# DavidPeicho/loupiote

Measured on AMD Instinct MI355X. Metric: Mrays/s (+ ms/frame) at 1920×1080, 4 spp, Sponza; 1/2/4/8 GPU, higher is better.
Workload: dtype f32

## Files before the change

bindings/rust/loupiote_hip/src/ffi.rs:

```rust
#![allow(non_camel_case_types, non_upper_case_globals, dead_code)]
use std::os::raw::{c_char, c_int, c_uint, c_void};

pub const LPT_ABI_VERSION: u32 = 6;
pub const LPT_INVALID_INDEX: u32 = 0xFFFFFFFF;
pub const LPT_ACCEL_BUILD_HOST_SAH: u32 = 0;
pub const LPT_ACCEL_BUILD_GPU_LBVH: u32 = 1;
pub const LPT_UPLOAD_NO_TEXTURE_PAIRS: u32 = 0x100;
pub const LPT_COMM_ID_BYTES: u32 = 128;
pub const LPT_OK: c_int = 0;
pub const LPT_ERR_FILE_NOT_FOUND: c_int = 1;
pub const LPT_ERR_READBACK: c_int = 2;
pub const LPT_ERR_ACCEL_BUILD: c_int = 3;
pub const LPT_ERR_HIP: c_int = 4;
pub const LPT_ERR_RCCL: c_int = 5;
pub const LPT_ERR_INVALID_ARG: c_int = 6;
pub const LPT_BLIT_PATHTRACE: c_int = 0;
pub const LPT_BLIT_DENOISED: c_int = 1;
pub const LPT_BLIT_TEMPORAL: c_int = 2;
pub const LPT_BLIT_GBUFFER: c_int = 3;
pub const LPT_BLIT_MOTION: c_int = 4;
pub const LPT_HOST_FRAME_HOST_ONLY: c_int = 1;
pub const LPT_EXCHANGE_GATHER_TILES: c_int = 0;
pub const LPT_EXCHANGE_REDUCE: c_int = 1;
pub const LPT_OPT_PACKET_PRIMARY: c_int = 1;
pub const LPT_OPT_WAVEFRONT_RAYS: c_int = 2;
pub const LPT_OPT_PATH_RAYS: c_int = 3;
pub const LPT_OPT_COOP_RAYS: c_int = 4;
pub const LPT_OPT_TAIL_LANES: c_int = 5;
pub const LPT_OPT_EXPERIMENT_BASE: c_int = 256;
pub const LPT_EXP_PIPE_RAYS: c_int = 0;
pub const LPT_EXP_REFILL: c_int = 1;
pub const LPT_EXP_TRACE_WAVES_PER_CU: c_int = 2;
pub const LPT_EXP_SHADE_BLOCKS_PER_CU: c_int = 3;
pub const LPT_EXP_PATH_WAVES_PER_CU: c_int = 4;
pub const LPT_EXP_PATH_REFILL: c_int = 5;
pub const LPT_EXP_OCC_CELL_MILLI: c_int = 6;
pub const LPT_EXP_STEP_BUDGET: c_int = 7;
pub const LPT_EXP_BUDGET_RAYS: c_int = 8;
pub const LPT_EXP_PACKET_QUADS: c_int = 9;
pub const LPT_EXP_SPLIT_RAYS: c_int = 10;
pub const LPT_EXP_BUDGET_SPLIT: c_int = 11;

#[repr(C)] pub struct lpt_device { _private: [u8; 0] }
#[repr(C)] pub struct lpt_scene { _private: [u8; 0] }
#[repr(C)] pub struct lpt_scene_gpu { _private: [u8; 0] }
#[repr(C)] pub struct lpt_probe { _private: [u8; 0] }
#[repr(C)] pub struct lpt_renderer { _private: [u8; 0] }
#[repr(C)] pub struct lpt_comm { _private: [u8; 0] }
#[repr(C)] pub struct lpt_host_frame { _private: [u8; 0] }

#[repr(C)] #[derive(Copy, Clone, Debug)]
pub struct lpt_material {
    pub color: [f32; 4],
    pub roughness: f32,
    pub reflectivity: f32,
    pub albedo_texture: u32,
    pub mra_texture: u32,
}
#[repr(C)] #[derive(Copy, Clone, Debug)]
pub struct lpt_vertex {
    pub position: [f32; 4],
    pub normal: [f32; 4],
}
#[repr(C)] #[derive(Copy, Clone, Debug)]
pub struct lpt_light {
    pub normal: [f32; 4],
    pub tangent: [f32; 4],
    pub bitangent: [f32; 4],
    pub origin: [f32; 4],
}
#[repr(C)] #[derive(Copy, Clone, Debug)]
pub struct lpt_instance {
    pub model_to_world: [f32; 16],
    pub blas_index: u32,
    pub material_index: u32,
    pub pad: [u32; 2],
}
#[repr(C)] #[derive(Copy, Clone, Debug)]
pub struct lpt_blas_entry {
    pub vertex_offset: u32,
    pub vertex_count: u32,
    pub index_offset: u32,
    pub index_count: u32,
}
#[repr(C)] #[derive(Copy, Clone, Debug)]
pub struct lpt_scene_counts {
    pub materials: u32,
    pub entries: u32,
    pub vertices: u32,
    pub indices: u32,
    pub instances: u32,
    pub lights: u32,
    pub images: u32,
}
#[repr(C)] #[derive(Copy, Clone, Debug)]
pub struct lpt_accel_stats {
    pub triangles: u32,
    pub nodes: u32,
    pub node_bytes: u32,
    pub tri_bytes: u32,
    pub max_depth: u32,
    pub build_ms: f32,
    pub host_baked_triangles: u32,
    pub upload_ms: f32,
    pub texture_pairs: u32,
    pub texture_bytes_resident: u64,
}
#[repr(C)] #[derive(Copy, Clone, Debug)]
pub struct lpt_hit {
    pub t: f32,
    pub u: f32,
    pub v: f32,
    pub prim: u32,
}
#[repr(C)] #[derive(Copy, Clone, Debug)]
pub struct lpt_ray_counts {
    pub closest: u64,
    pub shadow: u64,
    pub shaded: u64,
    pub nodes: u64,
    pub tris: u64,
    pub shadow_nodes: u64,
    pub shadow_tris: u64,
    pub wave_steps: u64,
    pub live_lanes: u64,
    pub node_lanes: u64,
    pub tri_lanes: u64,
    pub primary: u64,
    pub packet_nodes: u64,
    pub packet_tris: u64,
    pub shadow_occluded: u64,
    pub occluder_cache_found: u64,
    pub occluder_cache_hits: u64,
    pub wave_rays: u64,
}
#[repr(C)] #[derive(Copy, Clone, Debug)]
pub struct lpt_timing {
    pub label: [c_char; 32],
    pub ms: f32,
    pub launches: u32,
}

#[link(name = "loupiote_hip")]
extern "C" {
    pub fn lpt_last_error() -> *const c_char;
    pub fn lpt_status_string(status: c_int) -> *const c_char;
    pub fn lpt_abi_version() -> u32;
    pub fn lpt_device_create(hip_ordinal: c_int, out: *mut *mut lpt_device) -> c_int;
    pub fn lpt_device_destroy(dev: *mut lpt_device) -> c_int;
    pub fn lpt_device_synchronize(dev: *mut lpt_device) -> c_int;
    pub fn lpt_device_info(dev: *mut lpt_device, name: *mut c_char, name_cap: usize, compute_units: *mut c_int) -> c_int;
    pub fn lpt_device_stream(dev: *mut lpt_device, hip_stream: *mut *mut c_void) -> c_int;
    pub fn lpt_scene_create(out: *mut *mut lpt_scene) -> c_int;
    pub fn lpt_scene_destroy(scene: *mut lpt_scene) -> c_int;
    pub fn lpt_scene_counts_get(scene: *const lpt_scene, out: *mut lpt_scene_counts) -> c_int;
    pub fn lpt_scene_add_mesh(scene: *mut lpt_scene, positions: *const c_void, position_stride: usize, normals: *const c_void, normal_stride: usize, uvs: *const c_void, uv_stride: usize, vertex_count: u32, indices: *const u32, index_count: u32, out_blas_index: *mut u32) -> c_int;
    pub fn lpt_scene_add_instance(scene: *mut lpt_scene, blas_index: u32, model_to_world: *const f32, material_index: u32, out_instance_index: *mut u32) -> c_int;
    pub fn lpt_scene_set_instance_transform(scene: *mut lpt_scene, instance_index: u32, model_to_world: *const f32) -> c_int;
    pub fn lpt_scene_add_material(scene: *mut lpt_scene, m: *const lpt_material, out_index: *mut u32) -> c_int;
    pub fn lpt_scene_add_image(scene: *mut lpt_scene, rgba8: *const u8, width: u32, height: u32, out_index: *mut u32) -> c_int;
    pub fn lpt_scene_add_light(scene: *mut lpt_scene, l: *const lpt_light, out_index: *mut u32) -> c_int;
    pub fn lpt_scene_set_light(scene: *mut lpt_scene, index: u32, l: *const lpt_light) -> c_int;
    pub fn lpt_light_default(out: *mut lpt_light) -> c_int;
    pub fn lpt_scene_get_materials(s: *const lpt_scene, first: u32, count: u32, dst: *mut lpt_material) -> c_int;
    pub fn lpt_scene_get_entries(s: *const lpt_scene, first: u32, count: u32, dst: *mut lpt_blas_entry) -> c_int;
    pub fn lpt_scene_get_vertices(s: *const lpt_scene, first: u32, count: u32, dst: *mut lpt_vertex) -> c_int;
    pub fn lpt_scene_get_indices(s: *const lpt_scene, first: u32, count: u32, dst: *mut u32) -> c_int;
    pub fn lpt_scene_get_instances(s: *const lpt_scene, first: u32, count: u32, dst: *mut lpt_instance) -> c_int;
    pub fn lpt_scene_get_lights(s: *const lpt_scene, first: u32, count: u32, dst: *mut lpt_light) -> c_int;
    pub fn lpt_scene_get_image(s: *const lpt_scene, index: u32, width: *mut u32, height: *mut u32, dst_rgba8: *mut u8) -> c_int;
    pub fn lpt_load_gltf(scene: *mut lpt_scene, data: *const u8, size: usize) -> c_int;
    pub fn lpt_load_gltf_path(scene: *mut lpt_scene, path: *const c_char) -> c_int;
    pub fn lpt_write_png(path: *const c_char, rgba8: *const u8, width: u32, height: u32, row_bytes: usize) -> c_int;
    pub fn lpt_decode_hdr(data: *const u8, size: usize, rgbe8: *mut u8, capacity: usize, width: *mut u32, height: *mut u32) -> c_int;
    pub fn lpt_decode_image(data: *const u8, size: usize, rgba8: *mut u8, capacity: usize, width: *mut u32, height: *mut u32) -> c_int;
    pub fn lpt_write_hdr(path: *const c_char, rgba: *const f32, width: u32, height: u32, row_floats: usize) -> c_int;
    pub fn lpt_scene_upload(dev: *mut lpt_device, scene: *const lpt_scene, out: *mut *mut lpt_scene_gpu) -> c_int;
    pub fn lpt_scene_upload_ex(dev: *mut lpt_device, scene: *const lpt_scene, flags: u32, out: *mut *mut lpt_scene_gpu) -> c_int;
    pub fn lpt_scene_gpu_destroy(sg: *mut lpt_scene_gpu) -> c_int;
    pub fn lpt_scene_gpu_update_instances(scene_gpu: *mut lpt_scene_gpu, scene: *const lpt_scene, out_rebaked: *mut u32) -> c_int;
    pub fn lpt_scene_gpu_rebuild(scene_gpu: *mut lpt_scene_gpu, scene: *const lpt_scene) -> c_int;
    pub fn lpt_scene_gpu_stats(sg: *const lpt_scene_gpu, out: *mut lpt_accel_stats) -> c_int;
    pub fn lpt_probe_upload(dev: *mut lpt_device, rgbe8: *const u8, width: u32, height: u32, out: *mut *mut lpt_probe) -> c_int;
    pub fn lpt_probe_destroy(probe: *mut lpt_probe) -> c_int;
    pub fn lpt_trace_closest(dev: *mut lpt_device, sg: *const lpt_scene_gpu, origins: *const f32, dirs: *const f32, n: u32, out_hits: *mut lpt_hit) -> c_int;
    pub fn lpt_trace_occluded(dev: *mut lpt_device, sg: *const lpt_scene_gpu, origins: *const f32, dirs: *const f32, tmax: *const f32, n: u32, out_occluded: *mut u8) -> c_int;
    pub fn lpt_renderer_create(dev: *mut lpt_device, width: u32, height: u32, out: *mut *mut lpt_renderer) -> c_int;
    pub fn lpt_renderer_destroy(r: *mut lpt_renderer) -> c_int;
    pub fn lpt_renderer_set_downsample(r: *mut lpt_renderer, factor: f32) -> c_int;
    pub fn lpt_renderer_resize(r: *mut lpt_renderer, sg: *const lpt_scene_gpu, probe_or_null: *const lpt_probe, width: u32, height: u32) -> c_int;
    pub fn lpt_renderer_get_size(r: *const lpt_renderer, width: *mut u32, height: *mut u32) -> c_int;
    pub fn lpt_max_per_pixel_bytes() -> u32;
    pub fn lpt_renderer_set_resources(r: *mut lpt_renderer, sg: *const lpt_scene_gpu, probe_or_null: *const lpt_probe) -> c_int;
    pub fn lpt_renderer_raytrace(r: *mut lpt_renderer, view_transform: *const f32) -> c_int;
    pub fn lpt_renderer_submit(r: *mut lpt_renderer) -> c_int;
    pub fn lpt_renderer_set_max_fused(r: *mut lpt_renderer, n: u32) -> c_int;
    pub fn lpt_renderer_get_submission_stats(r: *const lpt_renderer, recorded_calls: *mut u64, wavefronts: *mut u64, pending_calls: *mut u32) -> c_int;
    pub fn lpt_renderer_raytrace_n(r: *mut lpt_renderer, view_transform: *const f32, n_samples: u32) -> c_int;
    pub fn lpt_renderer_reset_accumulation(r: *mut lpt_renderer) -> c_int;
    pub fn lpt_renderer_set_accumulate(r: *mut lpt_renderer, accumulate: c_int) -> c_int;
    pub fn lpt_renderer_get_accumulate(r: *const lpt_renderer, accumulate: *mut c_int) -> c_int;
    pub fn lpt_renderer_get_frame_state(r: *const lpt_renderer, frame_count: *mut u32, seed: *mut u32) -> c_int;
    pub fn lpt_renderer_upload_noise(r: *mut lpt_renderer, rgba8: *const u8, width: u32, height: u32, bytes_per_row: u32) -> c_int;
    pub fn lpt_renderer_use_noise(r: *mut lpt_renderer, flag: c_int) -> c_int;
    pub fn lpt_renderer_set_blit_mode(r: *mut lpt_renderer, mode: c_int) -> c_int;
    pub fn lpt_renderer_read_denoiser(r: *mut lpt_renderer, gbuffer: *mut u32, motion: *mut f32, radiance: *mut f32, history: *mut u32) -> c_int;
    pub fn lpt_renderer_blit_rgba8(r: *mut lpt_renderer, dst: *mut u8, row_bytes: usize) -> c_int;
    pub fn lpt_renderer_read_pixels(r: *mut lpt_renderer, dst: *mut u8) -> c_int;
    pub fn lpt_renderer_read_radiance(r: *mut lpt_renderer, dst: *mut f32) -> c_int;
    pub fn lpt_host_alloc(bytes: usize, out: *mut *mut c_void) -> c_int;
    pub fn lpt_host_free(ptr: *mut c_void) -> c_int;
    pub fn lpt_host_register(ptr: *mut c_void, bytes: usize) -> c_int;
    pub fn lpt_host_unregister(ptr: *mut c_void) -> c_int;
    pub fn lpt_renderer_read_radiance_owned(r: *mut lpt_renderer, frame_dst: *mut f32) -> c_int;
    pub fn lpt_host_frame_create(name: *const c_char, width: u32, height: u32, world: u32, flags: u32, out: *mut *mut lpt_host_frame) -> c_int;
    pub fn lpt_host_frame_attach(name: *const c_char, width: u32, height: u32, world: u32, flags: u32, out: *mut *mut lpt_host_frame) -> c_int;
    pub fn lpt_host_frame_ptr(f: *mut lpt_host_frame, frame: *mut *mut f32) -> c_int;
    pub fn lpt_host_frame_barrier(f: *mut lpt_host_frame, rank: u32, frame_no: u32, timeout_ms: u32) -> c_int;
    pub fn lpt_host_frame_destroy(f: *mut lpt_host_frame) -> c_int;
    pub fn lpt_renderer_get_timings(r: *mut lpt_renderer, out: *mut lpt_timing, inout_count: *mut c_int) -> c_int;
    pub fn lpt_renderer_enable_timings(r: *mut lpt_renderer, flag: c_int) -> c_int;
    pub fn lpt_renderer_set_max_bounces(r: *mut lpt_renderer, bounces: u32) -> c_int;
    pub fn lpt_renderer_set_seed(r: *mut lpt_renderer, user_seed: u32) -> c_int;
    pub fn lpt_renderer_set_vfov(r: *mut lpt_renderer, radians: f32) -> c_int;
    pub fn lpt_renderer_set_shard(r: *mut lpt_renderer, rank: u32, world_size: u32, tile_w: u32, tile_h: u32) -> c_int;
    pub fn lpt_renderer_set_shard_weighted(r: *mut lpt_renderer, rank: u32, world_size: u32, tile_w: u32, tile_h: u32, weights_or_null: *const u32) -> c_int;
    pub fn lpt_renderer_denoiser_inputs(r: *mut lpt_renderer, noisy: *mut *mut c_void, gbuffer: *mut *mut c_void, motion: *mut *mut c_void, n_pixels: *mut usize) -> c_int;
    pub fn lpt_renderer_denoise_filter(r: *mut lpt_renderer) -> c_int;
    pub fn lpt_renderer_radiance_device_ptr(r: *mut lpt_renderer, device_ptr: *mut *mut c_void, bytes: *mut usize) -> c_int;
    pub fn lpt_comm_unique_id(out_id: *mut c_void) -> c_int;
    pub fn lpt_comm_create(dev: *mut lpt_device, id: *const c_void, rank: c_int, world_size: c_int, out: *mut *mut lpt_comm) -> c_int;
    pub fn lpt_comm_destroy(comm: *mut lpt_comm) -> c_int;
    pub fn lpt_comm_info(comm: *const lpt_comm, rank: *mut c_int, world_size: *mut c_int) -> c_int;
    pub fn lpt_comm_group_begin() -> c_int;
    pub fn lpt_comm_group_end() -> c_int;
    pub fn lpt_renderer_set_comm(r: *mut lpt_renderer, comm_or_null: *mut lpt_comm) -> c_int;
    pub fn lpt_renderer_set_comm_weighted(r: *mut lpt_renderer, comm_or_null: *mut lpt_comm, weights_or_null: *const u32) -> c_int;
    pub fn lpt_renderer_exchange(r: *mut lpt_renderer, mode: c_int) -> c_int;
    pub fn lpt_renderer_exchange_local(root: *mut lpt_renderer, peers: *const *mut lpt_renderer, n_peers: c_int) -> c_int;
    pub fn lpt_renderer_set_lanes(r: *mut lpt_renderer, lanes: c_int) -> c_int;
    pub fn lpt_renderer_set_sort_queues(r: *mut lpt_renderer, flag: c_int) -> c_int;
    pub fn lpt_renderer_set_option(r: *mut lpt_renderer, option: c_int, value: u64) -> c_int;
    pub fn lpt_renderer_get_option(r: *const lpt_renderer, option: c_int, value: *mut u64) -> c_int;
    pub fn lpt_shard_layout(width: u32, height: u32, tile_w: u32, tile_h: u32, world_size: u32, rank: u32, out_slots: *mut u32, out_slot_offset: *mut u32) -> c_int;
    pub fn lpt_shard_layout_weighted(width: u32, height: u32, tile_w: u32, tile_h: u32, world_size: u32, rank: u32, weights_or_null: *const u32, out_slots: *mut u32, out_slot_offset: *mut u32) -> c_int;
    pub fn lpt_shard_owner(world_size: u32, weights_or_null: *const u32, tile: u32, out_rank: *mut u32) -> c_int;
    pub fn lpt_renderer_get_ray_counts(r: *mut lpt_renderer, out: *mut lpt_ray_counts) -> c_int;
    pub fn lpt_renderer_get_queue_counts(r: *mut lpt_renderer, closest: *mut u32, shadow: *mut u32, cap: u32) -> c_int;
    pub fn lpt_renderer_reset_ray_counts(r: *mut lpt_renderer) -> c_int;
    pub fn lpt_renderer_get_step_histogram(r: *mut lpt_renderer, max_steps: *mut u32, hist12: *mut u32) -> c_int;
    pub fn lpt_renderer_enable_stats(r: *mut lpt_renderer, flag: c_int) -> c_int;
    pub fn lpt_renderer_synchronize(r: *mut lpt_renderer) -> c_int;
    pub fn lpt_renderer_stream(r: *mut lpt_renderer, hip_stream: *mut *mut c_void) -> c_int;
}
```

include/lpt.h:

```cpp
#ifndef LPT_H
#define LPT_H

#include <stddef.h>
#include <stdint.h>

#ifdef __cplusplus
extern "C" {
#endif

#define LPT_ABI_VERSION 6u

#define LPT_INVALID_INDEX 0xFFFFFFFFu

enum {
    LPT_OK = 0,
    LPT_ERR_FILE_NOT_FOUND = 1,
    LPT_ERR_READBACK = 2,
    LPT_ERR_ACCEL_BUILD = 3,
    LPT_ERR_HIP = 4,
    LPT_ERR_RCCL = 5,
    LPT_ERR_INVALID_ARG = 6
};

const char *lpt_last_error(void);
const char *lpt_status_string(int status);
uint32_t lpt_abi_version(void);


typedef struct lpt_material {
    float color[4];
    float roughness;
    float reflectivity;
    uint32_t albedo_texture;
    uint32_t mra_texture;
} lpt_material;

typedef struct lpt_vertex {
    float position[4];
    float normal[4];
} lpt_vertex;

typedef struct lpt_light {
    float normal[4];
    float tangent[4];
    float bitangent[4];
    float origin[4];
} lpt_light;

typedef struct lpt_instance {
    float model_to_world[16];
    uint32_t blas_index;
    uint32_t material_index;
    uint32_t pad[2];
} lpt_instance;

typedef struct lpt_blas_entry {
    uint32_t vertex_offset;
    uint32_t vertex_count;
    uint32_t index_offset;
    uint32_t index_count;
} lpt_blas_entry;

typedef struct lpt_scene_counts {
    uint32_t materials, entries, vertices, indices, instances, lights, images;
} lpt_scene_counts;

typedef struct lpt_accel_stats {
    uint32_t triangles;
    uint32_t nodes;
    uint32_t node_bytes;
    uint32_t tri_bytes;
    uint32_t max_depth;
    float build_ms;
    uint32_t host_baked_triangles;
    float upload_ms;
    uint32_t texture_pairs;
    uint64_t texture_bytes_resident;
} lpt_accel_stats;

typedef struct lpt_hit {
    float t, u, v;
    uint32_t prim;
} lpt_hit;

typedef struct lpt_ray_counts {
    uint64_t closest;
    uint64_t shadow;
    uint64_t shaded;
    uint64_t nodes;
    uint64_t tris;
    uint64_t shadow_nodes;
    uint64_t shadow_tris;
    uint64_t wave_steps;
    uint64_t live_lanes;
    uint64_t node_lanes;
    uint64_t tri_lanes;
    uint64_t primary;
    uint64_t packet_nodes;
    uint64_t packet_tris;
    uint64_t shadow_occluded;
    uint64_t occluder_cache_found;
    uint64_t occluder_cache_hits;
    uint64_t wave_rays;
} lpt_ray_counts;

typedef struct lpt_timing {
    char label[32];
    float ms;
    uint32_t launches;
} lpt_timing;

enum {
    LPT_BLIT_PATHTRACE = 0,
    LPT_BLIT_DENOISED = 1,
    LPT_BLIT_TEMPORAL = 2,
    LPT_BLIT_GBUFFER = 3,
    LPT_BLIT_MOTION = 4
};

typedef struct lpt_device lpt_device;
typedef struct lpt_scene lpt_scene;
typedef struct lpt_scene_gpu lpt_scene_gpu;
typedef struct lpt_probe lpt_probe;
typedef struct lpt_renderer lpt_renderer;
typedef struct lpt_comm lpt_comm;

int lpt_device_create(int hip_ordinal, lpt_device **out);
int lpt_device_destroy(lpt_device *dev);
int lpt_device_synchronize(lpt_device *dev);
int lpt_device_info(lpt_device *dev, char *name, size_t name_cap, int *compute_units);
int lpt_device_stream(lpt_device *dev, void **hip_stream);

int lpt_scene_create(lpt_scene **out);
int lpt_scene_destroy(lpt_scene *scene);
int lpt_scene_counts_get(const lpt_scene *scene, lpt_scene_counts *out);

int lpt_scene_add_mesh(lpt_scene *scene, const void *positions, size_t position_stride,
                       const void *normals, size_t normal_stride, const void *uvs,
                       size_t uv_stride, uint32_t vertex_count, const uint32_t *indices,
                       uint32_t index_count, uint32_t *out_blas_index);
int lpt_scene_add_instance(lpt_scene *scene, uint32_t blas_index, const float model_to_world[16],
                           uint32_t material_index, uint32_t *out_instance_index);
int lpt_scene_set_instance_transform(lpt_scene *scene, uint32_t instance_index,
                                     const float model_to_world[16]);
int lpt_scene_add_material(lpt_scene *scene, const lpt_material *m, uint32_t *out_index);
int lpt_scene_add_image(lpt_scene *scene, const uint8_t *rgba8, uint32_t width, uint32_t height,
                        uint32_t *out_index);
int lpt_scene_add_light(lpt_scene *scene, const lpt_light *l, uint32_t *out_index);
int lpt_scene_set_light(lpt_scene *scene, uint32_t index, const lpt_light *l);
int lpt_light_default(lpt_light *out);

int lpt_scene_get_materials(const lpt_scene *s, uint32_t first, uint32_t count, lpt_material *dst);
int lpt_scene_get_entries(const lpt_scene *s, uint32_t first, uint32_t count, lpt_blas_entry *dst);
int lpt_scene_get_vertices(const lpt_scene *s, uint32_t first, uint32_t count, lpt_vertex *dst);
int lpt_scene_get_indices(const lpt_scene *s, uint32_t first, uint32_t count, uint32_t *dst);
int lpt_scene_get_instances(const lpt_scene *s, uint32_t first, uint32_t count, lpt_instance *dst);
int lpt_scene_get_lights(const lpt_scene *s, uint32_t first, uint32_t count, lpt_light *dst);
int lpt_scene_get_image(const lpt_scene *s, uint32_t index, uint32_t *width, uint32_t *height,
                        uint8_t *dst_rgba8 );

int lpt_load_gltf(lpt_scene *scene, const uint8_t *data, size_t size);
int lpt_load_gltf_path(lpt_scene *scene, const char *path);

int lpt_write_png(const char *path, const uint8_t *rgba8, uint32_t width, uint32_t height, size_t row_bytes);

int lpt_decode_hdr(const uint8_t *data, size_t size, uint8_t *rgbe8, size_t capacity, uint32_t *width, uint32_t *height);

int lpt_decode_image(const uint8_t *data, size_t size, uint8_t *rgba8, size_t capacity, uint32_t *width, uint32_t *height);

int lpt_write_hdr(const char *path, const float *rgba, uint32_t width, uint32_t height, size_t row_floats);

int lpt_scene_upload(lpt_device *dev, const lpt_scene *scene, lpt_scene_gpu **out);
#define LPT_ACCEL_BUILD_HOST_SAH 0u
#define LPT_ACCEL_BUILD_GPU_LBVH 1u
#define LPT_UPLOAD_NO_TEXTURE_PAIRS 0x100u
int lpt_scene_upload_ex(lpt_device *dev, const lpt_scene *scene, uint32_t flags, lpt_scene_gpu **out);
int lpt_scene_gpu_destroy(lpt_scene_gpu *sg);
int lpt_scene_gpu_update_instances(lpt_scene_gpu *scene_gpu, const lpt_scene *scene, uint32_t *out_rebaked);
int lpt_scene_gpu_rebuild(lpt_scene_gpu *scene_gpu, const lpt_scene *scene);
int lpt_scene_gpu_stats(const lpt_scene_gpu *sg, lpt_accel_stats *out);

int lpt_probe_upload(lpt_device *dev, const uint8_t *rgbe8, uint32_t width, uint32_t height,
                     lpt_probe **out);
int lpt_probe_destroy(lpt_probe *probe);

int lpt_trace_closest(lpt_device *dev, const lpt_scene_gpu *sg, const float *origins,
                      const float *dirs, uint32_t n, lpt_hit *out_hits);
int lpt_trace_occluded(lpt_device *dev, const lpt_scene_gpu *sg, const float *origins,
                       const float *dirs, const float *tmax, uint32_t n, uint8_t *out_occluded);

int lpt_renderer_create(lpt_device *dev, uint32_t width, uint32_t height, lpt_renderer **out);
int lpt_renderer_destroy(lpt_renderer *r);
int lpt_renderer_set_downsample(lpt_renderer *r, float factor);
int lpt_renderer_resize(lpt_renderer *r, const lpt_scene_gpu *sg, const lpt_probe *probe_or_null,
                        uint32_t width, uint32_t height);
int lpt_renderer_get_size(const lpt_renderer *r, uint32_t *width, uint32_t *height);
uint32_t lpt_max_per_pixel_bytes(void);
int lpt_renderer_set_resources(lpt_renderer *r, const lpt_scene_gpu *sg,
                               const lpt_probe *probe_or_null);
int lpt_renderer_raytrace(lpt_renderer *r, const float view_transform[16]);
int lpt_renderer_submit(lpt_renderer *r);
int lpt_renderer_set_max_fused(lpt_renderer *r, uint32_t n);
int lpt_renderer_get_submission_stats(const lpt_renderer *r, uint64_t *recorded_calls, uint64_t *wavefronts, uint32_t *pending_calls);
int lpt_renderer_raytrace_n(lpt_renderer *r, const float view_transform[16], uint32_t n_samples);
int lpt_renderer_reset_accumulation(lpt_renderer *r);
int lpt_renderer_set_accumulate(lpt_renderer *r, int accumulate);
int lpt_renderer_get_accumulate(const lpt_renderer *r, int *accumulate);
int lpt_renderer_get_frame_state(const lpt_renderer *r, uint32_t *frame_count, uint32_t *seed);
int lpt_renderer_upload_noise(lpt_renderer *r, const uint8_t *rgba8, uint32_t width,
                              uint32_t height, uint32_t bytes_per_row);
int lpt_renderer_use_noise(lpt_renderer *r, int flag);
int lpt_renderer_set_blit_mode(lpt_renderer *r, int mode);
int lpt_renderer_read_denoiser(lpt_renderer *r, uint32_t *gbuffer, float *motion, float *radiance, uint32_t *history);
int lpt_renderer_blit_rgba8(lpt_renderer *r, uint8_t *dst, size_t row_bytes);
int lpt_renderer_read_pixels(lpt_renderer *r, uint8_t *dst);
int lpt_renderer_read_radiance(lpt_renderer *r, float *dst);
int lpt_host_alloc(size_t bytes, void **out);
int lpt_host_free(void *ptr);
int lpt_host_register(void *ptr, size_t bytes);
int lpt_host_unregister(void *ptr);
int lpt_renderer_read_radiance_owned(lpt_renderer *r, float *frame_dst);
typedef struct lpt_host_frame lpt_host_frame;
enum { LPT_HOST_FRAME_HOST_ONLY = 1 };
int lpt_host_frame_create(const char *name, uint32_t width, uint32_t height, uint32_t world, uint32_t flags, lpt_host_frame **out);
int lpt_host_frame_attach(const char *name, uint32_t width, uint32_t height, uint32_t world, uint32_t flags, lpt_host_frame **out);
int lpt_host_frame_ptr(lpt_host_frame *f, float **frame);
int lpt_host_frame_barrier(lpt_host_frame *f, uint32_t rank, uint32_t frame_no, uint32_t timeout_ms);
int lpt_host_frame_destroy(lpt_host_frame *f);
int lpt_renderer_get_timings(lpt_renderer *r, lpt_timing *out, int *inout_count);
int lpt_renderer_enable_timings(lpt_renderer *r, int flag);

int lpt_renderer_set_max_bounces(lpt_renderer *r, uint32_t bounces);
int lpt_renderer_set_seed(lpt_renderer *r, uint32_t user_seed);
int lpt_renderer_set_vfov(lpt_renderer *r, float radians);
int lpt_renderer_set_shard(lpt_renderer *r, uint32_t rank, uint32_t world_size, uint32_t tile_w,
                           uint32_t tile_h);
int lpt_renderer_set_shard_weighted(lpt_renderer *r, uint32_t rank, uint32_t world_size, uint32_t tile_w, uint32_t tile_h,
                                    const uint32_t *weights_or_null);
int lpt_renderer_denoiser_inputs(lpt_renderer *r, void **noisy, void **gbuffer, void **motion, size_t *n_pixels);
int lpt_renderer_denoise_filter(lpt_renderer *r);
int lpt_renderer_radiance_device_ptr(lpt_renderer *r, void **device_ptr, size_t *bytes);
#define LPT_COMM_ID_BYTES 128
int lpt_comm_unique_id(void *out_id );
int lpt_comm_create(lpt_device *dev, const void *id , int rank, int world_size, lpt_comm **out);
int lpt_comm_destroy(lpt_comm *comm);
int lpt_comm_info(const lpt_comm *comm, int *rank, int *world_size);
int lpt_comm_group_begin(void);
int lpt_comm_group_end(void);

enum {
    LPT_EXCHANGE_GATHER_TILES = 0,
    LPT_EXCHANGE_REDUCE = 1
};
int lpt_renderer_set_comm(lpt_renderer *r, lpt_comm *comm_or_null);
int lpt_renderer_set_comm_weighted(lpt_renderer *r, lpt_comm *comm_or_null, const uint32_t *weights_or_null);
int lpt_renderer_exchange(lpt_renderer *r, int mode);
int lpt_renderer_exchange_local(lpt_renderer *root, lpt_renderer *const *peers, int n_peers);

int lpt_renderer_set_lanes(lpt_renderer *r, int lanes);
int lpt_renderer_set_sort_queues(lpt_renderer *r, int flag);
typedef enum lpt_option {
    LPT_OPT_PACKET_PRIMARY = 1,
    LPT_OPT_WAVEFRONT_RAYS = 2,
    LPT_OPT_PATH_RAYS = 3,
    LPT_OPT_COOP_RAYS = 4,
    LPT_OPT_TAIL_LANES = 5,
    LPT_OPT_EXPERIMENT_BASE = 256
} lpt_option;
#define LPT_OPT_EXPERIMENT(name) (LPT_OPT_EXPERIMENT_BASE + (name))
typedef enum lpt_experiment {
    LPT_EXP_PIPE_RAYS = 0,
    LPT_EXP_REFILL = 1,
    LPT_EXP_TRACE_WAVES_PER_CU = 2,
    LPT_EXP_SHADE_BLOCKS_PER_CU = 3,
    LPT_EXP_PATH_WAVES_PER_CU = 4,
    LPT_EXP_PATH_REFILL = 5,
    LPT_EXP_OCC_CELL_MILLI = 6,
    LPT_EXP_STEP_BUDGET = 7,
    LPT_EXP_BUDGET_RAYS = 8,
    LPT_EXP_PACKET_QUADS = 9,
    LPT_EXP_SPLIT_RAYS = 10,
    LPT_EXP_BUDGET_SPLIT = 11
} lpt_experiment;
int lpt_renderer_set_option(lpt_renderer *r, int option, uint64_t value);
int lpt_renderer_get_option(const lpt_renderer *r, int option, uint64_t *value);
int lpt_shard_layout(uint32_t width, uint32_t height, uint32_t tile_w, uint32_t tile_h, uint32_t world_size, uint32_t rank,
                     uint32_t *out_slots, uint32_t *out_slot_offset);
int lpt_shard_layout_weighted(uint32_t width, uint32_t height, uint32_t tile_w, uint32_t tile_h, uint32_t world_size, uint32_t rank,
                              const uint32_t *weights_or_null, uint32_t *out_slots, uint32_t *out_slot_offset);
int lpt_shard_owner(uint32_t world_size, const uint32_t *weights_or_null, uint32_t tile, uint32_t *out_rank);
int lpt_renderer_get_ray_counts(lpt_renderer *r, lpt_ray_counts *out);
int lpt_renderer_get_queue_counts(lpt_renderer *r, uint32_t *closest, uint32_t *shadow, uint32_t cap);
int lpt_renderer_reset_ray_counts(lpt_renderer *r);
int lpt_renderer_get_step_histogram(lpt_renderer *r, uint32_t *max_steps, uint32_t *hist12);
int lpt_renderer_enable_stats(lpt_renderer *r, int flag);
int lpt_renderer_synchronize(lpt_renderer *r);
int lpt_renderer_stream(lpt_renderer *r, void **hip_stream);

#ifdef __cplusplus
}
#endif
#endif
```

loupiote_amd/_abi.py:

```python
import ctypes as C
import os

import numpy as np

_HERE = os.path.dirname(os.path.abspath(__file__))
LIB_PATH = os.environ.get("LPT_LIB_PATH") or os.path.join(_HERE, "libloupiote_hip.so")

LPT_OK = 0
LPT_ERR_FILE_NOT_FOUND = 1
LPT_ERR_READBACK = 2
LPT_ERR_ACCEL_BUILD = 3
LPT_ERR_HIP = 4
LPT_ERR_RCCL = 5
LPT_ERR_INVALID_ARG = 6
COMM_ID_BYTES = 128
OPT_EXPERIMENT_BASE = 256
OPTIONS = {"packet_primary": 1, "wavefront_rays": 2, "path_rays": 3, "coop_rays": 4, "tail_lanes": 5}
EXPERIMENTS = {"pipe_rays": 0, "refill": 1, "trace_waves_per_cu": 2, "shade_blocks_per_cu": 3, "path_waves_per_cu": 4, "path_refill": 5, "occ_cell_milli": 6,
               "step_budget": 7, "budget_rays": 8, "packet_quads": 9, "split_rays": 10, "budget_split": 11}
OPTIONS.update({k: OPT_EXPERIMENT_BASE + v for k, v in EXPERIMENTS.items()})
EXCHANGE_GATHER_TILES = 0
HOST_FRAME_HOST_ONLY = 1
EXCHANGE_REDUCE = 1
INVALID_INDEX = 0xFFFFFFFF
LIGHT_BIT = 0x80000000

MATERIAL_DT = np.dtype([("color", "<f4", 4), ("roughness", "<f4"), ("reflectivity", "<f4"),
                        ("albedo_texture", "<u4"), ("mra_texture", "<u4")])
VERTEX_DT = np.dtype([("position", "<f4", 4), ("normal", "<f4", 4)])
LIGHT_DT = np.dtype([("normal", "<f4", 4), ("tangent", "<f4", 4), ("bitangent", "<f4", 4), ("origin", "<f4", 4)])
INSTANCE_DT = np.dtype([("model_to_world", "<f4", 16), ("blas_index", "<u4"), ("material_index", "<u4"),
                        ("pad", "<u4", 2)])
ENTRY_DT = np.dtype([("vertex_offset", "<u4"), ("vertex_count", "<u4"), ("index_offset", "<u4"),
                     ("index_count", "<u4")])
HIT_DT = np.dtype([("t", "<f4"), ("u", "<f4"), ("v", "<f4"), ("prim", "<u4")])


class SceneCounts(C.Structure):
    _fields_ = [(n, C.c_uint32) for n in ("materials", "entries", "vertices", "indices", "instances", "lights", "images")]


class AccelStats(C.Structure):
    _fields_ = [("triangles", C.c_uint32), ("nodes", C.c_uint32), ("node_bytes", C.c_uint32),
                ("tri_bytes", C.c_uint32), ("max_depth", C.c_uint32), ("build_ms", C.c_float),
                ("host_baked_triangles", C.c_uint32), ("upload_ms", C.c_float),
                ("texture_pairs", C.c_uint32), ("texture_bytes_resident", C.c_uint64)]


class RayCounts(C.Structure):
    _fields_ = [(n, C.c_uint64) for n in ("closest", "shadow", "shaded", "nodes", "tris", "shadow_nodes", "shadow_tris",
                                             "wave_steps", "live_lanes", "node_lanes", "tri_lanes", "primary", "packet_nodes", "packet_tris",
                                             "shadow_occluded", "occluder_cache_found", "occluder_cache_hits", "wave_rays")]


class Timing(C.Structure):
    _fields_ = [("label", C.c_char * 32), ("ms", C.c_float), ("launches", C.c_uint32)]


_vp, _u32, _i, _f, _sz = C.c_void_p, C.c_uint32, C.c_int, C.c_float, C.c_size_t
_pvp = C.POINTER(C.c_void_p)
_pu32 = C.POINTER(C.c_uint32)

SIGNATURES = {
    "lpt_last_error": (C.c_char_p, []),
    "lpt_status_string": (C.c_char_p, [_i]),
    "lpt_abi_version": (_u32, []),
    "lpt_device_create": (_i, [_i, _pvp]),
    "lpt_device_destroy": (_i, [_vp]),
    "lpt_device_synchronize": (_i, [_vp]),
    "lpt_device_info": (_i, [_vp, C.c_char_p, _sz, C.POINTER(_i)]),
    "lpt_device_stream": (_i, [_vp, _pvp]),
    "lpt_scene_create": (_i, [_pvp]),
    "lpt_scene_destroy": (_i, [_vp]),
    "lpt_scene_counts_get": (_i, [_vp, C.POINTER(SceneCounts)]),
    "lpt_scene_add_mesh": (_i, [_vp, _vp, _sz, _vp, _sz, _vp, _sz, _u32, _vp, _u32, _pu32]),
    "lpt_scene_add_instance": (_i, [_vp, _u32, _vp, _u32, _pu32]),
    "lpt_scene_set_instance_transform": (_i, [_vp, _u32, _vp]),
    "lpt_scene_add_material": (_i, [_vp, _vp, _pu32]),
    "lpt_scene_add_image": (_i, [_vp, _vp, _u32, _u32, _pu32]),
    "lpt_scene_add_light": (_i, [_vp, _vp, _pu32]),
    "lpt_scene_set_light": (_i, [_vp, _u32, _vp]),
    "lpt_light_default": (_i, [_vp]),
    "lpt_scene_get_materials": (_i, [_vp, _u32, _u32, _vp]),
    "lpt_scene_get_entries": (_i, [_vp, _u32, _u32, _vp]),
    "lpt_scene_get_vertices": (_i, [_vp, _u32, _u32, _vp]),
    "lpt_scene_get_indices": (_i, [_vp, _u32, _u32, _vp]),
    "lpt_scene_get_instances": (_i, [_vp, _u32, _u32, _vp]),
    "lpt_scene_get_lights": (_i, [_vp, _u32, _u32, _vp]),
    "lpt_scene_get_image": (_i, [_vp, _u32, _pu32, _pu32, _vp]),
    "lpt_load_gltf": (_i, [_vp, _vp, _sz]),
    "lpt_load_gltf_path": (_i, [_vp, C.c_char_p]),
    "lpt_decode_hdr": (_i, [_vp, C.c_size_t, _vp, C.c_size_t, C.POINTER(C.c_uint32), C.POINTER(C.c_uint32)]),
    "lpt_decode_image": (_i, [_vp, C.c_size_t, _vp, C.c_size_t, C.POINTER(C.c_uint32), C.POINTER(C.c_uint32)]),
    "lpt_write_hdr": (_i, [C.c_char_p, _vp, _u32, _u32, _sz]),
    "lpt_write_png": (_i, [C.c_char_p, _vp, _u32, _u32, _sz]),
    "lpt_scene_upload": (_i, [_vp, _vp, _pvp]),
    "lpt_scene_upload_ex": (_i, [_vp, _vp, _u32, _pvp]),
    "lpt_scene_gpu_destroy": (_i, [_vp]),
    "lpt_scene_gpu_stats": (_i, [_vp, C.POINTER(AccelStats)]),
    "lpt_scene_gpu_rebuild": (_i, [_vp, _vp]),
    "lpt_scene_gpu_update_instances": (_i, [_vp, _vp, C.POINTER(C.c_uint32)]),
    "lpt_probe_upload": (_i, [_vp, _vp, _u32, _u32, _pvp]),
    "lpt_probe_destroy": (_i, [_vp]),
    "lpt_trace_closest": (_i, [_vp, _vp, _vp, _vp, _u32, _vp]),
    "lpt_trace_occluded": (_i, [_vp, _vp, _vp, _vp, _vp, _u32, _vp]),
    "lpt_renderer_create": (_i, [_vp, _u32, _u32, _pvp]),
    "lpt_renderer_destroy": (_i, [_vp]),
    "lpt_renderer_set_downsample": (_i, [_vp, _f]),
    "lpt_renderer_resize": (_i, [_vp, _vp, _vp, _u32, _u32]),
    "lpt_renderer_get_size": (_i, [_vp, _pu32, _pu32]),
    "lpt_max_per_pixel_bytes": (_u32, []),
    "lpt_renderer_set_resources": (_i, [_vp, _vp, _vp]),
    "lpt_renderer_raytrace": (_i, [_vp, _vp]),
    "lpt_renderer_raytrace_n": (_i, [_vp, _vp, _u32]),
    "lpt_renderer_submit": (_i, [_vp]),
    "lpt_renderer_set_max_fused": (_i, [_vp, _u32]),
    "lpt_renderer_get_submission_stats": (_i, [_vp, C.POINTER(C.c_uint64), C.POINTER(C.c_uint64), _pu32]),
    "lpt_host_alloc": (_i, [_sz, _pvp]),
    "lpt_host_free": (_i, [_vp]),
    "lpt_host_register": (_i, [_vp, _sz]),
    "lpt_host_unregister": (_i, [_vp]),
    "lpt_renderer_read_radiance_owned": (_i, [_vp, _vp]),
    "lpt_host_frame_create": (_i, [C.c_char_p, _u32, _u32, _u32, _u32, _pvp]),
    "lpt_host_frame_attach": (_i, [C.c_char_p, _u32, _u32, _u32, _u32, _pvp]),
    "lpt_host_frame_ptr": (_i, [_vp, _pvp]),
    "lpt_host_frame_barrier": (_i, [_vp, _u32, _u32, _u32]),
    "lpt_host_frame_destroy": (_i, [_vp]),
    "lpt_renderer_reset_accumulation": (_i, [_vp]),
    "lpt_renderer_set_accumulate": (_i, [_vp, _i]),
    "lpt_renderer_get_accumulate": (_i, [_vp, C.POINTER(_i)]),
    "lpt_renderer_get_frame_state": (_i, [_vp, _pu32, _pu32]),
    "lpt_renderer_upload_noise": (_i, [_vp, _vp, _u32, _u32, _u32]),
    "lpt_renderer_use_noise": (_i, [_vp, _i]),
    "lpt_renderer_set_blit_mode": (_i, [_vp, _i]),
    "lpt_renderer_blit_rgba8": (_i, [_vp, _vp, _sz]),
    "lpt_renderer_read_pixels": (_i, [_vp, _vp]),
    "lpt_renderer_read_radiance": (_i, [_vp, _vp]),
    "lpt_renderer_read_denoiser": (_i, [_vp, _vp, _vp, _vp, _vp]),
    "lpt_renderer_get_timings": (_i, [_vp, _vp, C.POINTER(_i)]),
    "lpt_renderer_enable_timings": (_i, [_vp, _i]),
    "lpt_renderer_set_max_bounces": (_i, [_vp, _u32]),
    "lpt_renderer_set_seed": (_i, [_vp, _u32]),
    "lpt_renderer_set_vfov": (_i, [_vp, _f]),
    "lpt_renderer_set_shard": (_i, [_vp, _u32, _u32, _u32, _u32]),
    "lpt_renderer_radiance_device_ptr": (_i, [_vp, _pvp, C.POINTER(_sz)]),
    "lpt_renderer_denoiser_inputs": (_i, [_vp, C.POINTER(C.c_void_p), C.POINTER(C.c_void_p), C.POINTER(C.c_void_p), C.POINTER(C.c_size_t)]),
    "lpt_renderer_denoise_filter": (_i, [_vp]),
    "lpt_comm_unique_id": (_i, [_vp]),
    "lpt_comm_create": (_i, [_vp, _vp, _i, _i, _pvp]),
    "lpt_comm_destroy": (_i, [_vp]),
    "lpt_comm_info": (_i, [_vp, C.POINTER(_i), C.POINTER(_i)]),
    "lpt_comm_group_begin": (_i, []),
    "lpt_comm_group_end": (_i, []),
    "lpt_renderer_set_comm": (_i, [_vp, _vp]),
    "lpt_renderer_exchange": (_i, [_vp, _i]),
    "lpt_renderer_exchange_local": (_i, [_vp, _pvp, _i]),
    "lpt_shard_layout": (_i, [_u32, _u32, _u32, _u32, _u32, _u32, _pu32, _pu32]),
    "lpt_shard_layout_weighted": (_i, [_u32, _u32, _u32, _u32, _u32, _u32, _vp, _pu32, _pu32]),
    "lpt_shard_owner": (_i, [_u32, _vp, _u32, _pu32]),
    "lpt_renderer_set_shard_weighted": (_i, [_vp, _u32, _u32, _u32, _u32, _vp]),
    "lpt_renderer_set_comm_weighted": (_i, [_vp, _vp, _vp]),
    "lpt_renderer_set_lanes": (_i, [_vp, _i]),
    "lpt_renderer_set_sort_queues": (_i, [_vp, _i]),
    "lpt_renderer_set_option": (_i, [_vp, _i, C.c_uint64]),
    "lpt_renderer_get_option": (_i, [_vp, _i, C.POINTER(C.c_uint64)]),
    "lpt_renderer_get_queue_counts": (_i, [_vp, _vp, _vp, _u32]),
    "lpt_renderer_get_ray_counts": (_i, [_vp, C.POINTER(RayCounts)]),
    "lpt_renderer_reset_ray_counts": (_i, [_vp]),
    "lpt_renderer_get_step_histogram": (_i, [_vp, _pu32, _vp]),
    "lpt_renderer_enable_stats": (_i, [_vp, _i]),
    "lpt_renderer_synchronize": (_i, [_vp]),
    "lpt_renderer_stream": (_i, [_vp, _pvp]),
}

_LIB = None


def lib():
    global _LIB
    if _LIB is None:
        if not os.path.exists(LIB_PATH):
            raise ImportError(
                "loupiote_amd: %s is missing — build it with `python -c 'import __graft_entry__ as g; g.build()'` "
                "(hipcc --offload-arch=gfx950).  There is no fallback path." % LIB_PATH)
        L = C.CDLL(LIB_PATH)
        for name, (res, args) in SIGNATURES.items():
            if os.environ.get("LPT_ABI_LENIENT") and not hasattr(L, name):
                continue
            fn = getattr(L, name)
            fn.restype = res
            fn.argtypes = args
        _LIB = L
    return _LIB


def ptr(a):
    return None if a is None else a.ctypes.data_as(C.c_void_p)
```

loupiote_amd/csrc/device.hip:

```cpp
#include <hip/hip_runtime.h>

#include <dlfcn.h>

#include <algorithm>
#include <cmath>
#include <map>
#include <memory>
#include <cstdlib>
#include <mutex>
#include <new>
#include <numeric>

#include "common.h"
#include "kernels.h"
#include "build_kernels.h"
#include <hipcub/hipcub.hpp>
#include <rccl/rccl.h>

using namespace lpt;
using namespace lptd;

#define TRY(expr) do { const int st__ = (expr); if (st__ != LPT_OK) return st__; } while (0)
#define HIP_TRY(expr)                                                                              \
    do {                                                                                           \
        hipError_t e__ = (expr);                                                                   \
        if (e__ != hipSuccess) return fail(LPT_ERR_HIP, "%s failed: %s", #expr, hipGetErrorString(e__)); \
    } while (0)

struct lpt_device {
    int ordinal = 0;
    hipStream_t stream = nullptr;
    int compute_units = 0;
    char name[128] = {0};
    std::vector<lpt_renderer *> renderers;
};

struct lpt_comm {
    lpt_device *dev = nullptr;
    ncclComm_t comm = nullptr;
    int rank = 0, world = 1;
};

struct Rccl {
    void *handle = nullptr;
    ncclResult_t (*GetUniqueId)(ncclUniqueId *) = nullptr;
    ncclResult_t (*CommInitRank)(ncclComm_t *, int, ncclUniqueId, int) = nullptr;
    ncclResult_t (*CommDestroy)(ncclComm_t) = nullptr;
    ncclResult_t (*CommCount)(const ncclComm_t, int *) = nullptr;
    ncclResult_t (*CommUserRank)(const ncclComm_t, int *) = nullptr;
    ncclResult_t (*GroupStart)() = nullptr;
    ncclResult_t (*GroupEnd)() = nullptr;
    ncclResult_t (*Send)(const void *, size_t, ncclDataType_t, int, ncclComm_t, hipStream_t) = nullptr;
    ncclResult_t (*Recv)(void *, size_t, ncclDataType_t, int, ncclComm_t, hipStream_t) = nullptr;
    ncclResult_t (*Reduce)(const void *, void *, size_t, ncclDataType_t, ncclRedOp_t, int, ncclComm_t, hipStream_t) = nullptr;
    const char *(*GetErrorString)(ncclResult_t) = nullptr;
};
static const Rccl *rccl() {
    static Rccl table;
    static int state = 0;
    static std::string why = "missing symbol";
    static std::mutex mu;
    std::lock_guard<std::mutex> lock(mu);
    if (state == 1) return &table;
    if (state == 0) {
        const char *names[] = {"librccl.so.1", "librccl.so", "/opt/rocm/lib/librccl.so.1", "/opt/rocm/lib/librccl.so"};
        std::string rocm_path;
        if (const char *rp = getenv("ROCM_PATH")) rocm_path = std::string(rp) + "/lib/librccl.so";
        void *h = nullptr;
        state = -1;
        if (const char *lp = getenv("LPT_RCCL_LIBRARY")) { h = dlopen(lp, RTLD_NOW | RTLD_LOCAL); rocm_path.clear(); if (!h) { if (const char *e = dlerror()) why = e; goto rccl_done; } }
        if (!rocm_path.empty()) h = dlopen(rocm_path.c_str(), RTLD_NOW | RTLD_LOCAL);
        for (size_t i = 0; !h && i < sizeof names / sizeof names[0]; ++i) h = dlopen(names[i], RTLD_NOW | RTLD_LOCAL);
        if (!h) { if (const char *e = dlerror()) why = e; }
        if (h) {
            table.handle = h;
            bool ok = true;
#define RCCL_SYM(field, sym) do { *(void **)(&table.field) = dlsym(h, sym); if (!table.field) ok = false; } while (0)
            RCCL_SYM(GetUniqueId, "ncclGetUniqueId"); RCCL_SYM(CommInitRank, "ncclCommInitRank"); RCCL_SYM(CommDestroy, "ncclCommDestroy");
            RCCL_SYM(CommCount, "ncclCommCount"); RCCL_SYM(CommUserRank, "ncclCommUserRank");
            RCCL_SYM(GroupStart, "ncclGroupStart"); RCCL_SYM(GroupEnd, "ncclGroupEnd"); RCCL_SYM(Send, "ncclSend"); RCCL_SYM(Recv, "ncclRecv");
            RCCL_SYM(Reduce, "ncclReduce"); RCCL_SYM(GetErrorString, "ncclGetErrorString");
#undef RCCL_SYM
            if (ok) state = 1;
        }
    rccl_done:;
    }
    if (state == 1) return &table;
    fail(LPT_ERR_RCCL, "librccl could not be loaded (%s): the multi-GPU frame exchange needs RCCL", why.c_str());
    return nullptr;
}

#define RCCL_TRY(expr)                                                                                \
    do {                                                                                              \
        ncclResult_t r__ = (expr);                                                                    \
        if (r__ != ncclSuccess) return fail(LPT_ERR_RCCL, "%s failed: %s", #expr, rccl() ? rccl()->GetErrorString(r__) : "?"); \
    } while (0)

struct HipFree { void operator()(void *p) const { hipFree(p); } };
using DevMem = std::unique_ptr<void, HipFree>;
template <typename T> static inline T *as(const DevMem &m) { return (T *)m.get(); }

struct DevTree {
    DevMem nodes, woop, leaf_prim;
    DevMem node_lo, node_hi;
    std::vector<uint32_t> level_start;
    uint32_t n_nodes = 0, max_depth = 0;
    float build_ms = 0.f;
};

struct TexturePairs {
    std::map<std::pair<uint32_t, uint32_t>, uint32_t> map;
    std::vector<DImage> descs;
    std::vector<uint8_t> image_resident;
};

struct lpt_scene_gpu {
    lpt_device *dev = nullptr;
    DScene d{};
    float max_abs = 0.f;
    DevTree tree;
    DevMem tri_verts, materials, lights, texels, images, srgb_lut, pair_texels, pair_images;
    TexturePairs pairs;
    lpt_accel_stats stats{};
    DevMem obj_verts, obj_indices, bad_flag;
    DevMem arena;
    size_t arena_bytes = 0;
    std::vector<uint32_t> inst_first, inst_count;
    std::vector<lpt_instance> instances;
    size_t n_entries = 0, n_vertices = 0, n_indices = 0;
};

struct lpt_probe {
    lpt_device *dev = nullptr;
    DProbe d{};
    void *rgbe = nullptr;
};

enum { ST_RAYGEN = 0, ST_INTERSECT, ST_SHADE, ST_SHADOW, ST_ACCUM, ST_ASVGF, ST_EXCHANGE, ST_PRIMARY, ST_PATH, ST_COUNT };
static const char *kStageLabel[ST_COUNT] = {"ray generation", "intersection", "shading", "shadow", "accumulation", "asvgf", "exchange", "primary intersection", "path"};

struct Wavefront {
    hipStream_t stream = nullptr;
    Queue q[2]{};
    ShadowQueue sq{};
    float4 *hits = nullptr, *Lsum = nullptr;
    uint32_t *strag = nullptr;
    FrameCounters *ctr = nullptr;
    size_t ray_cap = 0;
    hipEvent_t done = nullptr;
    hipEvent_t consumed = nullptr;
    bool consumed_recorded = false;
};
constexpr int kMaxLanes = 4;
constexpr uint32_t kStepBudget = 48u, kBudgetRays = 3000000u;
constexpr float kPacketMaxPixelRad = 1.8e-3f;
constexpr uint32_t kOccEntries = 1u << 18;
constexpr uint32_t kPathRays = 120000u;
constexpr uint64_t kSplitRays = 3000000ull;
constexpr uint32_t kCoopRays = 32000u;
constexpr uint32_t kPacketBlocksPerCu = 128u;
constexpr uint32_t kCoopWavesPerCu = 32u;
constexpr uint64_t kWavefrontRays = 1ull << 22;

struct lpt_renderer {
    lpt_device *dev = nullptr;
    hipStream_t stream = nullptr;
    Wavefront wf[kMaxLanes];
    int n_lanes = 2;
    uint32_t lane_rr = 0;
    int last_lane = 0;
    uint32_t req_w = 0, req_h = 0, w = 0, h = 0;
    float downsample = 0.5f;
    const lpt_scene_gpu *sg = nullptr;
    const lpt_probe *probe = nullptr;
    bool resources_set = false;
    uint32_t frame_count = 1, seed = 0;
    bool accumulate = false, frame_back = true;
    struct Pending { float view[16]; uint32_t n = 0, frame_count0 = 1, seed0 = 0; bool acc0 = false; } pend;
    uint32_t max_fused = 0;
    uint32_t packet_primary = 2u;
    uint32_t pipe_rays = 0x7FFFFFFFu;
    uint64_t wavefront_rays = kWavefrontRays;
    uint32_t path_rays = kPathRays;
    uint32_t path_waves_per_cu = 16;
    int path_refill = 32;
    uint64_t n_recorded = 0, n_wavefronts = 0;
    int mode = LPT_BLIT_PATHTRACE;
    uint32_t max_bounces = 3, user_seed = 0;
    float vfov = 0.78539816339744830962f;
    uint32_t rank = 0, world = 1, tile_w = 32, tile_h = 8;
    std::vector<uint32_t> weights;
    ShardMap map{1u, 1u, {0u}};
    ShardTable h_table{};
    std::vector<uint32_t> h_offset;
    ShardTable *d_table = nullptr;
    bool use_noise = false, stats = false, timings = false;
    int refill = 44;
    int sort_queues = 0;
    uint32_t shade_blocks_per_cu = 0;
    uint32_t trace_waves_per_cu = 0;
    uint32_t n_slots = 0;
    float4 *accum = nullptr, *scratch = nullptr;
    lpt_comm *comm = nullptr;
    float4 *frame = nullptr, *xstage = nullptr;
    size_t xstage_elems = 0;
    bool presented = false;
    hipEvent_t xevent = nullptr;
    bool xevent_recorded = false;
    Totals *totals = nullptr;
    uint32_t step_budget = kStepBudget, budget_rays = kBudgetRays;
    bool budget_split = false;
    uint32_t coop_rays = kCoopRays;
    uint32_t tail_lanes = 4u;
    uint64_t split_rays = kSplitRays;
    uint32_t *err_host = nullptr, *err_dev = nullptr;
    bool packet_quads = true;
    uint32_t *occ_table = nullptr;
    float occ_cell = 0.25f;
    void *default_probe = nullptr;
    float *srgb_thr = nullptr;
    void *noise = nullptr;
    uint32_t noise_w = 0, noise_h = 0;
    uint4 *den_gbuf[2]{};
    float4 *den_rad[2]{};
    float2 *den_mom[2]{};
    uint32_t *den_hist[2]{};
    float2 *den_motion = nullptr;
    float4 *den_temp = nullptr;
    float4 *den_noisy = nullptr;
    float4 *den_nd = nullptr;
    bool den_inputs_ready = false;
    int den_cur = 1;
    CamBasis prev_cam{};
    static constexpr int kRing = 8;
    static constexpr int kMaxEvents = 3 * kMaxBounces + 4;
    hipEvent_t *ev_start = nullptr, *ev_stop = nullptr;
    int ev_stage[kRing][kMaxEvents]{};
    int ev_count[kRing]{};
    uint64_t ring_pos = 0;
    double stage_ms[ST_COUNT]{};
    uint32_t stage_launches[ST_COUNT]{};
};

static inline uint32_t div_up(uint32_t a, uint32_t b) { return (a + b - 1u) / b; }
struct ReadPlan {
    float *radiance = nullptr;
    uint8_t *rgba8 = nullptr;
    size_t row_bytes = 0;
};
static int flush_pending(lpt_renderer *r, const ReadPlan *read = nullptr);
static void forget_deferred_exchange(lpt_renderer *r);
static FrameParams shard_params(const lpt_renderer *r);
static inline uint32_t stream_grid(const lpt_renderer *r, size_t n);
#define FLUSH_OR_RETURN(r) do { int fst__ = flush_pending(r); if (fst__ != LPT_OK) return fst__; } while (0)
static int flush_device(lpt_device *dev) {
    int st = LPT_OK;
    if (!dev) return st;
    for (lpt_renderer *r : dev->renderers) {
        const int f = flush_pending(r);
        if (st == LPT_OK) st = f;
    }
    return st;
}
static inline const float4 *presented_target(const lpt_renderer *r) { return (r->presented && r->frame) ? r->frame : r->accum; }
static int check_device_error(lpt_renderer *r) {
    if (!r->err_host) return LPT_OK;
    const uint32_t code = *(volatile uint32_t *)r->err_host;
    if (!code) return LPT_OK;
    *(volatile uint32_t *)r->err_host = 0u;
    return fail(LPT_ERR_HIP, "a device-side bounded wait ran out (code 0x%x): the frame is void", code);
}
static inline size_t stack_bytes(const DScene &sc) { return (size_t)sc.stack_entries * kTraceBlock * sizeof(uint2); }

static int dev_alloc(DevMem &m, size_t bytes) {
    void *p = nullptr;
    HIP_TRY(hipMalloc(&p, bytes));
    m.reset(p);
    return LPT_OK;
}

template <typename T>
static int upload(DevMem &dst, const std::vector<T> &src, hipStream_t s) {
    TRY(dev_alloc(dst, sizeof(T) * std::max<size_t>(src.size(), 1u)));
    if (!src.empty()) HIP_TRY(hipMemcpyAsync(dst.get(), src.data(), sizeof(T) * src.size(), hipMemcpyHostToDevice, s));
    return LPT_OK;
}

static int scene_bounds_and_grid(lpt_scene_gpu *sg, uint32_t n, hipStream_t s, float blo[3], float bhi[3], bool keep_pad) {
    int hb[6];
    const int init[6] = {0x7FFFFFFF, 0x7FFFFFFF, 0x7FFFFFFF, (int)0x80000000, (int)0x80000000, (int)0x80000000};
    DevMem db;
    TRY(dev_alloc(db, sizeof init));
    HIP_TRY(hipMemcpyAsync(db.get(), init, sizeof init, hipMemcpyHostToDevice, s));
    hipLaunchKernelGGL(k_lbvh_bounds, dim3(std::min<uint32_t>(div_up(n, 256u), 1024u)), dim3(256), 0, s, sg->d, n, as<int>(db));
    HIP_TRY(hipMemcpyAsync(hb, db.get(), sizeof hb, hipMemcpyDeviceToHost, s));
    HIP_TRY(hipStreamSynchronize(s));
    for (int a = 0; a < 6; ++a) { const int o = hb[a] >= 0 ? hb[a] : hb[a] ^ 0x7FFFFFFF; float f; memcpy(&f, &o, 4); (a < 3 ? blo[a] : bhi[a - 3]) = f; }
    float now_abs = 0.0f;
    for (int a = 0; a < 3; ++a) now_abs = std::max(now_abs, std::max(fabsf(blo[a]), fabsf(bhi[a])));
    sg->max_abs = keep_pad ? std::max(sg->max_abs, now_abs) : now_abs;
    sg->d.pad_abs = kScenePad * sg->max_abs;
    float glo[3], ghi[3];
    for (int a = 0; a < 3; ++a) {
        const float e = 4.0f * sg->d.pad_abs + 2e-6f * (bhi[a] - blo[a]) + 1e-30f;
        glo[a] = blo[a] - e;
        ghi[a] = bhi[a] + e;
    }
    scene_grid(glo, ghi, sg->d.grid_lo, sg->d.grid_step);
    return LPT_OK;
}

static void refit_levels(const DScene &d, const DevTree &t, hipStream_t s) {
    for (size_t l = t.level_start.size() - 1; l-- > 0;) {
        const uint32_t a = t.level_start[l], b = t.level_start[l + 1];
        if (b > a) hipLaunchKernelGGL(k_refit_level, dim3(div_up(b - a, 64u)), dim3(64), 0, s, d, as<uint4>(t.nodes), as<float4>(t.node_lo), as<float4>(t.node_hi), a, b);
    }
}

static void scatter_woop(const DevTree &t, const void *woop_prim, uint32_t first, uint32_t count, hipStream_t s) {
    const uint32_t n_places = kNodeTris * t.n_nodes;
    hipLaunchKernelGGL(k_lbvh_scatter_woop, dim3(div_up(n_places, 256u)), dim3(256), 0, s, (const float4 *)woop_prim, as<float4>(t.woop), as<const uint32_t>(t.leaf_prim),
                       n_places, first, count);
}

static int build_lbvh(lpt_scene_gpu *sg, uint32_t n, const void *woop_prim, hipStream_t s, DevTree &out) {
    const auto t0 = std::chrono::steady_clock::now();
    float blo[3], bhi[3];
    TRY(scene_bounds_and_grid(sg, n, s, blo, bhi, false));
    float binv[3];
    for (int a = 0; a < 3; ++a) binv[a] = bhi[a] > blo[a] ? 1.0f / (bhi[a] - blo[a]) : 0.0f;

    size_t sort_bytes = 0, scan_bytes = 0;
    hipcub::DeviceRadixSort::SortPairs(nullptr, sort_bytes, (uint32_t *)nullptr, (uint32_t *)nullptr, (uint32_t *)nullptr, (uint32_t *)nullptr, (int)n, 0, 30, s);
    hipcub::DeviceScan::ExclusiveSum(nullptr, scan_bytes, (uint32_t *)nullptr, (uint32_t *)nullptr, (int)n, s);
    const size_t cub_cap = std::max(sort_bytes, scan_bytes);
    const size_t need = (size_t)n * 400u + cub_cap + 64u * 256u;
    if (sg->arena_bytes < need) {
        sg->arena.reset();
        sg->arena_bytes = 0;
        if (dev_alloc(sg->arena, need) != LPT_OK) return fail(LPT_ERR_HIP, "GPU BVH build: out of device memory (%zu bytes of scratch)", need);
        sg->arena_bytes = need;
    }
    size_t arena_used = 0;
    auto carve = [&](auto *&p, size_t count) {
        const size_t at = (arena_used + 255u) & ~(size_t)255u;
        p = (std::remove_reference_t<decltype(p)>)((char *)sg->arena.get() + at);
        arena_used = at + sizeof(*p) * count;
    };
    uint32_t *keys, *vals, *keys_s, *vals_s, *leaf_big, *inner_count, *tri_count, *inner_off, *tri_off;
    uint8_t *cub_tmp;
    uint4 *nodes_big;
    int *items_a, *items_b, *kid_ref;
    LbvhTree T{};
    carve(keys, n); carve(vals, n); carve(keys_s, n); carve(vals_s, n);
    carve(T.left, n); carve(T.right, n); carve(T.parent, n); carve(T.leaf_parent, n);
    carve(T.first, n); carve(T.last, n); carve(T.lo, n); carve(T.hi, n); carve(T.tri_lo, n); carve(T.tri_hi, n); carve(T.flag, n);
    carve(cub_tmp, cub_cap);
    carve(nodes_big, 4u * (size_t)n);
    carve(leaf_big, (size_t)kNodeTris * n);
    carve(items_a, n); carve(items_b, n); carve(kid_ref, 8u * (size_t)n);
    carve(inner_count, n); carve(tri_count, n); carve(inner_off, n); carve(tri_off, n);
    if (arena_used > sg->arena_bytes) return fail(LPT_ERR_HIP, "GPU BVH build: out of device memory");
    T.sorted_tri = vals_s; T.keys = keys_s; T.n = n;

    const uint32_t b256 = div_up(n, 256u);
    hipLaunchKernelGGL(k_lbvh_morton, dim3(b256), dim3(256), 0, s, sg->d, n, make_float3(blo[0], blo[1], blo[2]), make_float3(binv[0], binv[1], binv[2]), keys, vals);
    size_t cub_bytes = cub_cap;
    if (hipcub::DeviceRadixSort::SortPairs(cub_tmp, cub_bytes, keys, keys_s, vals, vals_s, (int)n, 0, 30, s) != hipSuccess) return fail(LPT_ERR_HIP, "GPU BVH build: sort failed");
    hipLaunchKernelGGL(k_lbvh_leaf_boxes, dim3(b256), dim3(256), 0, s, sg->d, T);
    HIP_TRY(hipMemsetAsync(T.flag, 0, sizeof(uint32_t) * n, s));
    hipLaunchKernelGGL(k_lbvh_tree, dim3(b256), dim3(256), 0, s, T);
    hipLaunchKernelGGL(k_lbvh_fit, dim3(b256), dim3(256), 0, s, T);

    HIP_TRY(hipMemsetAsync(leaf_big, 0xFF, sizeof(uint32_t) * (size_t)kNodeTris * n, s));
    HIP_TRY(hipMemsetAsync(items_a, 0, sizeof(int), s));
    int *items_cur = items_a, *items_next = items_b;
    uint32_t n_items = 1, level_first = 0, tri_running = 0;
    DevTree t;
    while (n_items) {
        if (t.level_start.size() > 64) return fail(LPT_ERR_ACCEL_BUILD, "GPU BVH build: tree deeper than 64 levels");
        LbvhLevel L{items_cur, n_items, kid_ref, inner_count, tri_count};
        hipLaunchKernelGGL(k_lbvh_collapse, dim3(div_up(n_items, 64u)), dim3(64), 0, s, T, L);
        cub_bytes = cub_cap;
        hipcub::DeviceScan::ExclusiveSum(cub_tmp, cub_bytes, inner_count, inner_off, (int)n_items, s);
        cub_bytes = cub_cap;
        hipcub::DeviceScan::ExclusiveSum(cub_tmp, cub_bytes, tri_count, tri_off, (int)n_items, s);
        uint32_t tail[4];
        HIP_TRY(hipMemcpyAsync(&tail[0], inner_off + (n_items - 1), 4, hipMemcpyDeviceToHost, s));
        HIP_TRY(hipMemcpyAsync(&tail[1], inner_count + (n_items - 1), 4, hipMemcpyDeviceToHost, s));
        HIP_TRY(hipMemcpyAsync(&tail[2], tri_off + (n_items - 1), 4, hipMemcpyDeviceToHost, s));
        HIP_TRY(hipMemcpyAsync(&tail[3], tri_count + (n_items - 1), 4, hipMemcpyDeviceToHost, s));
        HIP_TRY(hipStreamSynchronize(s));
        const uint32_t inner_total = tail[0] + tail[1], tri_total = tail[2] + tail[3];
        if ((size_t)level_first + n_items + inner_total > n) return fail(LPT_ERR_ACCEL_BUILD, "GPU BVH build: node budget exceeded");
        hipLaunchKernelGGL(k_lbvh_emit, dim3(div_up(n_items, 64u)), dim3(64), 0, s, T, L, inner_off, tri_off, level_first, level_first + n_items, tri_running,
                           nodes_big, leaf_big, items_next);
        t.level_start.push_back(level_first);
        level_first += n_items;
        tri_running += tri_total;
        n_items = inner_total;
        std::swap(items_cur, items_next);
    }
    t.level_start.push_back(level_first);
    if (tri_running != n) return fail(LPT_ERR_ACCEL_BUILD, "GPU BVH build: %u of %u triangles referenced", tri_running, n);
    t.n_nodes = level_first;
    t.max_depth = (uint32_t)t.level_start.size() - 1u;
    const size_t places = (size_t)kNodeTris * t.n_nodes;
    TRY(dev_alloc(t.nodes, sizeof(Node8) * (size_t)t.n_nodes));
    HIP_TRY(hipMemcpyAsync(t.nodes.get(), nodes_big, sizeof(Node8) * (size_t)t.n_nodes, hipMemcpyDeviceToDevice, s));
    TRY(dev_alloc(t.node_lo, sizeof(float4) * (size_t)t.n_nodes));
    TRY(dev_alloc(t.node_hi, sizeof(float4) * (size_t)t.n_nodes));
    TRY(dev_alloc(t.leaf_prim, sizeof(uint32_t) * places));
    HIP_TRY(hipMemcpyAsync(t.leaf_prim.get(), leaf_big, sizeof(uint32_t) * places, hipMemcpyDeviceToDevice, s));
    TRY(dev_alloc(t.woop, sizeof(WoopTri) * places));
    HIP_TRY(hipMemsetAsync(t.woop.get(), 0, sizeof(WoopTri) * places, s));
    scatter_woop(t, woop_prim, 0u, n, s);
    DScene d = sg->d;
    d.leaf_prim = as<const uint32_t>(t.leaf_prim);
    refit_levels(d, t, s);
    HIP_TRY(hipGetLastError());
    HIP_TRY(hipStreamSynchronize(s));
    t.build_ms = std::chrono::duration<float, std::milli>(std::chrono::steady_clock::now() - t0).count();
    out = std::move(t);
    return LPT_OK;
}

static int refit(lpt_scene_gpu *sg) {
    hipStream_t s = sg->dev->stream;
    float blo[3], bhi[3];
    TRY(scene_bounds_and_grid(sg, sg->stats.triangles, s, blo, bhi, true));
    refit_levels(sg->d, sg->tree, s);
    HIP_TRY(hipGetLastError());
    HIP_TRY(hipStreamSynchronize(s));
    return LPT_OK;
}

static void bind_view(lpt_scene_gpu *sg) {
    const DevTree &t = sg->tree;
    sg->d.nodes = as<const DNode8>(t.nodes);
    sg->d.leaf_prim = as<const uint32_t>(t.leaf_prim);
    sg->d.woop = as<const float4>(t.woop);
    sg->d.stack_entries = t.max_depth > 2u ? t.max_depth - 1u : 1u;
    sg->stats.nodes = t.n_nodes;
    sg->stats.max_depth = t.max_depth;
    sg->stats.build_ms = t.build_ms;
}

static lpt_material device_material(const TexturePairs &p, const lpt_material &m, bool *ok = nullptr) {
    lpt_material d = m;
    if (ok) *ok = true;
    const auto it = p.map.find(std::make_pair(m.albedo_texture, m.mra_texture));
    if (it != p.map.end()) {
        const DImage &di = p.descs[it->second];
        d.albedo_texture = kPairedBit | di.offset;
        d.mra_texture = di.width | (di.height << 16);
        return d;
    }
    uint32_t *ids[2] = {&d.albedo_texture, &d.mra_texture};
    for (uint32_t *id : ids) {
        if (*id >= p.image_resident.size()) *id = LPT_INVALID_INDEX;
        else if (!p.image_resident[*id] && ok) *ok = false;
    }
    return d;
}

static int bake_instances(lpt_scene_gpu *sg, const lpt_scene &scene, const std::vector<uint32_t> &which, void *woop_prim) {
    std::vector<BakeArgs> args;
    for (uint32_t i : which) {
        const lpt_instance &now = scene.instances[i];
        const uint32_t n = sg->inst_count[i];
        if (!n) continue;
        const lpt_blas_entry &e = scene.entries[now.blas_index];
        if (e.index_count / 3u != n) return fail(LPT_ERR_INVALID_ARG, "triangle count of instance %u changed since the upload", i);
        BakeArgs a;
        memcpy(a.m, now.model_to_world, sizeof a.m);
        const float *m = a.m;
        const float a00 = m[0], a10 = m[1], a20 = m[2], a01 = m[4], a11 = m[5], a21 = m[6], a02 = m[8], a12 = m[9], a22 = m[10];
        a.c[0] = a11 * a22 - a12 * a21; a.c[1] = a12 * a20 - a10 * a22; a.c[2] = a10 * a21 - a11 * a20;
        a.c[3] = a02 * a21 - a01 * a22; a.c[4] = a00 * a22 - a02 * a20; a.c[5] = a01 * a20 - a00 * a21;
        a.c[6] = a01 * a12 - a02 * a11; a.c[7] = a02 * a10 - a00 * a12; a.c[8] = a00 * a11 - a01 * a10;
        a.vertex_offset = e.vertex_offset; a.index_offset = e.index_offset; a.first_tri = sg->inst_first[i]; a.n_tris = n;
        bool resident = true;
        const lpt_material dm = device_material(sg->pairs, scene.materials[now.material_index < scene.materials.size() ? now.material_index : 0u], &resident);
        if (!resident) return fail(LPT_ERR_INVALID_ARG, "instance %u now samples a texture on its own that was uploaded only as half of an (albedo, mra) pair: upload the scene again", i);
        memcpy(a.mat, &dm, 32);
        args.push_back(a);
    }
    if (args.empty()) return LPT_OK;
    hipStream_t s = sg->dev->stream;
    for (const BakeArgs &a : args)
        hipLaunchKernelGGL(k_bake_instance, dim3(div_up(a.n_tris, 256u)), dim3(256), 0, s, a, as<const float4>(sg->obj_verts), as<const uint32_t>(sg->obj_indices),
                           as<float4>(sg->tri_verts), (float4 *)woop_prim, as<uint32_t>(sg->bad_flag));
    uint32_t bad = 0;
    HIP_TRY(hipMemcpyAsync(&bad, sg->bad_flag.get(), sizeof bad, hipMemcpyDeviceToHost, s));
    HIP_TRY(hipStreamSynchronize(s));
    if (!bad) return LPT_OK;
    HIP_TRY(hipMemsetAsync(sg->bad_flag.get(), 0, sizeof bad, s));
    return fail(LPT_ERR_ACCEL_BUILD, "non-finite vertex in a baked instance");
}

static std::vector<uint32_t> every_instance(const lpt_scene &scene) {
    std::vector<uint32_t> all(scene.instances.size());
    std::iota(all.begin(), all.end(), 0u);
    return all;
}

static int check_same_layout(const lpt_scene_gpu *sg, const lpt_scene &scene, const char *fn) {
    if (scene.instances.size() != sg->instances.size() || scene.entries.size() != sg->n_entries ||
        scene.vertices.size() != sg->n_vertices || scene.indices.size() != sg->n_indices)
        return fail(LPT_ERR_INVALID_ARG, "%s: the scene's meshes / instance list changed since the upload; upload again", fn);
    for (size_t i = 0; i < scene.instances.size(); ++i)
        if (scene.instances[i].blas_index != sg->instances[i].blas_index) return fail(LPT_ERR_INVALID_ARG, "%s: instance %zu refers to another mesh; upload again", fn, i);
    return LPT_OK;
}

static int instance_layout(const lpt_scene &scene, Accel &acc, uint32_t &n_tris) {
    size_t total = 0;
    for (const lpt_instance &in : scene.instances) {
        const uint32_t cnt = in.blas_index < scene.entries.size() ? scene.entries[in.blas_index].index_count / 3u : 0u;
        acc.inst_first.push_back((uint32_t)total);
        acc.inst_count.push_back(cnt);
        total += cnt;
    }
    if (total >= (1u << 29)) return fail(LPT_ERR_ACCEL_BUILD, "too many triangles (%zu)", total);
    n_tris = (uint32_t)total;
    return LPT_OK;
}

static std::vector<uint64_t> pair_textures(const lpt_scene &scene, bool enable, TexturePairs &p) {
    std::vector<uint64_t> texels;
    const size_t budget = (size_t)1 << 30;
    for (const lpt_material &m : scene.materials) {
        if (!enable) break;
        const uint32_t a = m.albedo_texture, r = m.mra_texture;
        if (a >= scene.images.size() || r >= scene.images.size()) continue;
        const Image &ia = scene.images[a], &ir = scene.images[r];
        if (ia.width != ir.width || ia.height != ir.height || !ia.width || !ia.height || ia.width > 65535u || ia.height > 65535u) continue;
        if (p.map.count(std::make_pair(a, r))) continue;
        const uint32_t tx = (ia.width + 2u) / 3u, ty = (ia.height + 2u) / 3u;
        if ((texels.size() + (size_t)tx * ty * 16u) * 8u > budget || texels.size() + (size_t)tx * ty * 16u > 0x3FFFFFFFull) continue;
        DImage di;
        di.offset = (uint32_t)texels.size();
        di.width = ia.width; di.height = ia.height; di.pad = tx;
        const size_t base = texels.size();
        texels.resize(base + (size_t)tx * ty * 16u, 0);
        for (uint32_t tyi = 0; tyi < ty; ++tyi)
            for (uint32_t txi = 0; txi < tx; ++txi)
                for (uint32_t j = 0; j < 4u; ++j)
                    for (uint32_t i = 0; i < 4u; ++i) {
                        const uint32_t x = (3u * txi + i) % ia.width, y = (3u * tyi + j) % ia.height;
                        uint32_t wa, wr;
                        memcpy(&wa, &ia.rgba8[4u * ((size_t)y * ia.width + x)], 4);
                        memcpy(&wr, &ir.rgba8[4u * ((size_t)y * ir.width + x)], 4);
                        texels[base + ((size_t)tyi * tx + txi) * 16u + j * 4u + i] = (uint64_t)wa | ((uint64_t)wr << 32);
                    }
        p.map[std::make_pair(a, r)] = (uint32_t)p.descs.size();
        p.descs.push_back(di);
    }
    std::vector<uint8_t> referenced(scene.images.size(), 0), alone(scene.images.size(), 0);
    for (const lpt_material &m : scene.materials) {
        const bool paired = p.map.count(std::make_pair(m.albedo_texture, m.mra_texture)) != 0;
        for (uint32_t id : {m.albedo_texture, m.mra_texture})
            if (id < scene.images.size()) { referenced[id] = 1; if (!paired) alone[id] = 1; }
    }
    p.image_resident.assign(scene.images.size(), 1);
    for (size_t i = 0; i < scene.images.size(); ++i) p.image_resident[i] = (!referenced[i] || alone[i]) ? 1 : 0;
    return texels;
}

static std::vector<uint8_t> tiled_atlas(const lpt_scene &scene, const std::vector<uint8_t> &image_resident, std::vector<DImage> &descs) {
    std::vector<uint8_t> texels;
    for (size_t ii = 0; ii < scene.images.size(); ++ii) {
        const Image &im = scene.images[ii];
        DImage di;
        di.offset = (uint32_t)(texels.size() / 4);
        if (!image_resident[ii]) {
            di.width = di.height = di.pad = 0u;
            descs.push_back(di);
            continue;
        }
        di.width = im.width; di.height = im.height;
        const uint32_t tx = (im.width + 7u) / 8u, ty = (im.height + 3u) / 4u;
        di.pad = tx;
        descs.push_back(di);
        const size_t base = texels.size();
        texels.resize(base + (size_t)tx * ty * 128u, 0);
        for (uint32_t y = 0; y < im.height; ++y)
            for (uint32_t x = 0; x < im.width; ++x)
                memcpy(&texels[base + 4u * (((size_t)(y >> 2) * tx + (x >> 3)) * 32u + (y & 3u) * 8u + (x & 7u))], &im.rgba8[4u * ((size_t)y * im.width + x)], 4);
    }
    return texels;
}

struct TriRec { float4 v[kTriRec]; };
static_assert(sizeof(TriRec) == 128 && sizeof(lpt_vertex) * 3 == 96 && sizeof(lpt_material) == 32, "shading record layout");
static std::vector<TriRec> shading_records(const lpt_scene &scene, const Accel &acc, const TexturePairs &p) {
    std::vector<TriRec> recs(acc.tri_material.size());
    for (size_t t = 0; t < recs.size(); ++t) {
        memcpy(recs[t].v, &acc.tri_verts[3 * t], 96);
        const lpt_material dm = device_material(p, scene.materials[acc.tri_material[t] < scene.materials.size() ? acc.tri_material[t] : 0]);
        memcpy(&recs[t].v[6], &dm, 32);
    }
    return recs;
}

extern "C" {

int lpt_device_create(int hip_ordinal, lpt_device **out) {
    if (!out) return fail(LPT_ERR_INVALID_ARG, "lpt_device_create: null out");
    int n = 0;
    hipError_t e = hipGetDeviceCount(&n);
    if (e != hipSuccess || n <= 0)
        return fail(LPT_ERR_HIP, "no HIP device visible (%s); this library has no CPU fallback", e == hipSuccess ? "count = 0" : hipGetErrorString(e));
    if (hip_ordinal < 0 || hip_ordinal >= n) return fail(LPT_ERR_INVALID_ARG, "HIP ordinal %d out of range (%d devices)", hip_ordinal, n);
    HIP_TRY(hipSetDevice(hip_ordinal));
    hipDeviceProp_t prop;
    HIP_TRY(hipGetDeviceProperties(&prop, hip_ordinal));
    lpt_device *d = new (std::nothrow) lpt_device();
    if (!d) return fail(LPT_ERR_INVALID_ARG, "out of host memory");
    d->ordinal = hip_ordinal;
    d->compute_units = prop.multiProcessorCount;
    snprintf(d->name, sizeof d->name, "%s (%s)", prop.name, prop.gcnArchName);
    hipError_t se = hipStreamCreateWithFlags(&d->stream, hipStreamNonBlocking);
    if (se != hipSuccess) { delete d; return fail(LPT_ERR_HIP, "hipStreamCreate failed: %s", hipGetErrorString(se)); }
    *out = d;
    return LPT_OK;
}

int lpt_device_destroy(lpt_device *dev) {
    if (!dev) return LPT_OK;
    hipSetDevice(dev->ordinal);
    hipStreamSynchronize(dev->stream);
    hipStreamDestroy(dev->stream);
    delete dev;
    return LPT_OK;
}

int lpt_device_synchronize(lpt_device *dev) {
    if (!dev) return fail(LPT_ERR_INVALID_ARG, "lpt_device_synchronize: null");
    HIP_TRY(hipStreamSynchronize(dev->stream));
    return LPT_OK;
}

int lpt_device_info(lpt_device *dev, char *name, size_t cap, int *cus) {
    if (!dev) return fail(LPT_ERR_INVALID_ARG, "lpt_device_info: null");
    if (name && cap) snprintf(name, cap, "%s", dev->name);
    if (cus) *cus = dev->compute_units;
    return LPT_OK;
}

int lpt_device_stream(lpt_device *dev, void **stream) {
    if (!dev || !stream) return fail(LPT_ERR_INVALID_ARG, "lpt_device_stream: null");
    *stream = (void *)dev->stream;
    return LPT_OK;
}

int lpt_scene_gpu_destroy(lpt_scene_gpu *sg) {
    if (!sg) return LPT_OK;
    hipSetDevice(sg->dev->ordinal);
    flush_device(sg->dev);
    hipDeviceSynchronize();
    for (lpt_renderer *r : sg->dev->renderers)
        if (r->sg == sg) { r->sg = nullptr; r->resources_set = false; }
    delete sg;
    return LPT_OK;
}

int lpt_scene_upload(lpt_device *dev, const lpt_scene *scene, lpt_scene_gpu **out) { return lpt_scene_upload_ex(dev, scene, LPT_ACCEL_BUILD_HOST_SAH, out); }

int lpt_scene_upload_ex(lpt_device *dev, const lpt_scene *scene, uint32_t flags, lpt_scene_gpu **out) {
    if (!dev || !scene || !out) return fail(LPT_ERR_INVALID_ARG, "lpt_scene_upload: null");
    if ((flags & ~LPT_UPLOAD_NO_TEXTURE_PAIRS) > LPT_ACCEL_BUILD_GPU_LBVH) return fail(LPT_ERR_INVALID_ARG, "lpt_scene_upload_ex: unknown flags %u", flags);
    const bool enable_pairs = !(flags & LPT_UPLOAD_NO_TEXTURE_PAIRS);
    flags &= ~LPT_UPLOAD_NO_TEXTURE_PAIRS;
    HIP_TRY(hipSetDevice(dev->ordinal));
    const auto t_upload = std::chrono::steady_clock::now();
    Accel acc;
    uint32_t n_tris = 0;
    bool gpu_build = flags == LPT_ACCEL_BUILD_GPU_LBVH;
    if (gpu_build) {
        TRY(instance_layout(*scene, acc, n_tris));
        gpu_build = n_tris >= 16u;
    }
    if (!gpu_build) {
        TRY(bake_and_build(*scene, acc));
        n_tris = (uint32_t)acc.tri_material.size();
    }
    TexturePairs pairs;
    const std::vector<uint64_t> pair_texels = pair_textures(*scene, enable_pairs, pairs);
    std::vector<DImage> descs;
    const std::vector<uint8_t> texels = tiled_atlas(*scene, pairs.image_resident, descs);
    const std::vector<TriRec> recs = gpu_build ? std::vector<TriRec>() : shading_records(*scene, acc, pairs);
    std::vector<float> lut(256);
    for (int i = 0; i < 256; ++i) {
        const double c = (double)i / 255.0;
        lut[i] = (float)(c <= 0.04045 ? c / 12.92 : pow((c + 0.055) / 1.055, 2.4));
    }
    const std::vector<uint32_t> zero(1, 0u);

    std::unique_ptr<lpt_scene_gpu, int (*)(lpt_scene_gpu *)> sg(new lpt_scene_gpu(), lpt_scene_gpu_destroy);
    sg->dev = dev;
    sg->pairs = std::move(pairs);
    hipStream_t s = dev->stream;
    if (gpu_build) {
        TRY(dev_alloc(sg->tri_verts, sizeof(TriRec) * (size_t)n_tris));
    } else {
        DevTree &t = sg->tree;
        t.n_nodes = (uint32_t)acc.nodes.size();
        t.max_depth = acc.max_depth;
        t.level_start = acc.level_start;
        t.build_ms = acc.build_ms;
        TRY(upload(t.nodes, acc.nodes, s));
        TRY(upload(t.woop, acc.woop, s));
        TRY(upload(t.leaf_prim, acc.leaf_prim, s));
        const size_t box_bytes = sizeof(float4) * std::max<size_t>(t.n_nodes, 1u);
        TRY(dev_alloc(t.node_lo, box_bytes));
        TRY(dev_alloc(t.node_hi, box_bytes));
        HIP_TRY(hipMemsetAsync(t.node_lo.get(), 0, box_bytes, s));
        HIP_TRY(hipMemsetAsync(t.node_hi.get(), 0, box_bytes, s));
        TRY(upload(sg->tri_verts, recs, s));
    }
    TRY(upload(sg->materials, scene->materials, s));
    TRY(upload(sg->lights, scene->lights, s));
    TRY(upload(sg->images, descs, s));
    TRY(upload(sg->texels, texels, s));
    TRY(upload(sg->pair_images, sg->pairs.descs, s));
    TRY(upload(sg->pair_texels, pair_texels, s));
    TRY(upload(sg->srgb_lut, lut, s));
    TRY(upload(sg->obj_verts, scene->vertices, s));
    TRY(upload(sg->obj_indices, scene->indices, s));
    TRY(upload(sg->bad_flag, zero, s));
    HIP_TRY(hipStreamSynchronize(s));
    sg->inst_first = acc.inst_first; sg->inst_count = acc.inst_count;
    sg->instances = scene->instances;
    sg->n_entries = scene->entries.size(); sg->n_vertices = scene->vertices.size(); sg->n_indices = scene->indices.size();

    DScene &d = sg->d;
    sg->max_abs = acc.max_abs;
    d.pad_abs = kScenePad * acc.max_abs;
    for (int a = 0; a < 3; ++a) { d.grid_lo[a] = acc.grid_lo[a]; d.grid_step[a] = acc.grid_step[a]; }
    d.tri_verts = as<const float4>(sg->tri_verts);
    d.materials = as<const lpt_material>(sg->materials);
    d.lights = as<const lpt_light>(sg->lights);
    d.texels = as<const uint8_t>(sg->texels);
    d.images = as<const DImage>(sg->images);
    d.srgb_lut = as<const float>(sg->srgb_lut);
    d.pair_texels = as<const uint2>(sg->pair_texels);
    d.pair_images = as<const DImage>(sg->pair_images);
    d.n_pairs = (uint32_t)sg->pairs.descs.size();
    d.n_tris = n_tris;
    d.n_materials = (uint32_t)scene->materials.size();
    d.n_lights = (uint32_t)scene->lights.size();
    d.n_images = (uint32_t)scene->images.size();
    sg->stats.triangles = d.n_tris;
    sg->stats.node_bytes = (uint32_t)sizeof(Node8);
    sg->stats.tri_bytes = (uint32_t)sizeof(WoopTri);
    sg->stats.host_baked_triangles = gpu_build ? 0u : n_tris;
    sg->stats.texture_bytes_resident = (uint64_t)texels.size() + 8u * (uint64_t)pair_texels.size();
    sg->stats.texture_pairs = d.n_pairs;

    if (gpu_build) {
        DevMem woop_prim;
        TRY(dev_alloc(woop_prim, sizeof(WoopTri) * (size_t)n_tris));
        TRY(bake_instances(sg.get(), *scene, every_instance(*scene), woop_prim.get()));
        TRY(build_lbvh(sg.get(), n_tris, woop_prim.get(), s, sg->tree));
    }
    bind_view(sg.get());
    sg->stats.upload_ms = std::chrono::duration<float, std::milli>(std::chrono::steady_clock::now() - t_upload).count();
    *out = sg.release();
    return LPT_OK;
}

int lpt_scene_gpu_stats(const lpt_scene_gpu *sg, lpt_accel_stats *out) {
    if (!sg || !out) return fail(LPT_ERR_INVALID_ARG, "lpt_scene_gpu_stats: null");
    *out = sg->stats;
    return LPT_OK;
}

int lpt_scene_gpu_update_instances(lpt_scene_gpu *sg, const lpt_scene *scene, uint32_t *out_rebaked) {
    if (!sg || !scene) return fail(LPT_ERR_INVALID_ARG, "lpt_scene_gpu_update_instances: null");
    TRY(check_same_layout(sg, *scene, "lpt_scene_gpu_update_instances"));
    HIP_TRY(hipSetDevice(sg->dev->ordinal));
    TRY(flush_device(sg->dev));
    HIP_TRY(hipDeviceSynchronize());
    std::vector<uint32_t> changed;
    for (size_t i = 0; i < scene->instances.size(); ++i)
        if (memcmp(&scene->instances[i], &sg->instances[i], sizeof(lpt_instance)) != 0) changed.push_back((uint32_t)i);
    if (!changed.empty()) {
        DevMem woop_prim;
        TRY(dev_alloc(woop_prim, sizeof(WoopTri) * (size_t)std::max(sg->stats.triangles, 1u)));
        const int st = bake_instances(sg, *scene, changed, woop_prim.get());
        if (st == LPT_ERR_INVALID_ARG) return st;
        for (uint32_t i : changed) {
            sg->instances[i] = scene->instances[i];
            if (sg->inst_count[i]) scatter_woop(sg->tree, woop_prim.get(), sg->inst_first[i], sg->inst_count[i], sg->dev->stream);
        }
        if (st != LPT_OK) return st;
        if (sg->stats.triangles) TRY(refit(sg));
    }
    if (out_rebaked) *out_rebaked = (uint32_t)changed.size();
    return LPT_OK;
}

int lpt_scene_gpu_rebuild(lpt_scene_gpu *sg, const lpt_scene *scene) {
    if (!sg || !scene) return fail(LPT_ERR_INVALID_ARG, "lpt_scene_gpu_rebuild: null");
    TRY(check_same_layout(sg, *scene, "lpt_scene_gpu_rebuild"));
    const uint32_t n = sg->stats.triangles;
    if (n < 16u) return lpt_scene_gpu_update_instances(sg, scene, nullptr);
    HIP_TRY(hipSetDevice(sg->dev->ordinal));
    TRY(flush_device(sg->dev));
    HIP_TRY(hipDeviceSynchronize());
    DevMem woop_prim;
    TRY(dev_alloc(woop_prim, sizeof(WoopTri) * (size_t)n));
    TRY(bake_instances(sg, *scene, every_instance(*scene), woop_prim.get()));
    DevTree t;
    const int st = build_lbvh(sg, n, woop_prim.get(), sg->dev->stream, t);
    if (st == LPT_OK) {
        sg->tree = std::move(t);
        bind_view(sg);
    } else {
        scatter_woop(sg->tree, woop_prim.get(), 0u, n, sg->dev->stream);
        refit(sg);
    }
    sg->instances = scene->instances;
    return st;
}

int lpt_probe_upload(lpt_device *dev, const uint8_t *rgbe8, uint32_t w, uint32_t h, lpt_probe **out) {
    if (!dev || !rgbe8 || !w || !h || !out) return fail(LPT_ERR_INVALID_ARG, "lpt_probe_upload: null or empty");
    HIP_TRY(hipSetDevice(dev->ordinal));
    lpt_probe *p = new lpt_probe();
    p->dev = dev;
    hipError_t e = hipMalloc(&p->rgbe, (size_t)w * h * 4);
    if (e == hipSuccess) e = hipMemcpy(p->rgbe, rgbe8, (size_t)w * h * 4, hipMemcpyHostToDevice);
    if (e != hipSuccess) { if (p->rgbe) hipFree(p->rgbe); delete p; return fail(LPT_ERR_HIP, "probe upload failed: %s", hipGetErrorString(e)); }
    p->d.rgbe = (const uint8_t *)p->rgbe;
    p->d.w = w; p->d.h = h;
    *out = p;
    return LPT_OK;
}

int lpt_probe_destroy(lpt_probe *p) {
    if (!p) return LPT_OK;
    hipSetDevice(p->dev->ordinal);
    flush_device(p->dev);
    hipDeviceSynchronize();
    for (lpt_renderer *r : p->dev->renderers)
        if (r->probe == p) r->probe = nullptr;
    if (p->rgbe) hipFree(p->rgbe);
    delete p;
    return LPT_OK;
}

int lpt_trace_closest(lpt_device *dev, const lpt_scene_gpu *sg, const float *origins, const float *dirs, uint32_t n, lpt_hit *out) {
    if (!dev || !sg || (n && (!origins || !dirs || !out))) return fail(LPT_ERR_INVALID_ARG, "lpt_trace_closest: null");
    if (!n) return LPT_OK;
    HIP_TRY(hipSetDevice(dev->ordinal));
    std::vector<float4> o(n), d(n);
    for (uint32_t i = 0; i < n; ++i) {
        o[i] = make_float4(origins[3 * i], origins[3 * i + 1], origins[3 * i + 2], 0.f);
        d[i] = make_float4(dirs[3 * i], dirs[3 * i + 1], dirs[3 * i + 2], -1.f);
    }
    float4 *dO = nullptr, *dD = nullptr, *dH = nullptr;
    int st = LPT_OK;
    hipError_t e = hipMalloc(&dO, sizeof(float4) * n);
    if (e == hipSuccess) e = hipMalloc(&dD, sizeof(float4) * n);
    if (e == hipSuccess) e = hipMalloc(&dH, sizeof(float4) * n);
    if (e == hipSuccess) e = hipMemcpyAsync(dO, o.data(), sizeof(float4) * n, hipMemcpyHostToDevice, dev->stream);
    if (e == hipSuccess) e = hipMemcpyAsync(dD, d.data(), sizeof(float4) * n, hipMemcpyHostToDevice, dev->stream);
    if (e == hipSuccess) {
        hipLaunchKernelGGL(k_query_closest, dim3(div_up(n, kTraceBlock)), dim3(kTraceBlock), stack_bytes(sg->d), dev->stream, sg->d, dO, dD, dH, n);
        e = hipGetLastError();
    }
    if (e == hipSuccess) e = hipMemcpyAsync(out, dH, sizeof(float4) * n, hipMemcpyDeviceToHost, dev->stream);
    if (e == hipSuccess) e = hipStreamSynchronize(dev->stream);
    if (e != hipSuccess) st = fail(LPT_ERR_HIP, "lpt_trace_closest: %s", hipGetErrorString(e));
    hipFree(dO); hipFree(dD); hipFree(dH);
    return st;
}

int lpt_trace_occluded(lpt_device *dev, const lpt_scene_gpu *sg, const float *origins, const float *dirs, const float *tmax, uint32_t n, uint8_t *out) {
    if (!dev || !sg || (n && (!origins || !dirs || !tmax || !out))) return fail(LPT_ERR_INVALID_ARG, "lpt_trace_occluded: null");
    if (!n) return LPT_OK;
    HIP_TRY(hipSetDevice(dev->ordinal));
    std::vector<float4> o(n), d(n);
    for (uint32_t i = 0; i < n; ++i) {
        o[i] = make_float4(origins[3 * i], origins[3 * i + 1], origins[3 * i + 2], tmax[i]);
        d[i] = make_float4(dirs[3 * i], dirs[3 * i + 1], dirs[3 * i + 2], 0.f);
    }
    float4 *dO = nullptr, *dD = nullptr;
    uint8_t *dR = nullptr;
    int st = LPT_OK;
    hipError_t e = hipMalloc(&dO, sizeof(float4) * n);
    if (e == hipSuccess) e = hipMalloc(&dD, sizeof(float4) * n);
    if (e == hipSuccess) e = hipMalloc(&dR, n);
    if (e == hipSuccess) e = hipMemcpyAsync(dO, o.data(), sizeof(float4) * n, hipMemcpyHostToDevice, dev->stream);
    if (e == hipSuccess) e = hipMemcpyAsync(dD, d.data(), sizeof(float4) * n, hipMemcpyHostToDevice, dev->stream);
    if (e == hipSuccess) {
        hipLaunchKernelGGL(k_query_occluded, dim3(div_up(n, kTraceBlock)), dim3(kTraceBlock), stack_bytes(sg->d), dev->stream, sg->d, dO, dD, dR, n);
        e = hipGetLastError();
    }
    if (e == hipSuccess) e = hipMemcpyAsync(out, dR, n, hipMemcpyDeviceToHost, dev->stream);
    if (e == hipSuccess) e = hipStreamSynchronize(dev->stream);
    if (e != hipSuccess) st = fail(LPT_ERR_HIP, "lpt_trace_occluded: %s", hipGetErrorString(e));
    hipFree(dO); hipFree(dD); hipFree(dR);
    return st;
}

static void free_denoiser(lpt_renderer *r) {
    for (int k = 0; k < 2; ++k) {
        if (r->den_gbuf[k]) hipFree(r->den_gbuf[k]);
        if (r->den_rad[k]) hipFree(r->den_rad[k]);
        if (r->den_mom[k]) hipFree(r->den_mom[k]);
        if (r->den_hist[k]) hipFree(r->den_hist[k]);
        r->den_gbuf[k] = nullptr; r->den_rad[k] = nullptr; r->den_mom[k] = nullptr; r->den_hist[k] = nullptr;
    }
    if (r->den_motion) hipFree(r->den_motion);
    if (r->den_temp) hipFree(r->den_temp);
    if (r->den_noisy) hipFree(r->den_noisy);
    if (r->den_nd) hipFree(r->den_nd);
    r->den_motion = nullptr; r->den_temp = nullptr; r->den_noisy = nullptr; r->den_nd = nullptr;
    r->den_inputs_ready = false;
    r->den_cur = 1;
}

static int alloc_denoiser(lpt_renderer *r);
static int ensure_denoiser(lpt_renderer *r) {
    if (r->den_temp) return LPT_OK;
    const int st = alloc_denoiser(r);
    if (st != LPT_OK) free_denoiser(r);
    return st;
}
static int alloc_denoiser(lpt_renderer *r) {
    const size_t n = (size_t)r->w * r->h;
    hipStream_t s = r->stream;
    for (int k = 0; k < 2; ++k) {
        HIP_TRY(hipMalloc(&r->den_gbuf[k], sizeof(uint4) * n));
        HIP_TRY(hipMalloc(&r->den_rad[k], sizeof(float4) * n));
        HIP_TRY(hipMalloc(&r->den_mom[k], sizeof(float2) * n));
        HIP_TRY(hipMalloc(&r->den_hist[k], sizeof(uint32_t) * n));
        HIP_TRY(hipMemsetAsync(r->den_gbuf[k], 0, sizeof(uint4) * n, s));
        HIP_TRY(hipMemsetAsync(r->den_rad[k], 0, sizeof(float4) * n, s));
        HIP_TRY(hipMemsetAsync(r->den_mom[k], 0, sizeof(float2) * n, s));
        HIP_TRY(hipMemsetAsync(r->den_hist[k], 0, sizeof(uint32_t) * n, s));
    }
    HIP_TRY(hipMalloc(&r->den_motion, sizeof(float2) * n));
    HIP_TRY(hipMalloc(&r->den_noisy, sizeof(float4) * n));
    HIP_TRY(hipMalloc(&r->den_nd, sizeof(float4) * n));
    HIP_TRY(hipMalloc(&r->den_temp, sizeof(float4) * n));
    HIP_TRY(hipMemsetAsync(r->den_noisy, 0, sizeof(float4) * n, s));
    HIP_TRY(hipMemsetAsync(r->den_motion, 0, sizeof(float2) * n, s));
    HIP_TRY(hipStreamSynchronize(s));
    return LPT_OK;
}

static void free_ray_buffers(Wavefront &wf) {
    void *ptrs[] = {wf.q[0].o, wf.q[0].d, wf.q[0].T, wf.q[1].o, wf.q[1].d, wf.q[1].T, wf.sq.o, wf.sq.d, wf.sq.c, wf.hits, wf.Lsum, wf.strag};
    for (void *p : ptrs) if (p) hipFree(p);
    wf.q[0] = Queue{}; wf.q[1] = Queue{}; wf.sq = ShadowQueue{};
    wf.hits = wf.Lsum = nullptr;
    wf.strag = nullptr;
    wf.ray_cap = 0;
}

static void free_frame_buffers(lpt_renderer *r) {
    free_denoiser(r);
    for (int l = 0; l < kMaxLanes; ++l) free_ray_buffers(r->wf[l]);
    if (r->accum) hipFree(r->accum);
    if (r->scratch) hipFree(r->scratch);
    r->accum = r->scratch = nullptr;
    if (r->frame) hipFree(r->frame);
    if (r->xstage) hipFree(r->xstage);
    r->frame = r->xstage = nullptr;
    r->xstage_elems = 0;
    r->xevent_recorded = false;
    r->presented = false;
    r->n_slots = 0;
}

static std::vector<uint32_t> deal_virtual_ranks(const std::vector<uint32_t> &weights, uint32_t world) {
    std::vector<uint32_t> owner;
    if (weights.empty()) { owner.resize(world); for (uint32_t q = 0; q < world; ++q) owner[q] = q; return owner; }
    uint32_t V = 0;
    for (uint32_t wq : weights) V += wq;
    std::vector<uint32_t> given(world, 0u);
    for (uint32_t v = 0; v < V; ++v) {
        uint32_t best = 0;
        long long best_deficit = -(1ll << 60);
        for (uint32_t q = 0; q < world; ++q) {
            const long long deficit = (long long)weights[q] * (v + 1u) - (long long)given[q] * V;
            if (given[q] < weights[q] && deficit > best_deficit) { best = q; best_deficit = deficit; }
        }
        owner.push_back(best);
        given[best]++;
    }
    return owner;
}
static inline uint32_t tiles_of_virtual(uint32_t n_tiles, uint32_t V, uint32_t v) { return n_tiles / V + (v < n_tiles % V ? 1u : 0u); }
static ShardMap make_shard_map(const std::vector<uint32_t> &weights, uint32_t rank, uint32_t world) {
    ShardMap m{};
    const std::vector<uint32_t> owner = deal_virtual_ranks(weights, world);
    m.V = (uint32_t)owner.size();
    for (uint32_t v = 0; v < m.V; ++v)
        if (owner[v] == rank && m.w < kMaxWeight) m.vlist[m.w++] = v;
    return m;
}
static uint32_t owned_tiles(const ShardMap &m, uint32_t n_tiles) {
    uint32_t n = 0;
    for (uint32_t j = 0; j < m.w; ++j) n += tiles_of_virtual(n_tiles, m.V, m.vlist[j]);
    return n;
}
static ShardTable make_shard_table(const std::vector<uint32_t> &weights, uint32_t world, uint32_t n_tiles, uint32_t area, std::vector<uint32_t> &offsets) {
    ShardTable t{};
    offsets.assign((size_t)world + 1u, 0u);
    if (weights.empty()) {
        t.V = world;
        t.unit_world = world;
        for (uint32_t q = 0; q <= world; ++q) offsets[q] = shard_slot_offset(n_tiles, world, area, q);
        return t;
    }
    const std::vector<uint32_t> owner = deal_virtual_ranks(weights, world);
    t.V = (uint32_t)owner.size();
    std::vector<uint32_t> tiles(world, 0u);
    for (uint32_t v = 0; v < t.V && v < kMaxVirtual; ++v) {
        if (owner[v] >= kMaxWorld) continue;
        t.owner[v] = (uint8_t)owner[v];
        t.j[v] = (uint8_t)t.w[owner[v]]++;
        tiles[owner[v]] += tiles_of_virtual(n_tiles, t.V, v);
    }
    for (uint32_t q = 0; q < world; ++q) {
        offsets[q + 1] = offsets[q] + tiles[q] * area;
        if (q < kMaxWorld) t.offset[q + 1] = offsets[q + 1];
    }
    return t;
}

static void shard_geometry(const lpt_renderer *r, uint32_t &tiles_x, uint32_t &n_tiles, uint32_t &n_slots) {
    tiles_x = div_up(r->w, r->tile_w);
    const uint32_t tiles_y = div_up(r->h, r->tile_h);
    n_tiles = tiles_x * tiles_y;
    n_slots = owned_tiles(r->map, n_tiles) * r->tile_w * r->tile_h;
}

static int alloc_ray_buffers(Wavefront &wf, size_t rays) {
    free_ray_buffers(wf);
    const size_t n = std::max<size_t>(rays, 64);
    if (n > 0x7FFFFFFFull) return fail(LPT_ERR_INVALID_ARG, "a wavefront of %zu rays exceeds 2^31", n);
    for (int k = 0; k < 2; ++k) {
        HIP_TRY(hipMalloc(&wf.q[k].o, sizeof(float4) * n));
        HIP_TRY(hipMalloc(&wf.q[k].d, sizeof(float4) * n));
        HIP_TRY(hipMalloc(&wf.q[k].T, sizeof(float4) * n));
    }
    HIP_TRY(hipMalloc(&wf.sq.o, sizeof(float4) * n));
    HIP_TRY(hipMalloc(&wf.sq.d, sizeof(float4) * n));
    HIP_TRY(hipMalloc(&wf.sq.c, sizeof(float4) * n));
    HIP_TRY(hipMalloc(&wf.hits, sizeof(float4) * n));
    HIP_TRY(hipMalloc(&wf.Lsum, sizeof(float4) * n));
    HIP_TRY(hipMalloc(&wf.strag, sizeof(uint32_t) * 2 * n));
    wf.ray_cap = n;
    return LPT_OK;
}

static int ensure_lane(lpt_renderer *r, int l) {
    Wavefront &wf = r->wf[l];
    if (!wf.stream) HIP_TRY(hipStreamCreateWithFlags(&wf.stream, hipStreamNonBlocking));
    if (!wf.done) HIP_TRY(hipEventCreateWithFlags(&wf.done, hipEventDisableTiming));
    if (!wf.consumed) HIP_TRY(hipEventCreateWithFlags(&wf.consumed, hipEventDisableTiming));
    if (!wf.ctr) HIP_TRY(hipMalloc(&wf.ctr, sizeof(FrameCounters)));
    return LPT_OK;
}

static int alloc_frame_buffers(lpt_renderer *r) {
    HIP_TRY(hipSetDevice(r->dev->ordinal));
    HIP_TRY(hipStreamSynchronize(r->stream));
    free_frame_buffers(r);
    if (!r->w || !r->h) return LPT_OK;
    uint32_t tiles_x, n_tiles, n_slots;
    shard_geometry(r, tiles_x, n_tiles, n_slots);
    const size_t px = (size_t)r->w * r->h;
    r->n_slots = n_slots;
    if (r->rank == 0u) {
        r->h_table = make_shard_table(r->weights, r->world, n_tiles, r->tile_w * r->tile_h, r->h_offset);
        if (!r->d_table) HIP_TRY(hipMalloc(&r->d_table, sizeof(ShardTable)));
        HIP_TRY(hipMemcpy(r->d_table, &r->h_table, sizeof(ShardTable), hipMemcpyHostToDevice));
    }
    HIP_TRY(hipMalloc(&r->accum, sizeof(float4) * px));
    HIP_TRY(hipMalloc(&r->scratch, sizeof(float4) * px));
    HIP_TRY(hipMemsetAsync(r->accum, 0, sizeof(float4) * px, r->stream));
    return LPT_OK;
}

int lpt_renderer_create(lpt_device *dev, uint32_t width, uint32_t height, lpt_renderer **out) {
    if (!dev || !out) return fail(LPT_ERR_INVALID_ARG, "lpt_renderer_create: null");
    HIP_TRY(hipSetDevice(dev->ordinal));
    lpt_renderer *r = new lpt_renderer();
    r->dev = dev;
    {
        hipError_t se = hipStreamCreateWithFlags(&r->stream, hipStreamNonBlocking);
        if (se != hipSuccess) { delete r; return fail(LPT_ERR_HIP, "hipStreamCreate failed: %s", hipGetErrorString(se)); }
    }
    r->prev_cam.origin = mk3(0.f, 0.f, 0.f); r->prev_cam.right = mk3(1.f, 0.f, 0.f); r->prev_cam.up = mk3(0.f, 1.f, 0.f);
    r->prev_cam.fwd = mk3(0.f, 0.f, 1.f); r->prev_cam.ax = r->prev_cam.ay = 1.0f;
    r->req_w = width; r->req_h = height;
    r->w = (uint32_t)((float)width * r->downsample);
    r->h = (uint32_t)((float)height * r->downsample);
    hipError_t e = hipMalloc(&r->totals, sizeof(Totals));
    if (e == hipSuccess) e = hipMemset(r->totals, 0, sizeof(Totals));
    if (e == hipSuccess) e = hipHostMalloc((void **)&r->err_host, sizeof(uint32_t), hipHostMallocMapped);
    if (e == hipSuccess) { *r->err_host = 0u; e = hipHostGetDevicePointer((void **)&r->err_dev, r->err_host, 0); }
    if (e == hipSuccess) e = hipMalloc(&r->default_probe, 4);
    if (e == hipSuccess) e = hipMemset(r->default_probe, 0, 4);
    if (e == hipSuccess) e = hipMalloc(&r->srgb_thr, 256 * sizeof(float));
    if (e == hipSuccess) {
        float thr[256];
        thr[0] = 0.0f;
        for (int i = 1; i < 256; ++i) {
            const double v = ((double)i - 0.5) / 255.0;
            thr[i] = (float)(v <= 0.04045 ? v / 12.92 : pow((v + 0.055) / 1.055, 2.4));
        }
        e = hipMemcpy(r->srgb_thr, thr, sizeof thr, hipMemcpyHostToDevice);
    }
    if (e != hipSuccess) {
        const int st = fail(LPT_ERR_HIP, "renderer allocation failed: %s", hipGetErrorString(e));
        lpt_renderer_destroy(r);
        return st;
    }
    int st = alloc_frame_buffers(r);
    if (st != LPT_OK) { lpt_renderer_destroy(r); return st; }
    dev->renderers.push_back(r);
    *out = r;
    return LPT_OK;
}

int lpt_renderer_destroy(lpt_renderer *r) {
    if (!r) return LPT_OK;
    hipSetDevice(r->dev->ordinal);
    r->pend.n = 0;
    forget_deferred_exchange(r);
    {
        auto &v = r->dev->renderers;
        v.erase(std::remove(v.begin(), v.end(), r), v.end());
    }
    hipStreamSynchronize(r->stream);
    for (int l = 0; l < kMaxLanes; ++l)
        if (r->wf[l].stream) hipStreamSynchronize(r->wf[l].stream);
    free_frame_buffers(r);
    for (int l = 0; l < kMaxLanes; ++l) {
        Wavefront &wf = r->wf[l];
        if (wf.stream) hipStreamDestroy(wf.stream);
        if (wf.done) hipEventDestroy(wf.done);
        if (wf.consumed) hipEventDestroy(wf.consumed);
        if (wf.ctr) hipFree(wf.ctr);
    }
    if (r->totals) hipFree(r->totals);
    if (r->err_host) hipHostFree(r->err_host);
    if (r->occ_table) hipFree(r->occ_table);
    if (r->d_table) hipFree(r->d_table);
    if (r->default_probe) hipFree(r->default_probe);
    if (r->srgb_thr) hipFree(r->srgb_thr);
    if (r->xevent) hipEventDestroy(r->xevent);
    if (r->stream) hipStreamDestroy(r->stream);
    if (r->noise) hipFree(r->noise);
    if (r->ev_start) {
        for (int i = 0; i < lpt_renderer::kRing * lpt_renderer::kMaxEvents; ++i) {
            if (r->ev_start[i]) hipEventDestroy(r->ev_start[i]);
            if (r->ev_stop[i]) hipEventDestroy(r->ev_stop[i]);
        }
        delete[] r->ev_start;
        delete[] r->ev_stop;
    }
    delete r;
    return LPT_OK;
}

int lpt_renderer_set_downsample(lpt_renderer *r, float factor) {
    if (!r || !(factor > 0.f) || factor > 16.f) return fail(LPT_ERR_INVALID_ARG, "lpt_renderer_set_downsample: factor must be in (0,16]");
    FLUSH_OR_RETURN(r);
    r->downsample = factor;
    return LPT_OK;
}

int lpt_renderer_set_resources(lpt_renderer *r, const lpt_scene_gpu *sg, const lpt_probe *probe) {
    if (!r || !sg) return fail(LPT_ERR_INVALID_ARG, "lpt_renderer_set_resources: null");
    if (sg->dev != r->dev || (probe && probe->dev != r->dev)) return fail(LPT_ERR_INVALID_ARG, "resources belong to another device");
    FLUSH_OR_RETURN(r);
    r->sg = sg;
    r->probe = probe;
    r->resources_set = true;
    r->frame_count = 1;
    return LPT_OK;
}

int lpt_renderer_resize(lpt_renderer *r, const lpt_scene_gpu *sg, const lpt_probe *probe, uint32_t width, uint32_t height) {
    if (!r || !sg) return fail(LPT_ERR_INVALID_ARG, "lpt_renderer_resize: null");
    FLUSH_OR_RETURN(r);
    const uint32_t nw = (uint32_t)((float)width * r->downsample), nh = (uint32_t)((float)height * r->downsample);
    if (nw > 8192u || nh > 8192u) return fail(LPT_ERR_INVALID_ARG, "lpt_renderer_resize: the path-traced size is limited to 8192 x 8192 (got %u x %u)", nw, nh);
    r->req_w = width; r->req_h = height;
    r->w = nw;
    r->h = nh;
    int st = alloc_frame_buffers(r);
    if (st != LPT_OK) return st;
    return lpt_renderer_set_resources(r, sg, probe);
}

int lpt_renderer_get_size(const lpt_renderer *r, uint32_t *w, uint32_t *h) {
    if (!r) return fail(LPT_ERR_INVALID_ARG, "lpt_renderer_get_size: null");
    if (w) *w = r->w;
    if (h) *h = r->h;
    return LPT_OK;
}

uint32_t lpt_max_per_pixel_bytes(void) { return 48u; }

int lpt_renderer_set_max_bounces(lpt_renderer *r, uint32_t b) {
    if (!r || b == 0 || b > (uint32_t)kMaxBounces) return fail(LPT_ERR_INVALID_ARG, "max_bounces must be in [1,%d]", kMaxBounces);
    FLUSH_OR_RETURN(r);
    r->max_bounces = b;
    return LPT_OK;
}
int lpt_renderer_set_seed(lpt_renderer *r, uint32_t s) {
    if (!r) return fail(LPT_ERR_INVALID_ARG, "lpt_renderer_set_seed: null");
    FLUSH_OR_RETURN(r);
    r->user_seed = s;
    return LPT_OK;
}
int lpt_renderer_set_vfov(lpt_renderer *r, float radians) {
    if (!r || !(radians > 0.f) || !(radians < 3.14159f)) return fail(LPT_ERR_INVALID_ARG, "vfov must be in (0, pi)");
    FLUSH_OR_RETURN(r);
    r->vfov = radians;
    return LPT_OK;
}
int lpt_renderer_set_shard_weighted(lpt_renderer *r, uint32_t rank, uint32_t world, uint32_t tile_w, uint32_t tile_h, const uint32_t *weights) {
    if (!r || world == 0 || rank >= world || tile_w == 0 || tile_h == 0 || (tile_w * tile_h) % 64u != 0u)
        return fail(LPT_ERR_INVALID_ARG, "bad shard (rank %u of %u, tile %ux%u; tile area must be a multiple of 64)", rank, world, tile_w, tile_h);
    std::vector<uint32_t> wv;
    if (weights) {
        if (world > kMaxWorld) return fail(LPT_ERR_INVALID_ARG, "weighted shards: at most %u ranks", kMaxWorld);
        uint32_t sum = 0;
        bool unit = true;
        for (uint32_t q = 0; q < world; ++q) {
            if (weights[q] > kMaxWeight) return fail(LPT_ERR_INVALID_ARG, "weighted shards: weight %u of rank %u exceeds %u", weights[q], q, kMaxWeight);
            sum += weights[q];
            unit = unit && weights[q] == 1u;
        }
        if (sum == 0u || sum > kMaxVirtual) return fail(LPT_ERR_INVALID_ARG, "weighted shards: the weights must sum to 1..%u (got %u)", kMaxVirtual, sum);
        if (!unit) wv.assign(weights, weights + world);
    }
    FLUSH_OR_RETURN(r);
    r->rank = rank; r->world = world; r->tile_w = tile_w; r->tile_h = tile_h;
    r->weights = wv;
    r->map = make_shard_map(r->weights, rank, world);
    r->frame_count = 1;
    return alloc_frame_buffers(r);
}
int lpt_renderer_set_shard(lpt_renderer *r, uint32_t rank, uint32_t world, uint32_t tile_w, uint32_t tile_h) {
    return lpt_renderer_set_shard_weighted(r, rank, world, tile_w, tile_h, nullptr);
}
int lpt_renderer_reset_accumulation(lpt_renderer *r) {
    if (!r) return fail(LPT_ERR_INVALID_ARG, "lpt_renderer_reset_accumulation: null");
    r->frame_count = 1;
    r->accumulate = false;
    return LPT_OK;
}
int lpt_renderer_set_accumulate(lpt_renderer *r, int a) {
    if (!r) return fail(LPT_ERR_INVALID_ARG, "lpt_renderer_set_accumulate: null");
    r->accumulate = a != 0;
    return LPT_OK;
}
int lpt_renderer_get_accumulate(const lpt_renderer *r, int *a) {
    if (!r || !a) return fail(LPT_ERR_INVALID_ARG, "lpt_renderer_get_accumulate: null");
    *a = r->accumulate ? 1 : 0;
    return LPT_OK;
}
int lpt_renderer_get_frame_state(const lpt_renderer *r, uint32_t *fc, uint32_t *seed) {
    if (!r) return fail(LPT_ERR_INVALID_ARG, "lpt_renderer_get_frame_state: null");
    if (fc) *fc = r->frame_count;
    if (seed) *seed = r->seed;
    return LPT_OK;
}
int lpt_renderer_upload_noise(lpt_renderer *r, const uint8_t *rgba8, uint32_t w, uint32_t h, uint32_t row_bytes) {
    if (!r || !rgba8 || !w || !h || row_bytes < w * 4u) return fail(LPT_ERR_INVALID_ARG, "lpt_renderer_upload_noise: bad arguments");
    FLUSH_OR_RETURN(r);
    HIP_TRY(hipSetDevice(r->dev->ordinal));
    HIP_TRY(hipStreamSynchronize(r->stream));
    if (r->noise) { hipFree(r->noise); r->noise = nullptr; }
    HIP_TRY(hipMalloc(&r->noise, (size_t)w * h * 4));
    HIP_TRY(hipMemcpy2D(r->noise, (size_t)w * 4, rgba8, row_bytes, (size_t)w * 4, h, hipMemcpyHostToDevice));
    r->noise_w = w; r->noise_h = h;
    return LPT_OK;
}
int lpt_renderer_use_noise(lpt_renderer *r, int flag) {
    if (!r) return fail(LPT_ERR_INVALID_ARG, "lpt_renderer_use_noise: null");
    FLUSH_OR_RETURN(r);
    r->use_noise = flag != 0;
    return LPT_OK;
}
int lpt_renderer_set_blit_mode(lpt_renderer *r, int mode) {
    if (!r || mode < LPT_BLIT_PATHTRACE || mode > LPT_BLIT_MOTION) return fail(LPT_ERR_INVALID_ARG, "lpt_renderer_set_blit_mode: bad mode %d", mode);
    FLUSH_OR_RETURN(r);
    r->mode = mode;
    return LPT_OK;
}
int lpt_renderer_set_lanes(lpt_renderer *r, int lanes) {
    if (!r || lanes < 1 || lanes > kMaxLanes) return fail(LPT_ERR_INVALID_ARG, "lpt_renderer_set_lanes: 1..%d", kMaxLanes);
    FLUSH_OR_RETURN(r);
    HIP_TRY(hipSetDevice(r->dev->ordinal));
    HIP_TRY(hipStreamSynchronize(r->stream));
    for (int l = 0; l < kMaxLanes; ++l) {
        if (r->wf[l].stream) HIP_TRY(hipStreamSynchronize(r->wf[l].stream));
        r->wf[l].consumed_recorded = false;
        if (l >= lanes) free_ray_buffers(r->wf[l]);
    }
    r->n_lanes = lanes;
    r->lane_rr = 0;
    return LPT_OK;
}
int lpt_renderer_set_sort_queues(lpt_renderer *r, int flag) {
    if (!r) return fail(LPT_ERR_INVALID_ARG, "lpt_renderer_set_sort_queues: null");
    FLUSH_OR_RETURN(r);
    r->sort_queues = flag ? ((flag & 3) ? (flag & 3) : 3) : 0;
    return LPT_OK;
}
int lpt_renderer_set_option(lpt_renderer *r, int option, uint64_t value) {
    if (!r) return fail(LPT_ERR_INVALID_ARG, "lpt_renderer_set_option: null");
    FLUSH_OR_RETURN(r);
    switch (option) {
    case LPT_OPT_PACKET_PRIMARY: if (value > 2u) return fail(LPT_ERR_INVALID_ARG, "LPT_OPT_PACKET_PRIMARY: 0 (never), 1 (always), 2 (by pixel footprint)"); r->packet_primary = (uint32_t)value; break;
    case LPT_OPT_EXPERIMENT(LPT_EXP_PIPE_RAYS): r->pipe_rays = (uint32_t)std::min<uint64_t>(value, 0x7FFFFFFFu); break;
    case LPT_OPT_WAVEFRONT_RAYS: r->wavefront_rays = std::max<uint64_t>(value, 64u); break;
    case LPT_OPT_EXPERIMENT(LPT_EXP_REFILL): if (value > 63u) return fail(LPT_ERR_INVALID_ARG, "LPT_EXP_REFILL: 0..63"); r->refill = (int)value; break;
    case LPT_OPT_EXPERIMENT(LPT_EXP_TRACE_WAVES_PER_CU): if (value > 32u) return fail(LPT_ERR_INVALID_ARG, "LPT_EXP_TRACE_WAVES_PER_CU: 0 (auto) or 1..32"); r->trace_waves_per_cu = (uint32_t)value; break;
    case LPT_OPT_EXPERIMENT(LPT_EXP_SHADE_BLOCKS_PER_CU): if (value > 64u) return fail(LPT_ERR_INVALID_ARG, "LPT_EXP_SHADE_BLOCKS_PER_CU: 0 (by the submission) or 1..64"); r->shade_blocks_per_cu = (uint32_t)value; break;
    case LPT_OPT_PATH_RAYS: r->path_rays = (uint32_t)std::min<uint64_t>(value, 0x7FFFFFFFu); break;
    case LPT_OPT_EXPERIMENT(LPT_EXP_PATH_WAVES_PER_CU): if (value < 1u || value > 32u) return fail(LPT_ERR_INVALID_ARG, "LPT_EXP_PATH_WAVES_PER_CU: 1..32"); r->path_waves_per_cu = (uint32_t)value; break;
    case LPT_OPT_EXPERIMENT(LPT_EXP_PATH_REFILL): if (value > 63u) return fail(LPT_ERR_INVALID_ARG, "LPT_EXP_PATH_REFILL: 0..63"); r->path_refill = (int)value; break;
    case LPT_OPT_EXPERIMENT(LPT_EXP_OCC_CELL_MILLI): r->occ_cell = (float)std::min<uint64_t>(value, 1000000u) * 1.0e-3f; break;
    case LPT_OPT_EXPERIMENT(LPT_EXP_STEP_BUDGET): r->step_budget = (uint32_t)std::min<uint64_t>(value, 1u << 20); break;
    case LPT_OPT_EXPERIMENT(LPT_EXP_BUDGET_RAYS): r->budget_rays = (uint32_t)std::min<uint64_t>(value, 0x7FFFFFFFu); break;
    case LPT_OPT_EXPERIMENT(LPT_EXP_PACKET_QUADS): r->packet_quads = value != 0; break;
    case LPT_OPT_EXPERIMENT(LPT_EXP_SPLIT_RAYS): r->split_rays = value; break;
    case LPT_OPT_EXPERIMENT(LPT_EXP_BUDGET_SPLIT): r->budget_split = value != 0; break;
    case LPT_OPT_TAIL_LANES: r->tail_lanes = (uint32_t)std::min<uint64_t>(value, kTailMax); break;
    case LPT_OPT_COOP_RAYS: r->coop_rays = (uint32_t)std::min<uint64_t>(value, 0x7FFFFFFFu); break;
    default: return fail(LPT_ERR_INVALID_ARG, "lpt_renderer_set_option: unknown option %d", option);
    }
    return LPT_OK;
}
int lpt_renderer_get_option(const lpt_renderer *r, int option, uint64_t *value) {
    if (!r || !value) return fail(LPT_ERR_INVALID_ARG, "lpt_renderer_get_option: null");
    switch (option) {
    case LPT_OPT_PACKET_PRIMARY: *value = r->packet_primary; break;
    case LPT_OPT_EXPERIMENT(LPT_EXP_PIPE_RAYS): *value = r->pipe_rays; break;
    case LPT_OPT_WAVEFRONT_RAYS: *value = r->wavefront_rays; break;
    case LPT_OPT_EXPERIMENT(LPT_EXP_REFILL): *value = (uint64_t)r->refill; break;
    case LPT_OPT_EXPERIMENT(LPT_EXP_TRACE_WAVES_PER_CU): *value = r->trace_waves_per_cu; break;
    case LPT_OPT_EXPERIMENT(LPT_EXP_SHADE_BLOCKS_PER_CU): *value = r->shade_blocks_per_cu; break;
    case LPT_OPT_PATH_RAYS: *value = r->path_rays; break;
    case LPT_OPT_EXPERIMENT(LPT_EXP_PATH_WAVES_PER_CU): *value = r->path_waves_per_cu; break;
    case LPT_OPT_EXPERIMENT(LPT_EXP_PATH_REFILL): *value = (uint64_t)r->path_refill; break;
    case LPT_OPT_EXPERIMENT(LPT_EXP_OCC_CELL_MILLI): *value = (uint64_t)(r->occ_cell * 1000.0f + 0.5f); break;
    case LPT_OPT_EXPERIMENT(LPT_EXP_STEP_BUDGET): *value = r->step_budget; break;
    case LPT_OPT_EXPERIMENT(LPT_EXP_BUDGET_RAYS): *value = r->budget_rays; break;
    case LPT_OPT_EXPERIMENT(LPT_EXP_PACKET_QUADS): *value = r->packet_quads; break;
    case LPT_OPT_EXPERIMENT(LPT_EXP_SPLIT_RAYS): *value = r->split_rays; break;
    case LPT_OPT_EXPERIMENT(LPT_EXP_BUDGET_SPLIT): *value = r->budget_split; break;
    case LPT_OPT_TAIL_LANES: *value = r->tail_lanes; break;
    case LPT_OPT_COOP_RAYS: *value = r->coop_rays; break;
    default: return fail(LPT_ERR_INVALID_ARG, "lpt_renderer_get_option: unknown option %d", option);
    }
    return LPT_OK;
}
int lpt_renderer_enable_stats(lpt_renderer *r, int flag) {
    if (!r) return fail(LPT_ERR_INVALID_ARG, "lpt_renderer_enable_stats: null");
    FLUSH_OR_RETURN(r);
    r->stats = flag != 0;
    if (flag) {
        HIP_TRY(hipSetDevice(r->dev->ordinal));
        if (!r->occ_table) HIP_TRY(hipMalloc(&r->occ_table, sizeof(uint32_t) * kOccEntries));
        HIP_TRY(hipMemsetAsync(r->occ_table, 0, sizeof(uint32_t) * kOccEntries, r->stream));
        HIP_TRY(hipStreamSynchronize(r->stream));
    }
    return LPT_OK;
}
int lpt_renderer_enable_timings(lpt_renderer *r, int flag) {
    if (!r) return fail(LPT_ERR_INVALID_ARG, "lpt_renderer_enable_timings: null");
    FLUSH_OR_RETURN(r);
    HIP_TRY(hipSetDevice(r->dev->ordinal));
    const int total = lpt_renderer::kRing * lpt_renderer::kMaxEvents;
    if (flag && !r->ev_start) {
        r->ev_start = new hipEvent_t[total]();
        r->ev_stop = new hipEvent_t[total]();
    }
    if (flag) {
        for (int i = 0; i < total; ++i) {
            if (!r->ev_start[i]) HIP_TRY(hipEventCreate(&r->ev_start[i]));
            if (!r->ev_stop[i]) HIP_TRY(hipEventCreate(&r->ev_stop[i]));
        }
    }
    if (flag) {
        HIP_TRY(hipStreamSynchronize(r->stream));
        for (int k = 0; k < lpt_renderer::kRing; ++k) r->ev_count[k] = 0;
        for (int i = 0; i < ST_COUNT; ++i) { r->stage_ms[i] = 0.0; r->stage_launches[i] = 0; }
    }
    r->timings = flag != 0;
    return LPT_OK;
}

static void harvest_slot(lpt_renderer *r, int slot) {
    const int n = r->ev_count[slot];
    for (int i = 0; i < n; ++i) {
        const int e = slot * lpt_renderer::kMaxEvents + i;
        float ms = 0.f;
        hipEventSynchronize(r->ev_stop[e]);
        if (hipEventElapsedTime(&ms, r->ev_start[e], r->ev_stop[e]) == hipSuccess) {
            r->stage_ms[r->ev_stage[slot][i]] += ms;
            r->stage_launches[r->ev_stage[slot][i]]++;
        }
    }
    r->ev_count[slot] = 0;
}
static inline int cur_slot(const lpt_renderer *r) { return (int)(r->ring_pos % lpt_renderer::kRing); }
static inline void stage_begin(lpt_renderer *r, int stage, hipStream_t stream) {
    if (!r->timings) return;
    const int slot = cur_slot(r);
    if (r->ev_count[slot] >= lpt_renderer::kMaxEvents) return;
    r->ev_stage[slot][r->ev_count[slot]] = stage;
    hipEventRecord(r->ev_start[slot * lpt_renderer::kMaxEvents + r->ev_count[slot]], stream);
}
static inline void stage_end(lpt_renderer *r, hipStream_t stream) {
    if (!r->timings) return;
    const int slot = cur_slot(r);
    if (r->ev_count[slot] >= lpt_renderer::kMaxEvents) return;
    hipEventRecord(r->ev_stop[slot * lpt_renderer::kMaxEvents + r->ev_count[slot]], stream);
    r->ev_count[slot]++;
}

}

static void launch_filter(lpt_renderer *r, hipStream_t s) {
    if (r->mode != LPT_BLIT_DENOISED && r->mode != LPT_BLIT_TEMPORAL) return;
    const int cur = r->den_cur, prv = 1 - r->den_cur;
    const uint32_t npx = r->w * r->h;
    const uint32_t px_blocks = div_up(npx, kBlock);
    const uint32_t stream_blocks = std::min<uint32_t>(px_blocks, (uint32_t)r->dev->compute_units * 8u);
    hipLaunchKernelGGL(k_temporal, dim3(stream_blocks), dim3(kBlock), 0, s, (int)r->w, (int)r->h, r->den_noisy, r->den_gbuf[cur], r->den_gbuf[prv], r->den_motion,
                       r->den_rad[prv], r->den_mom[prv], r->den_hist[prv], r->den_rad[cur], r->den_mom[cur], r->den_hist[cur]);
    const float4 *result = r->den_rad[cur];
    if (r->mode == LPT_BLIT_DENOISED) {
        hipMemcpyAsync(r->den_temp, r->den_rad[cur], sizeof(float4) * npx, hipMemcpyDeviceToDevice, s);
        hipLaunchKernelGGL(k_decode_gbuf, dim3(px_blocks), dim3(kBlock), 0, s, r->den_gbuf[cur], r->den_nd, npx);
        hipLaunchKernelGGL(k_atrous, dim3(px_blocks), dim3(kBlock), 0, s, r->den_nd, r->den_temp, r->accum, (int)r->w, (int)r->h, 1);
        hipLaunchKernelGGL(k_atrous, dim3(px_blocks), dim3(kBlock), 0, s, r->den_nd, r->accum, r->den_temp, (int)r->w, (int)r->h, 2);
        hipLaunchKernelGGL(k_atrous, dim3(px_blocks), dim3(kBlock), 0, s, r->den_nd, r->den_temp, r->accum, (int)r->w, (int)r->h, 4);
        hipLaunchKernelGGL(k_atrous, dim3(px_blocks), dim3(kBlock), 0, s, r->den_nd, r->accum, r->den_temp, (int)r->w, (int)r->h, 8);
        result = r->den_temp;
    }
    hipLaunchKernelGGL(k_composite, dim3(px_blocks), dim3(kBlock), 0, s, r->den_gbuf[cur], result, r->accum, npx);
}

extern "C" {

struct Ticket {
    FrameParams p;
    int lane = 0;
    bool split = false, denoise = false, packet = false;
    CamBasis cur{};
};

static int wavefront_trace(lpt_renderer *r, const float view[16], uint32_t n_samples, uint32_t frame_count0, uint32_t seed0, bool acc0,
                           uint32_t slot0, uint32_t piece_slots, Ticket &tk, bool solo) {
    HIP_TRY(hipSetDevice(r->dev->ordinal));
    hipStream_t sm = r->stream;
    const uint32_t nb = r->max_bounces;

    FrameParams p;
    p.right = mk3(view[0], view[1], view[2]);
    p.up = mk3(view[4], view[5], view[6]);
    p.fwd = mk3(view[8], view[9], view[10]);
    p.origin = mk3(view[12], view[13], view[14]);
    const float th = tanf(0.5f * r->vfov);
    const float aspect = (float)r->w / (float)r->h;
    p.ax = aspect * th; p.ay = th;
    p.width = r->w; p.height = r->h;
    p.user_seed = r->user_seed;
    p.seed_counter = seed0;
    p.rank = r->rank; p.world = r->world; p.tile_w = r->tile_w; p.tile_h = r->tile_h;
    p.map = r->map;
    shard_geometry(r, p.tiles_x, p.n_tiles, p.n_slots);
    p.slot0 = slot0;
    p.block8 = (r->tile_w % 8u == 0u && r->tile_h % 8u == 0u) ? 1u : 0u;
    p.n_slots = piece_slots;
    p.frame_count = frame_count0;
    p.max_bounces = nb;
    p.n_samples = n_samples;
    p.fc_inc0 = acc0 ? 1u : 0u;
    const uint32_t n_rays = p.n_slots * n_samples;
    const bool denoise = r->mode != LPT_BLIT_PATHTRACE;
    const bool split = r->n_lanes > 1;
    const int lane = (denoise || !split) ? 0 : (int)(r->lane_rr++ % (uint32_t)r->n_lanes);
    {
        int st = ensure_lane(r, lane);
        if (st != LPT_OK) return st;
    }
    Wavefront &wf = r->wf[lane];
    hipStream_t s = split ? wf.stream : sm;
    r->last_lane = lane;
    if ((size_t)n_rays > wf.ray_cap && p.n_slots) {
        HIP_TRY(hipStreamSynchronize(sm));
        HIP_TRY(hipStreamSynchronize(s));
        int st = alloc_ray_buffers(wf, n_rays);
        if (st != LPT_OK) return st;
        for (int l = 0; split && !denoise && l < r->n_lanes; ++l) {
            if (l == lane || r->wf[l].ray_cap >= (size_t)n_rays) continue;
            st = ensure_lane(r, l);
            if (st != LPT_OK) return st;
            HIP_TRY(hipStreamSynchronize(r->wf[l].stream));
            st = alloc_ray_buffers(r->wf[l], n_rays);
            if (st != LPT_OK) return st;
        }
    }
    GBufArgs gb{};
    if (denoise) {
        int st = ensure_denoiser(r);
        if (st != LPT_OK) return st;
    }
    if (split && denoise) { HIP_TRY(hipEventRecord(wf.consumed, sm)); wf.consumed_recorded = true; }
    if (split && wf.consumed_recorded) HIP_TRY(hipStreamWaitEvent(s, wf.consumed, 0));
    if (denoise) {
        r->den_cur = 1 - r->den_cur;
        if (r->world != 1u) {
            const size_t npx = (size_t)r->w * r->h;
            HIP_TRY(hipMemsetAsync(r->den_gbuf[r->den_cur], 0, sizeof(uint4) * npx, s));
            HIP_TRY(hipMemsetAsync(r->den_motion, 0, sizeof(float2) * npx, s));
            HIP_TRY(hipMemsetAsync(r->den_noisy, 0, sizeof(float4) * npx, sm));
        }
        gb.gbuf = r->den_gbuf[r->den_cur];
        gb.motion = r->den_motion;
        gb.cur.origin = p.origin; gb.cur.right = p.right; gb.cur.up = p.up; gb.cur.fwd = p.fwd; gb.cur.ax = p.ax; gb.cur.ay = p.ay;
        gb.prev = r->prev_cam;
    }

    DProbe probe = r->probe ? r->probe->d : DProbe{(const uint8_t *)r->default_probe, 1u, 1u};
    DNoise nz{(const uint8_t *)r->noise, r->noise_w, r->noise_h, (r->use_noise && r->noise) ? 1u : 0u};
    const DScene &sc = r->sg->d;
    if (r->timings) { r->ring_pos++; harvest_slot(r, cur_slot(r)); }

    if (p.n_slots) {
        HIP_TRY(hipMemsetAsync(wf.ctr, 0, sizeof(FrameCounters), s));
        const uint32_t cus = (uint32_t)r->dev->compute_units;
        const uint32_t stream_blocks = std::min<uint32_t>(div_up(n_rays, kBlock), cus * 8u);
        const uint32_t shade_blocks = std::min<uint32_t>(div_up(n_rays, kBlock), cus * (r->shade_blocks_per_cu ? r->shade_blocks_per_cu : (solo ? 4u : 3u)));
        const bool pipe = n_rays <= r->pipe_rays;
        uint32_t waves = r->trace_waves_per_cu ? cus * r->trace_waves_per_cu : std::min(std::max(n_rays / 160u, cus * 8u), cus * (pipe ? 24u : 32u));
        waves = std::max(8u, waves & ~7u);
        const uint32_t trace_blocks = std::min<uint32_t>(div_up(n_rays, kTraceBlock), waves);
        const size_t lds = stack_bytes(sc);

        stage_begin(r, ST_RAYGEN, s);
        const bool dense = (r->w % r->tile_w == 0u) && (r->h % r->tile_h == 0u);
        if (dense) {
            hipLaunchKernelGGL(k_raygen<true>, dim3(stream_blocks), dim3(kBlock), 0, s, p, nz, wf.q[0], wf.Lsum, wf.ctr);
        } else {
            hipLaunchKernelGGL(k_raygen<false>, dim3(stream_blocks), dim3(kBlock), 0, s, p, nz, wf.q[0], wf.Lsum, wf.ctr);
        }
        stage_end(r, s);

        const float pixel_rad = 2.0f * th / (float)std::max(r->h, 1u);
        const bool packet = (r->packet_primary == 1u || (r->packet_primary == 2u && pixel_rad <= kPacketMaxPixelRad));
        tk.packet = packet;
        uint32_t seed = seed0;
        OccProbe occ{nullptr, 0u, 0.0f};
        if (r->stats && r->occ_table && r->occ_cell > 0.0f) occ = OccProbe{r->occ_table, kOccEntries - 1u, 1.0f / r->occ_cell};
        const bool tail_launch = !r->stats && (solo || r->budget_split) && n_rays <= r->budget_rays;
        const uint32_t tail = tail_launch ? std::min(std::min(r->tail_lanes, kTailMax), (uint32_t)std::max(r->refill, 0)) : 0u;
        const uint32_t budget = (tail_launch && !tail && r->step_budget) ? r->step_budget : 0u;
        const size_t tail_lds = tail ? sizeof(uint32_t) * tail_lds_words(r->sg->stats.max_depth) : 0u;
        const bool coop_all = !r->stats && r->coop_rays && n_rays <= r->coop_rays;
        auto trace = [&](int cb, int sb) {
            stage_begin(r, cb >= 0 ? ST_INTERSECT : ST_SHADOW, s);
            const Queue qin = wf.q[(uint32_t)(cb < 0 ? 0 : cb) & 1u];
            const int launch_no = cb >= 0 ? cb : (int)nb;
            if (coop_all) {
                const size_t clds = sizeof(uint32_t) * coop_stack_entries(kCoopStack, r->sg->stats.max_depth);
                hipLaunchKernelGGL(k_trace_coop<false>, dim3(std::min(2u * n_rays, cus * kCoopWavesPerCu)), dim3(kTraceBlock), clds, s, sc, qin, wf.hits, wf.sq, wf.Lsum, wf.ctr, cb, sb, (const uint32_t *)nullptr, launch_no);
                stage_end(r, s);
                return;
            }
            if (tail) {
                if (pipe) hipLaunchKernelGGL((k_trace<false, true, true>), dim3(trace_blocks), dim3(kTraceBlock), lds + tail_lds, s, TraceKernargs{sc, qin, wf.hits, wf.sq, wf.Lsum, wf.ctr, cb, sb, r->refill, occ, 0u, wf.strag, launch_no, tail});
                else hipLaunchKernelGGL((k_trace<false, false, true>), dim3(trace_blocks), dim3(kTraceBlock), lds + tail_lds, s, TraceKernargs{sc, qin, wf.hits, wf.sq, wf.Lsum, wf.ctr, cb, sb, r->refill, occ, 0u, wf.strag, launch_no, tail});
            } else if (pipe) {
                if (r->stats) hipLaunchKernelGGL((k_trace<true, true>), dim3(trace_blocks), dim3(kTraceBlock), lds + 64u, s, TraceKernargs{sc, qin, wf.hits, wf.sq, wf.Lsum, wf.ctr, cb, sb, r->refill, occ, budget, wf.strag, launch_no, 0u});
                else hipLaunchKernelGGL((k_trace<false, true>), dim3(trace_blocks), dim3(kTraceBlock), lds, s, TraceKernargs{sc, qin, wf.hits, wf.sq, wf.Lsum, wf.ctr, cb, sb, r->refill, occ, budget, wf.strag, launch_no, 0u});
            } else if (r->stats) hipLaunchKernelGGL((k_trace<true, false>), dim3(trace_blocks), dim3(kTraceBlock), lds + 64u, s, TraceKernargs{sc, qin, wf.hits, wf.sq, wf.Lsum, wf.ctr, cb, sb, r->refill, occ, budget, wf.strag, launch_no, 0u});
            else hipLaunchKernelGGL((k_trace<false, false>), dim3(trace_blocks), dim3(kTraceBlock), lds, s, TraceKernargs{sc, qin, wf.hits, wf.sq, wf.Lsum, wf.ctr, cb, sb, r->refill, occ, budget, wf.strag, launch_no, 0u});
            if (budget) {
                const size_t clds = sizeof(uint32_t) * coop_stack_entries(kCoopStack, r->sg->stats.max_depth);
                if (r->stats) hipLaunchKernelGGL(k_trace_coop<true>, dim3(cus * kCoopWavesPerCu), dim3(kTraceBlock), clds, s, sc, qin, wf.hits, wf.sq, wf.Lsum, wf.ctr, cb, sb, wf.strag, launch_no);
                else hipLaunchKernelGGL(k_trace_coop<false>, dim3(cus * kCoopWavesPerCu), dim3(kTraceBlock), clds, s, sc, qin, wf.hits, wf.sq, wf.Lsum, wf.ctr, cb, sb, wf.strag, launch_no);
            }
            stage_end(r, s);
        };
        {
            if (packet) {
                stage_begin(r, ST_PRIMARY, s);
                const uint32_t packets = div_up(n_rays, 64u);
                const size_t plds = (size_t)(48u + 7u * r->sg->stats.max_depth + 8u) * sizeof(uint32_t);
                const uint32_t quad_slots = (r->packet_quads && dense && p.block8 && p.n_slots % 64u == 0u && p.slot0 % 64u == 0u && n_samples % 4u == 0u) ? p.n_slots : 0u;
                if (r->stats) hipLaunchKernelGGL(k_trace_packet<true>, dim3(std::min(packets, cus * kPacketBlocksPerCu)), dim3(kTraceBlock), plds, s, sc, wf.q[0], wf.hits, wf.ctr, 0, quad_slots);
                else hipLaunchKernelGGL(k_trace_packet<false>, dim3(std::min(packets, cus * kPacketBlocksPerCu)), dim3(kTraceBlock), plds, s, sc, wf.q[0], wf.hits, wf.ctr, 0, quad_slots);
                stage_end(r, s);
            } else if (coop_all || !(r->path_rays && n_rays <= r->path_rays)) trace(0, -1);
        }
        const bool path = r->path_rays && n_rays <= r->path_rays && !coop_all;
        if (path) {
            stage_begin(r, ST_PATH, s);
            const uint32_t pblocks = std::min<uint32_t>(div_up(n_rays, kTraceBlock), std::max(8u, (cus * r->path_waves_per_cu) & ~7u));
            const size_t plds = lds + kPathLdsExtra;
            if (denoise) {
                if (r->stats) hipLaunchKernelGGL((k_path<true, true>), dim3(pblocks), dim3(kTraceBlock), plds, s, sc, probe, nz, p, wf.q[0], packet ? wf.hits : (const float4 *)nullptr, wf.Lsum, wf.ctr, seed0, gb, r->path_refill);
                else hipLaunchKernelGGL((k_path<true, false>), dim3(pblocks), dim3(kTraceBlock), plds, s, sc, probe, nz, p, wf.q[0], packet ? wf.hits : (const float4 *)nullptr, wf.Lsum, wf.ctr, seed0, gb, r->path_refill);
            } else if (r->stats) hipLaunchKernelGGL((k_path<false, true>), dim3(pblocks), dim3(kTraceBlock), plds, s, sc, probe, nz, p, wf.q[0], packet ? wf.hits : (const float4 *)nullptr, wf.Lsum, wf.ctr, seed0, gb, r->path_refill);
            else hipLaunchKernelGGL((k_path<false, false>), dim3(pblocks), dim3(kTraceBlock), plds, s, sc, probe, nz, p, wf.q[0], packet ? wf.hits : (const float4 *)nullptr, wf.Lsum, wf.ctr, seed0, gb, r->path_refill);
            stage_end(r, s);
        }
        for (uint32_t b = 0; b < nb && !path; ++b) {
            seed += 1u;
            const Queue qin = wf.q[b & 1u], qout = wf.q[(b + 1u) & 1u];
            stage_begin(r, ST_SHADE, s);
            if (denoise && b == 0u)
                hipLaunchKernelGGL(k_shade<true>, dim3(shade_blocks), dim3(kBlock), 0, s, sc, probe, nz, p, qin, wf.hits, qout, wf.sq, wf.Lsum, wf.ctr, (int)b, seed, gb, r->sort_queues);
            else
                hipLaunchKernelGGL(k_shade<false>, dim3(shade_blocks), dim3(kBlock), 0, s, sc, probe, nz, p, qin, wf.hits, qout, wf.sq, wf.Lsum, wf.ctr, (int)b, seed, gb, r->sort_queues);
            stage_end(r, s);
            trace(b + 1u < nb ? (int)(b + 1u) : -1, (int)b);
        }
        if (split) HIP_TRY(hipEventRecord(wf.done, s));
        HIP_TRY(hipGetLastError());
    }
    tk.p = p; tk.lane = lane; tk.split = split; tk.denoise = denoise; tk.cur = gb.cur;
    return LPT_OK;
}

static int wavefront_finish(lpt_renderer *r, const Ticket &tk, const ReadPlan *read, uint32_t row0, uint32_t row1) {
    hipStream_t sm = r->stream;
    const FrameParams &p = tk.p;
    Wavefront &wf = r->wf[tk.lane];
    const bool split = tk.split;
    const uint32_t nb = p.max_bounces;
    if (p.n_slots) {
        const uint32_t stream_blocks = std::min<uint32_t>(div_up(p.n_slots * p.n_samples, kBlock), (uint32_t)r->dev->compute_units * 8u);
        if (split) HIP_TRY(hipStreamWaitEvent(sm, wf.done, 0));
        if (r->mode == LPT_BLIT_PATHTRACE) {
            stage_begin(r, ST_ACCUM, sm);
            hipLaunchKernelGGL(k_accumulate, dim3(stream_blocks), dim3(kBlock), 0, sm, p, wf.Lsum, r->accum);
            stage_end(r, sm);
            if (read && row1 > row0) {
                const size_t off = (size_t)row0 * r->w, cnt = (size_t)(row1 - row0) * r->w;
                if (read->radiance) {
                    hipLaunchKernelGGL(k_resolve, dim3(div_up((uint32_t)cnt, kBlock)), dim3(kBlock), 0, sm, r->accum + off, r->scratch + off, (uint32_t)cnt);
                    HIP_TRY(hipMemcpyAsync(read->radiance + 4u * off, r->scratch + off, sizeof(float4) * cnt, hipMemcpyDeviceToHost, sm));
                } else {
                    uchar4 *px = reinterpret_cast<uchar4 *>(r->scratch) + off;
                    hipLaunchKernelGGL(k_tonemap, dim3(div_up((uint32_t)cnt, kBlock)), dim3(kBlock), 0, sm, r->accum + off, px, (uint32_t)cnt, r->srgb_thr);
                    HIP_TRY(hipMemcpy2DAsync(read->rgba8 + (size_t)row0 * read->row_bytes, read->row_bytes, px, (size_t)r->w * 4, (size_t)r->w * 4, row1 - row0, hipMemcpyDeviceToHost, sm));
                }
            }
        } else {
            stage_begin(r, ST_ASVGF, sm);
            hipLaunchKernelGGL(k_den_scatter, dim3(stream_blocks), dim3(kBlock), 0, sm, p, wf.Lsum, r->den_noisy);
            r->den_inputs_ready = true;
            if (r->world == 1u) launch_filter(r, sm);
            stage_end(r, sm);
        }
        hipLaunchKernelGGL(k_finish_frame, dim3(1), dim3(64), 0, sm, wf.ctr, r->totals, nb, tk.packet ? 1u : 0u);
        if (split) {
            HIP_TRY(hipEventRecord(wf.consumed, sm));
            wf.consumed_recorded = true;
        }
        HIP_TRY(hipGetLastError());
    } else if (r->mode != LPT_BLIT_PATHTRACE) {
        r->den_inputs_ready = true;
    }
    if (tk.denoise) r->prev_cam = tk.cur;
    return LPT_OK;
}

static int flush_pending(lpt_renderer *r, const ReadPlan *read) {
    if (!r->pend.n) return LPT_OK;
    const lpt_renderer::Pending b = r->pend;
    r->pend.n = 0;
    uint32_t tiles_x, n_tiles, n_slots;
    shard_geometry(r, tiles_x, n_tiles, n_slots);
    const uint32_t area = r->tile_w * r->tile_h;
    const bool whole_rows = r->world == 1u;
    const uint32_t granule = whole_rows ? tiles_x * area : area;
    const uint32_t granules = granule ? n_slots / granule : 0u;
    uint32_t per_piece = granules;
    const uint64_t total = (uint64_t)n_slots * b.n;
    if (!r->max_fused && r->mode == LPT_BLIT_PATHTRACE && granules > 1u && (total > r->wavefront_rays || (r->split_rays && total > r->split_rays && r->n_lanes > 1))) {
        const uint64_t fit = r->wavefront_rays / ((uint64_t)granule * b.n);
        const uint32_t pieces = std::max(2u, div_up(granules, (uint32_t)std::max<uint64_t>(fit, 1u)));
        per_piece = div_up(granules, pieces);
    }
    Ticket tk[kMaxLanes];
    if (!granules) {
        r->n_wavefronts++;
        const int st = wavefront_trace(r, b.view, b.n, b.frame_count0, b.seed0, b.acc0, 0u, 0u, tk[0], true);
        return st != LPT_OK ? st : wavefront_finish(r, tk[0], nullptr, 0u, 0u);
    }
    const bool early = read && whole_rows && r->mode == LPT_BLIT_PATHTRACE;
    const uint32_t ahead = (r->mode != LPT_BLIT_PATHTRACE || r->n_lanes < 2) ? 1u : (uint32_t)r->n_lanes;
    const uint32_t pieces = div_up(granules, per_piece);
    auto finish = [&](uint32_t k) {
        const uint32_t g0 = k * per_piece, g1 = std::min(granules, g0 + per_piece);
        return wavefront_finish(r, tk[k % ahead], early ? read : nullptr, std::min(r->h, g0 * r->tile_h), std::min(r->h, g1 * r->tile_h));
    };
    auto bail = [&](int st) {
        for (int l = 0; l < kMaxLanes; ++l) {
            if (r->wf[l].stream) hipStreamSynchronize(r->wf[l].stream);
            r->wf[l].consumed_recorded = false;
        }
        hipStreamSynchronize(r->stream);
        return st;
    };
    for (uint32_t k = 0; k < pieces; ++k) {
        if (k >= ahead) { const int st = finish(k - ahead); if (st != LPT_OK) return bail(st); }
        const uint32_t g0 = k * per_piece, g1 = std::min(granules, g0 + per_piece);
        r->n_wavefronts++;
        const int st = wavefront_trace(r, b.view, b.n, b.frame_count0, b.seed0, b.acc0, g0 * granule, (g1 - g0) * granule, tk[k % ahead], pieces == 1u);
        if (st != LPT_OK) return bail(st);
    }
    for (uint32_t k = pieces > ahead ? pieces - ahead : 0u; k < pieces; ++k) { const int st = finish(k); if (st != LPT_OK) return bail(st); }
    return LPT_OK;
}

static uint32_t fuse_cap(const lpt_renderer *r) { return r->max_fused ? r->max_fused : 64u; }

static int record_call(lpt_renderer *r, const float view[16]) {
    r->frame_back = !r->frame_back;
    if (!r->resources_set || !r->sg) return LPT_OK;
    if (!r->w || !r->h) return LPT_OK;
    r->presented = false;
    lpt_renderer::Pending &b = r->pend;
    const bool pathtrace = r->mode == LPT_BLIT_PATHTRACE;
    if (b.n) {
        const uint32_t expect_fc = b.frame_count0 + (b.acc0 ? 1u : 0u) + (b.n - 1u);
        const bool fuses = pathtrace && r->accumulate && r->frame_count == expect_fc && b.n < fuse_cap(r) && memcmp(view, b.view, sizeof b.view) == 0;
        if (!fuses) FLUSH_OR_RETURN(r);
    }
    if (!b.n) {
        memcpy(b.view, view, sizeof b.view);
        b.frame_count0 = r->frame_count; b.seed0 = r->seed; b.acc0 = r->accumulate;
    }
    b.n++;
    r->n_recorded++;
    r->seed += r->max_bounces;
    if (pathtrace && r->accumulate) r->frame_count += 1u;
    if (!pathtrace || b.n >= fuse_cap(r)) return flush_pending(r);
    return LPT_OK;
}

int lpt_renderer_raytrace(lpt_renderer *r, const float view[16]) {
    if (!r || !view) return fail(LPT_ERR_INVALID_ARG, "lpt_renderer_raytrace: null");
    return record_call(r, view);
}

int lpt_renderer_submit(lpt_renderer *r) {
    if (!r) return fail(LPT_ERR_INVALID_ARG, "lpt_renderer_submit: null");
    return flush_pending(r);
}

int lpt_renderer_get_submission_stats(const lpt_renderer *r, uint64_t *recorded_calls, uint64_t *wavefronts, uint32_t *pending_calls) {
    if (!r) return fail(LPT_ERR_INVALID_ARG, "lpt_renderer_get_submission_stats: null");
    if (recorded_calls) *recorded_calls = r->n_recorded;
    if (wavefronts) *wavefronts = r->n_wavefronts;
    if (pending_calls) *pending_calls = r->pend.n;
    return LPT_OK;
}

int lpt_renderer_set_max_fused(lpt_renderer *r, uint32_t n) {
    if (!r || n > 64u) return fail(LPT_ERR_INVALID_ARG, "lpt_renderer_set_max_fused: 0 (auto) or 1..64");
    FLUSH_OR_RETURN(r);
    r->max_fused = n;
    return LPT_OK;
}

int lpt_renderer_raytrace_n(lpt_renderer *r, const float view[16], uint32_t n_samples) {
    if (!r || !view) return fail(LPT_ERR_INVALID_ARG, "lpt_renderer_raytrace: null");
    if (n_samples == 0u || n_samples > 64u) return fail(LPT_ERR_INVALID_ARG, "lpt_renderer_raytrace_n: n must be in [1,64]");
    const uint32_t keep = r->max_fused;
    if (r->mode == LPT_BLIT_PATHTRACE) r->max_fused = std::min(64u, std::max(fuse_cap(r), n_samples + r->pend.n));
    int st = LPT_OK;
    for (uint32_t k = 0; k < n_samples && st == LPT_OK; ++k) {
        st = record_call(r, view);
        if (n_samples > 1u) r->accumulate = true;
    }
    if (st == LPT_OK) st = flush_pending(r);
    r->max_fused = keep;
    return st;
}

int lpt_renderer_stream(lpt_renderer *r, void **stream) {
    if (!r || !stream) return fail(LPT_ERR_INVALID_ARG, "lpt_renderer_stream: null");
    FLUSH_OR_RETURN(r);
    *stream = (void *)r->stream;
    return LPT_OK;
}

int lpt_renderer_synchronize(lpt_renderer *r) {
    if (!r) return fail(LPT_ERR_INVALID_ARG, "lpt_renderer_synchronize: null");
    FLUSH_OR_RETURN(r);
    HIP_TRY(hipSetDevice(r->dev->ordinal));
    HIP_TRY(hipStreamSynchronize(r->stream));
    return check_device_error(r);
}

int lpt_renderer_radiance_device_ptr(lpt_renderer *r, void **ptr, size_t *bytes) {
    if (!r || !ptr) return fail(LPT_ERR_INVALID_ARG, "lpt_renderer_radiance_device_ptr: null");
    FLUSH_OR_RETURN(r);
    *ptr = r->accum;
    if (bytes) *bytes = sizeof(float4) * (size_t)r->w * r->h;
    return LPT_OK;
}

int lpt_renderer_read_radiance(lpt_renderer *r, float *dst) {
    if (!r || !dst) return fail(LPT_ERR_INVALID_ARG, "lpt_renderer_read_radiance: null");
    if (r->pend.n && r->accum && r->world == 1u && r->mode == LPT_BLIT_PATHTRACE) {
        ReadPlan plan;
        plan.radiance = dst;
        const int st = flush_pending(r, &plan);
        if (st != LPT_OK) return st;
        const hipError_t se = hipStreamSynchronize(r->stream);
        if (se != hipSuccess) return fail(LPT_ERR_READBACK, "failed to read pixels from GPU to CPU: %s", hipGetErrorString(se));
        return check_device_error(r);
    }
    FLUSH_OR_RETURN(r);
    if (!r->accum) return fail(LPT_ERR_READBACK, "failed to read pixels from GPU to CPU: no render target");
    hipError_t e = hipSetDevice(r->dev->ordinal);
    const uint32_t n = r->w * r->h;
    if (e == hipSuccess) { hipLaunchKernelGGL(k_resolve, dim3(div_up(n, kBlock)), dim3(kBlock), 0, r->stream, presented_target(r), r->scratch, n); e = hipGetLastError(); }
    if (e == hipSuccess) e = hipMemcpyAsync(dst, r->scratch, sizeof(float4) * (size_t)n, hipMemcpyDeviceToHost, r->stream);
    if (e == hipSuccess) e = hipStreamSynchronize(r->stream);
    if (e != hipSuccess) return fail(LPT_ERR_READBACK, "failed to read pixels from GPU to CPU: %s", hipGetErrorString(e));
    return check_device_error(r);
}

int lpt_renderer_read_radiance_owned(lpt_renderer *r, float *frame_dst) {
    if (!r || !frame_dst) return fail(LPT_ERR_INVALID_ARG, "lpt_renderer_read_radiance_owned: null");
    FLUSH_OR_RETURN(r);
    if (!r->accum) return fail(LPT_ERR_READBACK, "failed to read pixels from GPU to CPU: no render target");
    if (r->mode != LPT_BLIT_PATHTRACE) return fail(LPT_ERR_INVALID_ARG, "lpt_renderer_read_radiance_owned: BlitMode::Pathtrace only (the denoising modes filter the whole frame on rank 0)");
    HIP_TRY(hipSetDevice(r->dev->ordinal));
    void *mapped = nullptr;
    if (hipHostGetDevicePointer(&mapped, frame_dst, 0) != hipSuccess || !mapped) {
        (void)hipGetLastError();
        return fail(LPT_ERR_INVALID_ARG, "lpt_renderer_read_radiance_owned: the destination must be page-locked host memory (lpt_host_alloc / lpt_host_register)");
    }
    const FrameParams p = shard_params(r);
    if (p.n_slots) hipLaunchKernelGGL(k_resolve_owned, dim3(stream_grid(r, p.n_slots)), dim3(kBlock), 0, r->stream, p, r->accum, reinterpret_cast<float4 *>(mapped));
    hipError_t e = hipGetLastError();
    if (e == hipSuccess) e = hipStreamSynchronize(r->stream);
    if (e != hipSuccess) return fail(LPT_ERR_READBACK, "failed to read pixels from GPU to CPU: %s", hipGetErrorString(e));
    return check_device_error(r);
}

int lpt_host_register(void *ptr, size_t bytes) {
    if (!ptr || !bytes) return fail(LPT_ERR_INVALID_ARG, "lpt_host_register: null");
    HIP_TRY(hipHostRegister(ptr, bytes, hipHostRegisterMapped | hipHostRegisterPortable));
    return LPT_OK;
}
int lpt_host_unregister(void *ptr) {
    if (!ptr) return LPT_OK;
    HIP_TRY(hipHostUnregister(ptr));
    return LPT_OK;
}

int lpt_host_alloc(size_t bytes, void **out) {
    if (!out || !bytes) return fail(LPT_ERR_INVALID_ARG, "lpt_host_alloc: null / zero size");
    HIP_TRY(hipHostMalloc(out, bytes, hipHostMallocDefault));
    return LPT_OK;
}
int lpt_host_free(void *ptr) {
    if (ptr) HIP_TRY(hipHostFree(ptr));
    return LPT_OK;
}

int lpt_renderer_blit_rgba8(lpt_renderer *r, uint8_t *dst, size_t row_bytes) {
    if (!r || !dst || row_bytes < (size_t)r->w * 4) return fail(LPT_ERR_INVALID_ARG, "lpt_renderer_blit_rgba8: bad arguments");
    if (r->pend.n && r->accum && r->world == 1u && r->mode == LPT_BLIT_PATHTRACE) {
        ReadPlan plan;
        plan.rgba8 = dst; plan.row_bytes = row_bytes;
        const int st = flush_pending(r, &plan);
        if (st != LPT_OK) return st;
        const hipError_t se = hipStreamSynchronize(r->stream);
        if (se != hipSuccess) return fail(LPT_ERR_READBACK, "failed to read pixels from GPU to CPU: %s", hipGetErrorString(se));
        return check_device_error(r);
    }
    FLUSH_OR_RETURN(r);
    if (!r->accum) return fail(LPT_ERR_READBACK, "failed to read pixels from GPU to CPU: no render target");
    hipError_t e = hipSetDevice(r->dev->ordinal);
    const uint32_t n = r->w * r->h;
    if (e == hipSuccess) {
        if ((r->mode == LPT_BLIT_GBUFFER || r->mode == LPT_BLIT_MOTION) && r->den_temp)
            hipLaunchKernelGGL(k_debug_view, dim3(div_up(n, kBlock)), dim3(kBlock), 0, r->stream, r->den_gbuf[r->den_cur], r->den_motion,
                               (uchar4 *)r->scratch, (int)r->w, (int)r->h, r->mode);
        else
            hipLaunchKernelGGL(k_tonemap, dim3(div_up(n, kBlock)), dim3(kBlock), 0, r->stream, presented_target(r), (uchar4 *)r->scratch, n, r->srgb_thr);
        e = hipGetLastError();
    }
    if (e == hipSuccess) e = hipMemcpy2DAsync(dst, row_bytes, r->scratch, (size_t)r->w * 4, (size_t)r->w * 4, r->h, hipMemcpyDeviceToHost, r->stream);
    if (e == hipSuccess) e = hipStreamSynchronize(r->stream);
    if (e != hipSuccess) return fail(LPT_ERR_READBACK, "failed to read pixels from GPU to CPU: %s", hipGetErrorString(e));
    return check_device_error(r);
}

int lpt_renderer_read_pixels(lpt_renderer *r, uint8_t *dst) {
    if (!r || !dst) return fail(LPT_ERR_INVALID_ARG, "lpt_renderer_read_pixels: null");
    const int mode = r->mode;
    if (mode == LPT_BLIT_GBUFFER || mode == LPT_BLIT_MOTION) r->mode = LPT_BLIT_PATHTRACE;
    const int st = lpt_renderer_blit_rgba8(r, dst, (size_t)r->w * 4);
    r->mode = mode;
    return st;
}

int lpt_renderer_read_denoiser(lpt_renderer *r, uint32_t *gbuffer, float *motion, float *radiance, uint32_t *history) {
    if (!r) return fail(LPT_ERR_INVALID_ARG, "lpt_renderer_read_denoiser: null");
    FLUSH_OR_RETURN(r);
    if (!r->den_temp) return fail(LPT_ERR_READBACK, "failed to read pixels from GPU to CPU: no denoising frame has been traced");
    HIP_TRY(hipSetDevice(r->dev->ordinal));
    HIP_TRY(hipStreamSynchronize(r->stream));
    const size_t n = (size_t)r->w * r->h;
    const int c = r->den_cur;
    if (gbuffer) HIP_TRY(hipMemcpy(gbuffer, r->den_gbuf[c], sizeof(uint4) * n, hipMemcpyDeviceToHost));
    if (motion) HIP_TRY(hipMemcpy(motion, r->den_motion, sizeof(float2) * n, hipMemcpyDeviceToHost));
    if (radiance) HIP_TRY(hipMemcpy(radiance, r->den_rad[c], sizeof(float4) * n, hipMemcpyDeviceToHost));
    if (history) HIP_TRY(hipMemcpy(history, r->den_hist[c], sizeof(uint32_t) * n, hipMemcpyDeviceToHost));
    return LPT_OK;
}

int lpt_renderer_denoiser_inputs(lpt_renderer *r, void **noisy, void **gbuffer, void **motion, size_t *n_pixels) {
    if (!r) return fail(LPT_ERR_INVALID_ARG, "lpt_renderer_denoiser_inputs: null");
    FLUSH_OR_RETURN(r);
    if (!r->den_temp) return fail(LPT_ERR_INVALID_ARG, "lpt_renderer_denoiser_inputs: no denoising frame has been traced");
    if (noisy) *noisy = r->den_noisy;
    if (gbuffer) *gbuffer = r->den_gbuf[r->den_cur];
    if (motion) *motion = r->den_motion;
    if (n_pixels) *n_pixels = (size_t)r->w * r->h;
    return LPT_OK;
}

int lpt_renderer_denoise_filter(lpt_renderer *r) {
    if (!r) return fail(LPT_ERR_INVALID_ARG, "lpt_renderer_denoise_filter: null");
    FLUSH_OR_RETURN(r);
    if (!r->den_temp || !r->den_inputs_ready) return fail(LPT_ERR_INVALID_ARG, "lpt_renderer_denoise_filter: no denoising frame has been traced");
    if (r->world == 1u) return LPT_OK;
    HIP_TRY(hipSetDevice(r->dev->ordinal));
    launch_filter(r, r->stream);
    HIP_TRY(hipGetLastError());
    r->den_inputs_ready = false;
    return LPT_OK;
}

int lpt_renderer_get_ray_counts(lpt_renderer *r, lpt_ray_counts *out) {
    if (!r || !out) return fail(LPT_ERR_INVALID_ARG, "lpt_renderer_get_ray_counts: null");
    FLUSH_OR_RETURN(r);
    HIP_TRY(hipSetDevice(r->dev->ordinal));
    Totals t;
    HIP_TRY(hipMemcpyAsync(&t, r->totals, sizeof t, hipMemcpyDeviceToHost, r->stream));
    HIP_TRY(hipStreamSynchronize(r->stream));
    out->closest = t.closest; out->shadow = t.shadow; out->shaded = t.shaded; out->nodes = t.nodes; out->tris = t.tris;
    out->shadow_nodes = t.shadow_nodes; out->shadow_tris = t.shadow_tris;
    out->wave_steps = t.wave_steps; out->live_lanes = t.live_lanes; out->node_lanes = t.node_lanes; out->tri_lanes = t.tri_lanes;
    out->primary = t.primary; out->packet_nodes = t.packet_nodes; out->packet_tris = t.packet_tris;
    out->shadow_occluded = t.shadow_occluded; out->occluder_cache_found = t.occ_found; out->occluder_cache_hits = t.occ_hits; out->wave_rays = t.wave_rays;
    return check_device_error(r);
}

int lpt_renderer_reset_ray_counts(lpt_renderer *r) {
    if (!r) return fail(LPT_ERR_INVALID_ARG, "lpt_renderer_reset_ray_counts: null");
    FLUSH_OR_RETURN(r);
    HIP_TRY(hipSetDevice(r->dev->ordinal));
    HIP_TRY(hipMemsetAsync(r->totals, 0, sizeof(Totals), r->stream));
    return LPT_OK;
}

int lpt_renderer_get_timings(lpt_renderer *r, lpt_timing *out, int *inout_count) {
    if (!r || !inout_count) return fail(LPT_ERR_INVALID_ARG, "lpt_renderer_get_timings: null");
    FLUSH_OR_RETURN(r);
    HIP_TRY(hipSetDevice(r->dev->ordinal));
    HIP_TRY(hipStreamSynchronize(r->stream));
    lpt_timing acc[ST_COUNT];
    if (r->ev_start) for (int k = 0; k < lpt_renderer::kRing; ++k) harvest_slot(r, k);
    for (int i = 0; i < ST_COUNT; ++i) {
        memset(&acc[i], 0, sizeof acc[i]);
        snprintf(acc[i].label, sizeof acc[i].label, "%s", kStageLabel[i]);
        acc[i].ms = (float)r->stage_ms[i];
        acc[i].launches = r->stage_launches[i];
    }
    const int n = std::min(*inout_count, (int)ST_COUNT);
    if (out) for (int i = 0; i < n; ++i) out[i] = acc[i];
    *inout_count = ST_COUNT;
    return LPT_OK;
}

int lpt_renderer_get_queue_counts(lpt_renderer *r, uint32_t *closest, uint32_t *shadow, uint32_t cap) {
    if (!r) return fail(LPT_ERR_INVALID_ARG, "lpt_renderer_get_queue_counts: null");
    FLUSH_OR_RETURN(r);
    HIP_TRY(hipSetDevice(r->dev->ordinal));
    const uint32_t n = std::min<uint32_t>(cap, (uint32_t)kMaxBounces);
    HIP_TRY(hipStreamSynchronize(r->stream));
    const FrameCounters *ctr = r->wf[r->last_lane].ctr;
    if (!ctr) { if (closest) memset(closest, 0, sizeof(uint32_t) * n); if (shadow) memset(shadow, 0, sizeof(uint32_t) * n); return LPT_OK; }
    uint32_t host[2 + 2 * kMaxBounces];
    HIP_TRY(hipMemcpy(host, &ctr->q0, sizeof host, hipMemcpyDeviceToHost));
    for (uint32_t b = 0; b < n; ++b) {
        if (closest) closest[b] = b == 0u ? host[0] : host[2u + 2u * (b - 1u) + 1u];
        if (shadow) shadow[b] = host[2u + 2u * b];
    }
    return LPT_OK;
}

int lpt_renderer_get_step_histogram(lpt_renderer *r, uint32_t *max_steps, uint32_t *hist12) {
    if (!r) return fail(LPT_ERR_INVALID_ARG, "lpt_renderer_get_step_histogram: null");
    FLUSH_OR_RETURN(r);
    HIP_TRY(hipSetDevice(r->dev->ordinal));
    HIP_TRY(hipStreamSynchronize(r->stream));
    const FrameCounters *ctr = r->wf[r->last_lane].ctr;
    if (max_steps) *max_steps = 0;
    if (hist12) memset(hist12, 0, sizeof(uint32_t) * 12);
    if (!ctr) return LPT_OK;
    if (max_steps) HIP_TRY(hipMemcpy(max_steps, &ctr->max_steps, sizeof(uint32_t), hipMemcpyDeviceToHost));
    if (hist12) HIP_TRY(hipMemcpy(hist12, ctr->step_hist, sizeof(uint32_t) * 12, hipMemcpyDeviceToHost));
    return LPT_OK;
}

int lpt_comm_unique_id(void *out_id) {
    if (!out_id) return fail(LPT_ERR_INVALID_ARG, "lpt_comm_unique_id: null");
    static_assert(sizeof(ncclUniqueId) == LPT_COMM_ID_BYTES, "LPT_COMM_ID_BYTES must match ncclUniqueId");
    const Rccl *nc = rccl();
    if (!nc) return LPT_ERR_RCCL;
    ncclUniqueId id;
    RCCL_TRY(nc->GetUniqueId(&id));
    memcpy(out_id, &id, sizeof id);
    return LPT_OK;
}

int lpt_comm_create(lpt_device *dev, const void *id_bytes, int rank, int world, lpt_comm **out) {
    if (!dev || !id_bytes || !out) return fail(LPT_ERR_INVALID_ARG, "lpt_comm_create: null");
    if (world < 1 || rank < 0 || rank >= world) return fail(LPT_ERR_INVALID_ARG, "lpt_comm_create: rank %d of %d", rank, world);
    const Rccl *nc = rccl();
    if (!nc) return LPT_ERR_RCCL;
    HIP_TRY(hipSetDevice(dev->ordinal));
    ncclUniqueId id;
    memcpy(&id, id_bytes, sizeof id);
    lpt_comm *c = new (std::nothrow) lpt_comm();
    if (!c) return fail(LPT_ERR_INVALID_ARG, "out of host memory");
    c->dev = dev; c->rank = rank; c->world = world;
    ncclResult_t st = nc->CommInitRank(&c->comm, world, id, rank);
    if (st != ncclSuccess) { delete c; return fail(LPT_ERR_RCCL, "ncclCommInitRank(rank %d of %d) failed: %s", rank, world, nc->GetErrorString(st)); }
    *out = c;
    return LPT_OK;
}

int lpt_comm_destroy(lpt_comm *c) {
    if (!c) return LPT_OK;
    hipSetDevice(c->dev->ordinal);
    flush_device(c->dev);
    for (lpt_renderer *r : c->dev->renderers)
        if (r->comm == c) { forget_deferred_exchange(r); hipStreamSynchronize(r->stream); r->comm = nullptr; }
    if (c->comm && rccl()) rccl()->CommDestroy(c->comm);
    delete c;
    return LPT_OK;
}

int lpt_comm_info(const lpt_comm *c, int *rank, int *world) {
    if (!c) return fail(LPT_ERR_INVALID_ARG, "lpt_comm_info: null");
    const Rccl *nc = rccl();
    if (!nc) return LPT_ERR_RCCL;
    int rk = -1, n = -1;
    if (c->comm) {
        RCCL_TRY(nc->CommUserRank(c->comm, &rk));
        RCCL_TRY(nc->CommCount(c->comm, &n));
    }
    if (rank) *rank = rk;
    if (world) *world = n;
    return LPT_OK;
}

int lpt_shard_layout_weighted(uint32_t width, uint32_t height, uint32_t tile_w, uint32_t tile_h, uint32_t world, uint32_t rank, const uint32_t *weights,
                              uint32_t *out_slots, uint32_t *out_offset) {
    if (!world || rank >= world || !tile_w || !tile_h) return fail(LPT_ERR_INVALID_ARG, "lpt_shard_layout: bad shard (rank %u of %u, tile %ux%u)", rank, world, tile_w, tile_h);
    const uint32_t n_tiles = div_up(width, tile_w) * div_up(height, tile_h), area = tile_w * tile_h;
    if (!weights) {
        const uint32_t a = shard_slot_offset(n_tiles, world, area, rank), b = shard_slot_offset(n_tiles, world, area, rank + 1u);
        if (out_slots) *out_slots = b - a;
        if (out_offset) *out_offset = a;
        return LPT_OK;
    }
    if (world > kMaxWorld) return fail(LPT_ERR_INVALID_ARG, "weighted shards: at most %u ranks", kMaxWorld);
    uint32_t sum = 0;
    for (uint32_t q = 0; q < world; ++q) { if (weights[q] > kMaxWeight) return fail(LPT_ERR_INVALID_ARG, "weighted shards: weight %u exceeds %u", weights[q], kMaxWeight); sum += weights[q]; }
    if (sum == 0u || sum > kMaxVirtual) return fail(LPT_ERR_INVALID_ARG, "weighted shards: the weights must sum to 1..%u (got %u)", kMaxVirtual, sum);
    std::vector<uint32_t> off;
    make_shard_table(std::vector<uint32_t>(weights, weights + world), world, n_tiles, area, off);
    if (out_slots) *out_slots = off[rank + 1] - off[rank];
    if (out_offset) *out_offset = off[rank];
    return LPT_OK;
}
int lpt_shard_layout(uint32_t width, uint32_t height, uint32_t tile_w, uint32_t tile_h, uint32_t world, uint32_t rank, uint32_t *out_slots, uint32_t *out_offset) {
    return lpt_shard_layout_weighted(width, height, tile_w, tile_h, world, rank, nullptr, out_slots, out_offset);
}
int lpt_shard_owner(uint32_t world, const uint32_t *weights, uint32_t tile, uint32_t *out_rank) {
    if (!world || !out_rank || (weights && world > kMaxWorld)) return fail(LPT_ERR_INVALID_ARG, "lpt_shard_owner: bad arguments");
    std::vector<uint32_t> wv;
    if (weights) {
        uint32_t sum = 0;
        for (uint32_t q = 0; q < world; ++q) { if (weights[q] > kMaxWeight) return fail(LPT_ERR_INVALID_ARG, "weighted shards: weight %u exceeds %u", weights[q], kMaxWeight); sum += weights[q]; }
        if (sum == 0u || sum > kMaxVirtual) return fail(LPT_ERR_INVALID_ARG, "weighted shards: the weights must sum to 1..%u (got %u)", kMaxVirtual, sum);
        wv.assign(weights, weights + world);
    }
    const std::vector<uint32_t> owner = deal_virtual_ranks(wv, world);
    *out_rank = owner[tile % owner.size()];
    return LPT_OK;
}

int lpt_renderer_set_comm_weighted(lpt_renderer *r, lpt_comm *comm, const uint32_t *weights) {
    if (!r) return fail(LPT_ERR_INVALID_ARG, "lpt_renderer_set_comm: null");
    if (comm && comm->dev != r->dev) return fail(LPT_ERR_INVALID_ARG, "lpt_renderer_set_comm: the communicator belongs to another device");
    FLUSH_OR_RETURN(r);
    const int st = comm ? lpt_renderer_set_shard_weighted(r, (uint32_t)comm->rank, (uint32_t)comm->world, 32u, 8u, weights) : lpt_renderer_set_shard(r, 0u, 1u, 32u, 8u);
    if (st == LPT_OK) r->comm = comm;
    return st;
}
int lpt_renderer_set_comm(lpt_renderer *r, lpt_comm *comm) { return lpt_renderer_set_comm_weighted(r, comm, nullptr); }

}

static FrameParams shard_params(const lpt_renderer *r) {
    FrameParams p{};
    p.width = r->w; p.height = r->h;
    p.rank = r->rank; p.world = r->world; p.tile_w = r->tile_w; p.tile_h = r->tile_h;
    p.map = r->map;
    p.block8 = (r->tile_w % 8u == 0u && r->tile_h % 8u == 0u) ? 1u : 0u;
    shard_geometry(r, p.tiles_x, p.n_tiles, p.n_slots);
    return p;
}

static int ensure_exchange_buffers(lpt_renderer *r, bool root, bool want_frame, bool want_stage, size_t bytes_per_slot = 16) {
    const size_t npx = (size_t)r->w * r->h;
    if ((root || want_frame) && !r->frame) HIP_TRY(hipMalloc(&r->frame, sizeof(float4) * std::max<size_t>(npx, 1)));
    if (!r->xevent) HIP_TRY(hipEventCreateWithFlags(&r->xevent, hipEventDisableTiming));
    if (!want_stage) return LPT_OK;
    const FrameParams p = shard_params(r);
    const size_t slots = root ? (size_t)p.n_tiles * p.tile_w * p.tile_h : (size_t)p.n_slots;
    const size_t need = std::max<size_t>((slots * bytes_per_slot + 15) / 16, 1);
    if (r->xstage_elems < need) {
        HIP_TRY(hipStreamSynchronize(r->stream));
        if (r->xstage) hipFree(r->xstage);
        r->xstage = nullptr; r->xstage_elems = 0;
        HIP_TRY(hipMalloc(&r->xstage, sizeof(float4) * need));
        r->xstage_elems = need;
    }
    return LPT_OK;
}
static inline uint32_t stream_grid(const lpt_renderer *r, size_t n) {
    return (uint32_t)std::max<size_t>(1, std::min<size_t>((n + kBlock - 1) / kBlock, (size_t)r->dev->compute_units * 8u));
}

static int exchange_enqueue(lpt_renderer *r, int mode) {
    lpt_comm *c = r->comm;
    hipStream_t s = r->stream;
    const bool root = c->rank == 0;
    const size_t npx = (size_t)r->w * r->h;
    const Rccl &nc = *rccl();
    stage_begin(r, ST_EXCHANGE, s);
    if (r->mode != LPT_BLIT_PATHTRACE) {
        if (mode == LPT_EXCHANGE_REDUCE) {
            RCCL_TRY(nc.Reduce(r->den_noisy, r->den_noisy, 4 * npx, ncclFloat32, ncclSum, 0, c->comm, s));
            RCCL_TRY(nc.Reduce(r->den_gbuf[r->den_cur], r->den_gbuf[r->den_cur], 4 * npx, ncclInt32, ncclSum, 0, c->comm, s));
            RCCL_TRY(nc.Reduce(r->den_motion, r->den_motion, 2 * npx, ncclFloat32, ncclSum, 0, c->comm, s));
            return LPT_OK;
        }
        int st = ensure_exchange_buffers(r, root, false, true, 40);
        if (st != LPT_OK) return st;
        const FrameParams p = shard_params(r);
        unsigned char *stage = reinterpret_cast<unsigned char *>(r->xstage);
        if (p.n_slots) hipLaunchKernelGGL(k_pack_den, dim3(stream_grid(r, p.n_slots)), dim3(kBlock), 0, s, p, r->den_noisy, r->den_gbuf[r->den_cur], r->den_motion, stage);
        HIP_TRY(hipGetLastError());
        if (root) {
            RCCL_TRY(nc.GroupStart());
            for (uint32_t q = 1; q < p.world; ++q) {
                const uint32_t nq = r->h_offset[q + 1] - r->h_offset[q];
                if (!nq) continue;
                ncclResult_t e = nc.Recv(stage + 40u * (size_t)r->h_offset[q], 40u * (size_t)nq, ncclUint8, (int)q, c->comm, s);
                if (e != ncclSuccess) { nc.GroupEnd(); return fail(LPT_ERR_RCCL, "ncclRecv from rank %u failed: %s", q, nc.GetErrorString(e)); }
            }
            RCCL_TRY(nc.GroupEnd());
        } else if (p.n_slots) {
            RCCL_TRY(nc.Send(stage, 40u * (size_t)p.n_slots, ncclUint8, 0, c->comm, s));
        }
        return LPT_OK;
    }
    int st = ensure_exchange_buffers(r, root, mode == LPT_EXCHANGE_REDUCE, mode == LPT_EXCHANGE_GATHER_TILES);
    if (st != LPT_OK) return st;
    const FrameParams p = shard_params(r);
    if (mode == LPT_EXCHANGE_REDUCE) {
        RCCL_TRY(nc.Reduce(r->accum, r->frame, 4 * npx, ncclFloat32, ncclSum, 0, c->comm, s));
        return LPT_OK;
    }
    if (p.n_slots) hipLaunchKernelGGL(k_pack_owned, dim3(stream_grid(r, p.n_slots)), dim3(kBlock), 0, s, p, r->accum, r->xstage);
    HIP_TRY(hipGetLastError());
    if (root) {
        RCCL_TRY(nc.GroupStart());
        for (uint32_t q = 1; q < p.world; ++q) {
            const uint32_t nq = r->h_offset[q + 1] - r->h_offset[q];
            if (!nq) continue;
            ncclResult_t e = nc.Recv(r->xstage + r->h_offset[q], 4 * (size_t)nq, ncclFloat32, (int)q, c->comm, s);
            if (e != ncclSuccess) { nc.GroupEnd(); return fail(LPT_ERR_RCCL, "ncclRecv from rank %u failed: %s", q, nc.GetErrorString(e)); }
        }
        RCCL_TRY(nc.GroupEnd());
    } else if (p.n_slots) {
        RCCL_TRY(nc.Send(r->xstage, 4 * (size_t)p.n_slots, ncclFloat32, 0, c->comm, s));
    }
    return LPT_OK;
}

static int exchange_finish(lpt_renderer *r, int mode) {
    hipStream_t s = r->stream;
    const bool root = r->comm->rank == 0;
    const size_t npx = (size_t)r->w * r->h;
    if (r->mode != LPT_BLIT_PATHTRACE) {
        if (root && mode == LPT_EXCHANGE_GATHER_TILES) {
            const FrameParams p = shard_params(r);
            hipLaunchKernelGGL(k_unpack_den, dim3(stream_grid(r, npx)), dim3(kBlock), 0, s, p, r->d_table, reinterpret_cast<unsigned char *>(r->xstage), r->den_noisy, r->den_gbuf[r->den_cur], r->den_motion);
        }
        if (root && r->world != 1u) launch_filter(r, s);
        stage_end(r, s);
        HIP_TRY(hipGetLastError());
        r->den_inputs_ready = false;
        return LPT_OK;
    }
    if (root && mode == LPT_EXCHANGE_GATHER_TILES) {
        const FrameParams p = shard_params(r);
        hipLaunchKernelGGL(k_unpack_frame, dim3(stream_grid(r, npx)), dim3(kBlock), 0, s, p, r->d_table, r->xstage, r->frame);
    }
    stage_end(r, s);
    HIP_TRY(hipGetLastError());
    r->presented = root;
    return LPT_OK;
}

struct DeferredFinish { lpt_renderer *r; int mode; };
static thread_local int t_group_depth = 0;
static thread_local std::vector<DeferredFinish> t_deferred;
static void forget_deferred_exchange(lpt_renderer *r) {
    t_deferred.erase(std::remove_if(t_deferred.begin(), t_deferred.end(), [r](const DeferredFinish &d) { return d.r == r; }), t_deferred.end());
}

extern "C" {

int lpt_comm_group_begin(void) {
    const Rccl *nc = rccl();
    if (!nc) return LPT_ERR_RCCL;
    RCCL_TRY(nc->GroupStart());
    ++t_group_depth;
    return LPT_OK;
}
int lpt_comm_group_end(void) {
    const Rccl *nc = rccl();
    if (!nc) return LPT_ERR_RCCL;
    if (t_group_depth <= 0) return fail(LPT_ERR_INVALID_ARG, "lpt_comm_group_end without lpt_comm_group_begin");
    const ncclResult_t e = nc->GroupEnd();
    if (--t_group_depth > 0) { if (e != ncclSuccess) return fail(LPT_ERR_RCCL, "ncclGroupEnd failed: %s", nc->GetErrorString(e)); return LPT_OK; }
    std::vector<DeferredFinish> todo;
    todo.swap(t_deferred);
    if (e != ncclSuccess) return fail(LPT_ERR_RCCL, "ncclGroupEnd failed: %s", nc->GetErrorString(e));
    int st = LPT_OK;
    for (const DeferredFinish &d : todo) {
        hipSetDevice(d.r->dev->ordinal);
        const int f = exchange_finish(d.r, d.mode);
        if (st == LPT_OK) st = f;
    }
    return st;
}

int lpt_renderer_exchange(lpt_renderer *r, int mode) {
    if (!r) return fail(LPT_ERR_INVALID_ARG, "lpt_renderer_exchange: null");
    if (mode != LPT_EXCHANGE_GATHER_TILES && mode != LPT_EXCHANGE_REDUCE) return fail(LPT_ERR_INVALID_ARG, "lpt_renderer_exchange: unknown mode %d", mode);
    FLUSH_OR_RETURN(r);
    if (!r->comm) return LPT_OK;
    if (!r->w || !r->h || !r->accum) return LPT_OK;
    lpt_comm *c = r->comm;
    if ((uint32_t)c->rank != r->rank || (uint32_t)c->world != r->world)
        return fail(LPT_ERR_INVALID_ARG, "lpt_renderer_exchange: the renderer's shard (%u of %u) is not the communicator's (%d of %d); call lpt_renderer_set_comm again",
                    r->rank, r->world, c->rank, c->world);
    if (r->mode != LPT_BLIT_PATHTRACE && (!r->den_temp || !r->den_inputs_ready)) return fail(LPT_ERR_INVALID_ARG, "lpt_renderer_exchange: no denoising frame has been traced");
    if (!rccl()) return LPT_ERR_RCCL;
    HIP_TRY(hipSetDevice(r->dev->ordinal));
    if (r->timings) { r->ring_pos++; harvest_slot(r, cur_slot(r)); }
    int st = exchange_enqueue(r, mode);
    if (st != LPT_OK) { stage_end(r, r->stream); return st; }
    if (t_group_depth > 0) {
        t_deferred.push_back(DeferredFinish{r, mode});
        return LPT_OK;
    }
    return exchange_finish(r, mode);
}

int lpt_renderer_exchange_local(lpt_renderer *root, lpt_renderer *const *peers, int n_peers) {
    if (!root || n_peers < 0 || (n_peers && !peers)) return fail(LPT_ERR_INVALID_ARG, "lpt_renderer_exchange_local: null");
    if (root->rank != 0u || root->world != (uint32_t)n_peers + 1u)
        return fail(LPT_ERR_INVALID_ARG, "lpt_renderer_exchange_local: root must be rank 0 of %d (is %u of %u)", n_peers + 1, root->rank, root->world);
    const bool den = root->mode != LPT_BLIT_PATHTRACE;
    FLUSH_OR_RETURN(root);
    for (int i = 0; i < n_peers; ++i) if (peers[i]) FLUSH_OR_RETURN(peers[i]);
    if (!root->w || !root->h || !root->accum) return LPT_OK;
    std::vector<char> seen(root->world, 0);
    seen[0] = 1;
    for (int i = 0; i < n_peers; ++i) {
        const lpt_renderer *q = peers[i];
        if (!q || q->w != root->w || q->h != root->h || q->world != root->world || q->tile_w != root->tile_w || q->tile_h != root->tile_h || q->rank >= root->world || seen[q->rank] ||
            q->weights != root->weights || (q->mode != LPT_BLIT_PATHTRACE) != den)
            return fail(LPT_ERR_INVALID_ARG, "lpt_renderer_exchange_local: peer %d does not complete the shard set of the root", i);
        if (den && (!q->den_temp || !q->den_inputs_ready)) return fail(LPT_ERR_INVALID_ARG, "lpt_renderer_exchange_local: peer %d has not traced a denoising frame", i);
        seen[q->rank] = 1;
    }
    if (den && (!root->den_temp || !root->den_inputs_ready)) return fail(LPT_ERR_INVALID_ARG, "lpt_renderer_exchange_local: no denoising frame has been traced");
    const size_t bps = den ? 40 : 16;
    HIP_TRY(hipSetDevice(root->dev->ordinal));
    int st = ensure_exchange_buffers(root, true, true, true, bps);
    if (st != LPT_OK) return st;
    const FrameParams p0 = shard_params(root);
    unsigned char *stage0 = reinterpret_cast<unsigned char *>(root->xstage);
    if (p0.n_slots) {
        if (den) hipLaunchKernelGGL(k_pack_den, dim3(stream_grid(root, p0.n_slots)), dim3(kBlock), 0, root->stream, p0, root->den_noisy, root->den_gbuf[root->den_cur], root->den_motion, stage0);
        else hipLaunchKernelGGL(k_pack_owned, dim3(stream_grid(root, p0.n_slots)), dim3(kBlock), 0, root->stream, p0, root->accum, root->xstage);
    }
    for (int i = 0; i < n_peers; ++i) {
        lpt_renderer *q = peers[i];
        HIP_TRY(hipSetDevice(q->dev->ordinal));
        st = ensure_exchange_buffers(q, false, false, true, bps);
        if (st != LPT_OK) return st;
        const FrameParams pq = shard_params(q);
        if (root->xevent_recorded) HIP_TRY(hipStreamWaitEvent(q->stream, root->xevent, 0));
        if (pq.n_slots) {
            if (den) hipLaunchKernelGGL(k_pack_den, dim3(stream_grid(q, pq.n_slots)), dim3(kBlock), 0, q->stream, pq, q->den_noisy, q->den_gbuf[q->den_cur], q->den_motion, reinterpret_cast<unsigned char *>(q->xstage));
            else hipLaunchKernelGGL(k_pack_owned, dim3(stream_grid(q, pq.n_slots)), dim3(kBlock), 0, q->stream, pq, q->accum, q->xstage);
            HIP_TRY(hipMemcpyPeerAsync(stage0 + bps * (size_t)root->h_offset[pq.rank], root->dev->ordinal, q->xstage, q->dev->ordinal,
                                       bps * (size_t)pq.n_slots, q->stream));
        }
        if (den) q->den_inputs_ready = false;
        HIP_TRY(hipEventRecord(q->xevent, q->stream));
        HIP_TRY(hipSetDevice(root->dev->ordinal));
        HIP_TRY(hipStreamWaitEvent(root->stream, q->xevent, 0));
    }
    if (den) {
        hipLaunchKernelGGL(k_unpack_den, dim3(stream_grid(root, (size_t)root->w * root->h)), dim3(kBlock), 0, root->stream, p0, root->d_table, stage0, root->den_noisy, root->den_gbuf[root->den_cur], root->den_motion);
        launch_filter(root, root->stream);
        HIP_TRY(hipGetLastError());
        HIP_TRY(hipEventRecord(root->xevent, root->stream));
        root->xevent_recorded = true;
        root->den_inputs_ready = false;
        return LPT_OK;
    }
    hipLaunchKernelGGL(k_unpack_frame, dim3(stream_grid(root, (size_t)root->w * root->h)), dim3(kBlock), 0, root->stream, p0, root->d_table, root->xstage, root->frame);
    HIP_TRY(hipGetLastError());
    HIP_TRY(hipEventRecord(root->xevent, root->stream));
    root->xevent_recorded = true;
    root->presented = true;
    return LPT_OK;
}

}
```

Before: 5424.

## Stagger concurrent wavefront lanes with cross-lane events to phase traversal stages

Restructures the wavefront launch code into a per-stage closure so that the pieces in a group of lanes can be issued interleaved stage by stage. Events between lanes either offset each lane's start (default mode 1) or alternate traversal kernels across lanes (mode 2). The aim is to keep concurrent lanes from contending for the same phase (traversal versus shading) at the same moment. Lane 0 now runs on the main stream instead of its own stream. This adds host-side std::function overhead, extra events and extra cross-stream dependencies.

```diff
diff --git a/bindings/rust/loupiote_hip/src/ffi.rs b/bindings/rust/loupiote_hip/src/ffi.rs
--- a/bindings/rust/loupiote_hip/src/ffi.rs
+++ b/bindings/rust/loupiote_hip/src/ffi.rs
@@ -40,6 +40,7 @@
 pub const LPT_EXP_PACKET_QUADS: c_int = 9;
 pub const LPT_EXP_SPLIT_RAYS: c_int = 10;
 pub const LPT_EXP_BUDGET_SPLIT: c_int = 11;
+pub const LPT_EXP_LANE_PHASE: c_int = 12;
 
 #[repr(C)] pub struct lpt_device { _private: [u8; 0] }
 #[repr(C)] pub struct lpt_scene { _private: [u8; 0] }
diff --git a/include/lpt.h b/include/lpt.h
--- a/include/lpt.h
+++ b/include/lpt.h
@@ -280,7 +280,8 @@
     LPT_EXP_BUDGET_RAYS = 8,
     LPT_EXP_PACKET_QUADS = 9,
     LPT_EXP_SPLIT_RAYS = 10,
-    LPT_EXP_BUDGET_SPLIT = 11
+    LPT_EXP_BUDGET_SPLIT = 11,
+    LPT_EXP_LANE_PHASE = 12
 } lpt_experiment;
 int lpt_renderer_set_option(lpt_renderer *r, int option, uint64_t value);
 int lpt_renderer_get_option(const lpt_renderer *r, int option, uint64_t *value);
diff --git a/loupiote_amd/_abi.py b/loupiote_amd/_abi.py
--- a/loupiote_amd/_abi.py
+++ b/loupiote_amd/_abi.py
@@ -17,7 +17,7 @@
 OPT_EXPERIMENT_BASE = 256
 OPTIONS = {"packet_primary": 1, "wavefront_rays": 2, "path_rays": 3, "coop_rays": 4, "tail_lanes": 5}
 EXPERIMENTS = {"pipe_rays": 0, "refill": 1, "trace_waves_per_cu": 2, "shade_blocks_per_cu": 3, "path_waves_per_cu": 4, "path_refill": 5, "occ_cell_milli": 6,
-               "step_budget": 7, "budget_rays": 8, "packet_quads": 9, "split_rays": 10, "budget_split": 11}
+               "step_budget": 7, "budget_rays": 8, "packet_quads": 9, "split_rays": 10, "budget_split": 11, "lane_phase": 12}
 OPTIONS.update({k: OPT_EXPERIMENT_BASE + v for k, v in EXPERIMENTS.items()})
 EXCHANGE_GATHER_TILES = 0
 HOST_FRAME_HOST_ONLY = 1
diff --git a/loupiote_amd/csrc/device.hip b/loupiote_amd/csrc/device.hip
--- a/loupiote_amd/csrc/device.hip
+++ b/loupiote_amd/csrc/device.hip
@@ -7,6 +7,7 @@
 #include <map>
 #include <memory>
 #include <cstdlib>
+#include <functional>
 #include <mutex>
 #include <new>
 #include <numeric>
@@ -150,6 +151,7 @@
     hipEvent_t done = nullptr;
     hipEvent_t consumed = nullptr;
     bool consumed_recorded = false;
+    std::vector<hipEvent_t> trav;
 };
 constexpr int kMaxLanes = 4;
 constexpr uint32_t kStepBudget = 48u, kBudgetRays = 3000000u;
@@ -199,6 +201,7 @@
     int sort_queues = 0;
     uint32_t shade_blocks_per_cu = 0;
     uint32_t trace_waves_per_cu = 0;
+    uint32_t lane_phase = 1;
     uint32_t n_slots = 0;
     float4 *accum = nullptr, *scratch = nullptr;
     lpt_comm *comm = nullptr;
@@ -1063,7 +1066,7 @@
 
 static int ensure_lane(lpt_renderer *r, int l) {
     Wavefront &wf = r->wf[l];
-    if (!wf.stream) HIP_TRY(hipStreamCreateWithFlags(&wf.stream, hipStreamNonBlocking));
+    if (l > 0 && !wf.stream) HIP_TRY(hipStreamCreateWithFlags(&wf.stream, hipStreamNonBlocking));
     if (!wf.done) HIP_TRY(hipEventCreateWithFlags(&wf.done, hipEventDisableTiming));
     if (!wf.consumed) HIP_TRY(hipEventCreateWithFlags(&wf.consumed, hipEventDisableTiming));
     if (!wf.ctr) HIP_TRY(hipMalloc(&wf.ctr, sizeof(FrameCounters)));
@@ -1150,6 +1153,7 @@
         if (wf.stream) hipStreamDestroy(wf.stream);
         if (wf.done) hipEventDestroy(wf.done);
         if (wf.consumed) hipEventDestroy(wf.consumed);
+        for (hipEvent_t e : wf.trav) hipEventDestroy(e);
         if (wf.ctr) hipFree(wf.ctr);
     }
     if (r->totals) hipFree(r->totals);
@@ -1341,6 +1345,7 @@
     case LPT_OPT_EXPERIMENT(LPT_EXP_PACKET_QUADS): r->packet_quads = value != 0; break;
     case LPT_OPT_EXPERIMENT(LPT_EXP_SPLIT_RAYS): r->split_rays = value; break;
     case LPT_OPT_EXPERIMENT(LPT_EXP_BUDGET_SPLIT): r->budget_split = value != 0; break;
+    case LPT_OPT_EXPERIMENT(LPT_EXP_LANE_PHASE): if (value > 2u) return fail(LPT_ERR_INVALID_ARG, "LPT_EXP_LANE_PHASE: 0 (free), 1 (offset start), 2 (alternating traversal)"); r->lane_phase = (uint32_t)value; break;
     case LPT_OPT_TAIL_LANES: r->tail_lanes = (uint32_t)std::min<uint64_t>(value, kTailMax); break;
     case LPT_OPT_COOP_RAYS: r->coop_rays = (uint32_t)std::min<uint64_t>(value, 0x7FFFFFFFu); break;
     default: return fail(LPT_ERR_INVALID_ARG, "lpt_renderer_set_option: unknown option %d", option);
@@ -1365,6 +1370,7 @@
     case LPT_OPT_EXPERIMENT(LPT_EXP_PACKET_QUADS): *value = r->packet_quads; break;
     case LPT_OPT_EXPERIMENT(LPT_EXP_SPLIT_RAYS): *value = r->split_rays; break;
     case LPT_OPT_EXPERIMENT(LPT_EXP_BUDGET_SPLIT): *value = r->budget_split; break;
+    case LPT_OPT_EXPERIMENT(LPT_EXP_LANE_PHASE): *value = r->lane_phase; break;
     case LPT_OPT_TAIL_LANES: *value = r->tail_lanes; break;
     case LPT_OPT_COOP_RAYS: *value = r->coop_rays; break;
     default: return fail(LPT_ERR_INVALID_ARG, "lpt_renderer_get_option: unknown option %d", option);
@@ -1421,16 +1427,16 @@
     r->ev_count[slot] = 0;
 }
 static inline int cur_slot(const lpt_renderer *r) { return (int)(r->ring_pos % lpt_renderer::kRing); }
-static inline void stage_begin(lpt_renderer *r, int stage, hipStream_t stream) {
+static inline void stage_begin(lpt_renderer *r, int stage, hipStream_t stream, int slot = -1) {
     if (!r->timings) return;
-    const int slot = cur_slot(r);
+    if (slot < 0) slot = cur_slot(r);
     if (r->ev_count[slot] >= lpt_renderer::kMaxEvents) return;
     r->ev_stage[slot][r->ev_count[slot]] = stage;
     hipEventRecord(r->ev_start[slot * lpt_renderer::kMaxEvents + r->ev_count[slot]], stream);
 }
-static inline void stage_end(lpt_renderer *r, hipStream_t stream) {
+static inline void stage_end(lpt_renderer *r, hipStream_t stream, int slot = -1) {
     if (!r->timings) return;
-    const int slot = cur_slot(r);
+    if (slot < 0) slot = cur_slot(r);
     if (r->ev_count[slot] >= lpt_renderer::kMaxEvents) return;
     hipEventRecord(r->ev_stop[slot * lpt_renderer::kMaxEvents + r->ev_count[slot]], stream);
     r->ev_count[slot]++;
@@ -1461,15 +1467,19 @@
 
 extern "C" {
 
+struct PhaseHooks { hipEvent_t wait_start = nullptr, wait_trav = nullptr, rec_trav = nullptr; };
+
 struct Ticket {
     FrameParams p;
     int lane = 0;
     bool split = false, denoise = false, packet = false;
     CamBasis cur{};
+    uint32_t stages = 0;
+    std::function<int(uint32_t, const PhaseHooks &)> run;
 };
 
 static int wavefront_trace(lpt_renderer *r, const float view[16], uint32_t n_samples, uint32_t frame_count0, uint32_t seed0, bool acc0,
-                           uint32_t slot0, uint32_t piece_slots, Ticket &tk, bool solo) {
+                           uint32_t slot0, uint32_t piece_slots, Ticket &tk, bool solo, bool defer = false) {
     HIP_TRY(hipSetDevice(r->dev->ordinal));
     hipStream_t sm = r->stream;
     const uint32_t nb = r->max_bounces;
@@ -1504,7 +1514,7 @@
         if (st != LPT_OK) return st;
     }
     Wavefront &wf = r->wf[lane];
-    hipStream_t s = split ? wf.stream : sm;
+    hipStream_t s = (split && lane > 0) ? wf.stream : sm;
     r->last_lane = lane;
     if ((size_t)n_rays > wf.ray_cap && p.n_slots) {
         HIP_TRY(hipStreamSynchronize(sm));
@@ -1515,7 +1525,7 @@
             if (l == lane || r->wf[l].ray_cap >= (size_t)n_rays) continue;
             st = ensure_lane(r, l);
             if (st != LPT_OK) return st;
-            HIP_TRY(hipStreamSynchronize(r->wf[l].stream));
+            if (r->wf[l].stream) HIP_TRY(hipStreamSynchronize(r->wf[l].stream));
             st = alloc_ray_buffers(r->wf[l], n_rays);
             if (st != LPT_OK) return st;
         }
@@ -1546,8 +1556,8 @@
     const DScene &sc = r->sg->d;
     if (r->timings) { r->ring_pos++; harvest_slot(r, cur_slot(r)); }
 
+    tk.stages = 0; tk.run = nullptr;
     if (p.n_slots) {
-        HIP_TRY(hipMemsetAsync(wf.ctr, 0, sizeof(FrameCounters), s));
         const uint32_t cus = (uint32_t)r->dev->compute_units;
         const uint32_t stream_blocks = std::min<uint32_t>(div_up(n_rays, kBlock), cus * 8u);
         const uint32_t shade_blocks = std::min<uint32_t>(div_up(n_rays, kBlock), cus * (r->shade_blocks_per_cu ? r->shade_blocks_per_cu : (solo ? 4u : 3u)));
@@ -1556,20 +1566,11 @@
         waves = std::max(8u, waves & ~7u);
         const uint32_t trace_blocks = std::min<uint32_t>(div_up(n_rays, kTraceBlock), waves);
         const size_t lds = stack_bytes(sc);
-
-        stage_begin(r, ST_RAYGEN, s);
         const bool dense = (r->w % r->tile_w == 0u) && (r->h % r->tile_h == 0u);
-        if (dense) {
-            hipLaunchKernelGGL(k_raygen<true>, dim3(stream_blocks), dim3(kBlock), 0, s, p, nz, wf.q[0], wf.Lsum, wf.ctr);
-        } else {
-            hipLaunchKernelGGL(k_raygen<false>, dim3(stream_blocks), dim3(kBlock), 0, s, p, nz, wf.q[0], wf.Lsum, wf.ctr);
-        }
-        stage_end(r, s);
 
         const float pixel_rad = 2.0f * th / (float)std::max(r->h, 1u);
         const bool packet = (r->packet_primary == 1u || (r->packet_primary == 2u && pixel_rad <= kPacketMaxPixelRad));
         tk.packet = packet;
-        uint32_t seed = seed0;
         OccProbe occ{nullptr, 0u, 0.0f};
         if (r->stats && r->occ_table && r->occ_cell > 0.0f) occ = OccProbe{r->occ_table, kOccEntries - 1u, 1.0f / r->occ_cell};
         const bool tail_launch = !r->stats && (solo || r->budget_split) && n_rays <= r->budget_rays;
@@ -1577,67 +1578,89 @@
         const uint32_t budget = (tail_launch && !tail && r->step_budget) ? r->step_budget : 0u;
         const size_t tail_lds = tail ? sizeof(uint32_t) * tail_lds_words(r->sg->stats.max_depth) : 0u;
         const bool coop_all = !r->stats && r->coop_rays && n_rays <= r->coop_rays;
-        auto trace = [&](int cb, int sb) {
-            stage_begin(r, cb >= 0 ? ST_INTERSECT : ST_SHADOW, s);
-            const Queue qin = wf.q[(uint32_t)(cb < 0 ? 0 : cb) & 1u];
-            const int launch_no = cb >= 0 ? cb : (int)nb;
-            if (coop_all) {
-                const size_t clds = sizeof(uint32_t) * coop_stack_entries(kCoopStack, r->sg->stats.max_depth);
-                hipLaunchKernelGGL(k_trace_coop<false>, dim3(std::min(2u * n_rays, cus * kCoopWavesPerCu)), dim3(kTraceBlock), clds, s, sc, qin, wf.hits, wf.sq, wf.Lsum, wf.ctr, cb, sb, (const uint32_t *)nullptr, launch_no);
-                stage_end(r, s);
-                return;
+        const bool path = r->path_rays && n_rays <= r->path_rays && !coop_all;
+        const int slot = cur_slot(r);
+        Wavefront *w = &wf;
+        tk.stages = nb + 1u;
+        tk.run = [=](uint32_t t, const PhaseHooks &ph) -> int {
+            if (ph.wait_start) HIP_TRY(hipStreamWaitEvent(s, ph.wait_start, 0));
+            auto trace = [&](int cb, int sb) {
+                stage_begin(r, cb >= 0 ? ST_INTERSECT : ST_SHADOW, s, slot);
+                const Queue qin = w->q[(uint32_t)(cb < 0 ? 0 : cb) & 1u];
+                const int launch_no = cb >= 0 ? cb : (int)nb;
+                if (coop_all) {
+                    const size_t clds = sizeof(uint32_t) * coop_stack_entries(kCoopStack, r->sg->stats.max_depth);
+                    hipLaunchKernelGGL(k_trace_coop<false>, dim3(std::min(2u * n_rays, cus * kCoopWavesPerCu)), dim3(kTraceBlock), clds, s, sc, qin, w->hits, w->sq, w->Lsum, w->ctr, cb, sb, (const uint32_t *)nullptr, launch_no);
+                    stage_end(r, s, slot);
+                    return;
+                }
+                if (tail) {
+                    if (pipe) hipLaunchKernelGGL((k_trace<false, true, true>), dim3(trace_blocks), dim3(kTraceBlock), lds + tail_lds, s, TraceKernargs{sc, qin, w->hits, w->sq, w->Lsum, w->ctr, cb, sb, r->refill, occ, 0u, w->strag, launch_no, tail});
+                    else hipLaunchKernelGGL((k_trace<false, false, true>), dim3(trace_blocks), dim3(kTraceBlock), lds + tail_lds, s, TraceKernargs{sc, qin, w->hits, w->sq, w->Lsum, w->ctr, cb, sb, r->refill, occ, 0u, w->strag, launch_no, tail});
+                } else if (pipe) {
+                    if (r->stats) hipLaunchKernelGGL((k_trace<true, true>), dim3(trace_blocks), dim3(kTraceBlock), lds + 64u, s, TraceKernargs{sc, qin, w->hits, w->sq, w->Lsum, w->ctr, cb, sb, r->refill, occ, budget, w->strag, launch_no, 0u});
+                    else hipLaunchKernelGGL((k_trace<false, true>), dim3(trace_blocks), dim3(kTraceBlock), lds, s, TraceKernargs{sc, qin, w->hits, w->sq, w->Lsum, w->ctr, cb, sb, r->refill, occ, budget, w->strag, launch_no, 0u});
+                } else if (r->stats) hipLaunchKernelGGL((k_trace<true, false>), dim3(trace_blocks), dim3(kTraceBlock), lds + 64u, s, TraceKernargs{sc, qin, w->hits, w->sq, w->Lsum, w->ctr, cb, sb, r->refill, occ, budget, w->strag, launch_no, 0u});
+                else hipLaunchKernelGGL((k_trace<false, false>), dim3(trace_blocks), dim3(kTraceBlock), lds, s, TraceKernargs{sc, qin, w->hits, w->sq, w->Lsum, w->ctr, cb, sb, r->refill, occ, budget, w->strag, launch_no, 0u});
+                if (budget) {
+                    const size_t clds = sizeof(uint32_t) * coop_stack_entries(kCoopStack, r->sg->stats.max_depth);
+                    if (r->stats) hipLaunchKernelGGL(k_trace_coop<true>, dim3(cus * kCoopWavesPerCu), dim3(kTraceBlock), clds, s, sc, qin, w->hits, w->sq, w->Lsum, w->ctr, cb, sb, w->strag, launch_no);
+                    else hipLaunchKernelGGL(k_trace_coop<false>, dim3(cus * kCoopWavesPerCu), dim3(kTraceBlock), clds, s, sc, qin, w->hits, w->sq, w->Lsum, w->ctr, cb, sb, w->strag, launch_no);
+                }
+                stage_end(r, s, slot);
+            };
+            if (t == 0u) {
+                HIP_TRY(hipMemsetAsync(w->ctr, 0, sizeof(FrameCounters), s));
+                stage_begin(r, ST_RAYGEN, s, slot);
+                if (dense) {
+                    hipLaunchKernelGGL(k_raygen<true>, dim3(stream_blocks), dim3(kBlock), 0, s, p, nz, w->q[0], w->Lsum, w->ctr);
+                } else {
+                    hipLaunchKernelGGL(k_raygen<false>, dim3(stream_blocks), dim3(kBlock), 0, s, p, nz, w->q[0], w->Lsum, w->ctr);
+                }
+                stage_end(r, s, slot);
+                if (ph.wait_trav) HIP_TRY(hipStreamWaitEvent(s, ph.wait_trav, 0));
+                if (packet) {
+                    stage_begin(r, ST_PRIMARY, s, slot);
+                    const uint32_t packets = div_up(n_rays, 64u);
+                    const size_t plds = (size_t)(48u + 7u * r->sg->stats.max_depth + 8u) * sizeof(uint32_t);
+                    const uint32_t quad_slots = (r->packet_quads && dense && p.block8 && p.n_slots % 64u == 0u && p.slot0 % 64u == 0u && n_samples % 4u == 0u) ? p.n_slots : 0u;
+                    if (r->stats) hipLaunchKernelGGL(k_trace_packet<true>, dim3(std::min(packets, cus * kPacketBlocksPerCu)), dim3(kTraceBlock), plds, s, sc, w->q[0], w->hits, w->ctr, 0, quad_slots);
+                    else hipLaunchKernelGGL(k_trace_packet<false>, dim3(std::min(packets, cus * kPacketBlocksPerCu)), dim3(kTraceBlock), plds, s, sc, w->q[0], w->hits, w->ctr, 0, quad_slots);
+                    stage_end(r, s, slot);
+                } else if (coop_all || !path) trace(0, -1);
+                if (path) {
+                    stage_begin(r, ST_PATH, s, slot);
+                    const uint32_t pblocks = std::min<uint32_t>(div_up(n_rays, kTraceBlock), std::max(8u, (cus * r->path_waves_per_cu) & ~7u));
+                    const size_t plds = lds + kPathLdsExtra;
+                    if (denoise) {
+                        if (r->stats) hipLaunchKernelGGL((k_path<true, true>), dim3(pblocks), dim3(kTraceBlock), plds, s, sc, probe, nz, p, w->q[0], packet ? w->hits : (const float4 *)nullptr, w->Lsum, w->ctr, seed0, gb, r->path_refill);
+                        else hipLaunchKernelGGL((k_path<true, false>), dim3(pblocks), dim3(kTraceBlock), plds, s, sc, probe, nz, p, w->q[0], packet ? w->hits : (const float4 *)nullptr, w->Lsum, w->ctr, seed0, gb, r->path_refill);
+                    } else if (r->stats) hipLaunchKernelGGL((k_path<false, true>), dim3(pblocks), dim3(kTraceBlock), plds, s, sc, probe, nz, p, w->q[0], packet ? w->hits : (const float4 *)nullptr, w->Lsum, w->ctr, seed0, gb, r->path_refill);
+                    else hipLaunchKernelGGL((k_path<false, false>), dim3(pblocks), dim3(kTraceBlock), plds, s, sc, probe, nz, p, w->q[0], packet ? w->hits : (const float4 *)nullptr, w->Lsum, w->ctr, seed0, gb, r->path_refill);
+                    stage_end(r, s, slot);
+                }
+            } else if (!path) {
+                const uint32_t b = t - 1u;
+                const uint32_t seed = seed0 + t;
+                const Queue qin = w->q[b & 1u], qout = w->q[(b + 1u) & 1u];
+                stage_begin(r, ST_SHADE, s, slot);
+                if (denoise && b == 0u)
+                    hipLaunchKernelGGL(k_shade<true>, dim3(shade_blocks), dim3(kBlock), 0, s, sc, probe, nz, p, qin, w->hits, qout, w->sq, w->Lsum, w->ctr, (int)b, seed, gb, r->sort_queues);
+                else
+                    hipLaunchKernelGGL(k_shade<false>, dim3(shade_blocks), dim3(kBlock), 0, s, sc, probe, nz, p, qin, w->hits, qout, w->sq, w->Lsum, w->ctr, (int)b, seed, gb, r->sort_queues);
+                stage_end(r, s, slot);
+                if (ph.wait_trav) HIP_TRY(hipStreamWaitEvent(s, ph.wait_trav, 0));
+                trace(b + 1u < nb ? (int)(b + 1u) : -1, (int)b);
             }
-            if (tail) {
-                if (pipe) hipLaunchKernelGGL((k_trace<false, true, true>), dim3(trace_blocks), dim3(kTraceBlock), lds + tail_lds, s, TraceKernargs{sc, qin, wf.hits, wf.sq, wf.Lsum, wf.ctr, cb, sb, r->refill, occ, 0u, wf.strag, launch_no, tail});
-                else hipLaunchKernelGGL((k_trace<false, false, true>), dim3(trace_blocks), dim3(kTraceBlock), lds + tail_lds, s, TraceKernargs{sc, qin, wf.hits, wf.sq, wf.Lsum, wf.ctr, cb, sb, r->refill, occ, 0u, wf.strag, launch_no, tail});
-            } else if (pipe) {
-                if (r->stats) hipLaunchKernelGGL((k_trace<true, true>), dim3(trace_blocks), dim3(kTraceBlock), lds + 64u, s, TraceKernargs{sc, qin, wf.hits, wf.sq, wf.Lsum, wf.ctr, cb, sb, r->refill, occ, budget, wf.strag, launch_no, 0u});
-                else hipLaunchKernelGGL((k_trace<false, true>), dim3(trace_blocks), dim3(kTraceBlock), lds, s, TraceKernargs{sc, qin, wf.hits, wf.sq, wf.Lsum, wf.ctr, cb, sb, r->refill, occ, budget, wf.strag, launch_no, 0u});
-            } else if (r->stats) hipLaunchKernelGGL((k_trace<true, false>), dim3(trace_blocks), dim3(kTraceBlock), lds + 64u, s, TraceKernargs{sc, qin, wf.hits, wf.sq, wf.Lsum, wf.ctr, cb, sb, r->refill, occ, budget, wf.strag, launch_no, 0u});
-            else hipLaunchKernelGGL((k_trace<false, false>), dim3(trace_blocks), dim3(kTraceBlock), lds, s, TraceKernargs{sc, qin, wf.hits, wf.sq, wf.Lsum, wf.ctr, cb, sb, r->refill, occ, budget, wf.strag, launch_no, 0u});
-            if (budget) {
-                const size_t clds = sizeof(uint32_t) * coop_stack_entries(kCoopStack, r->sg->stats.max_depth);
-                if (r->stats) hipLaunchKernelGGL(k_trace_coop<true>, dim3(cus * kCoopWavesPerCu), dim3(kTraceBlock), clds, s, sc, qin, wf.hits, wf.sq, wf.Lsum, wf.ctr, cb, sb, wf.strag, launch_no);
-                else hipLaunchKernelGGL(k_trace_coop<false>, dim3(cus * kCoopWavesPerCu), dim3(kTraceBlock), clds, s, sc, qin, wf.hits, wf.sq, wf.Lsum, wf.ctr, cb, sb, wf.strag, launch_no);
-            }
-            stage_end(r, s);
+            if (ph.rec_trav) HIP_TRY(hipEventRecord(ph.rec_trav, s));
+            if (t == nb && split) HIP_TRY(hipEventRecord(w->done, s));
+            HIP_TRY(hipGetLastError());
+            return LPT_OK;
         };
-        {
-            if (packet) {
-                stage_begin(r, ST_PRIMARY, s);
-                const uint32_t packets = div_up(n_rays, 64u);
-                const size_t plds = (size_t)(48u + 7u * r->sg->stats.max_depth + 8u) * sizeof(uint32_t);
-                const uint32_t quad_slots = (r->packet_quads && dense && p.block8 && p.n_slots % 64u == 0u && p.slot0 % 64u == 0u && n_samples % 4u == 0u) ? p.n_slots : 0u;
-                if (r->stats) hipLaunchKernelGGL(k_trace_packet<true>, dim3(std::min(packets, cus * kPacketBlocksPerCu)), dim3(kTraceBlock), plds, s, sc, wf.q[0], wf.hits, wf.ctr, 0, quad_slots);
-                else hipLaunchKernelGGL(k_trace_packet<false>, dim3(std::min(packets, cus * kPacketBlocksPerCu)), dim3(kTraceBlock), plds, s, sc, wf.q[0], wf.hits, wf.ctr, 0, quad_slots);
-                stage_end(r, s);
-            } else if (coop_all || !(r->path_rays && n_rays <= r->path_rays)) trace(0, -1);
+        for (uint32_t t = 0; !defer && t < tk.stages; ++t) {
+            const int st = tk.run(t, PhaseHooks{});
+            if (st != LPT_OK) return st;
         }
-        const bool path = r->path_rays && n_rays <= r->path_rays && !coop_all;
-        if (path) {
-            stage_begin(r, ST_PATH, s);
-            const uint32_t pblocks = std::min<uint32_t>(div_up(n_rays, kTraceBlock), std::max(8u, (cus * r->path_waves_per_cu) & ~7u));
-            const size_t plds = lds + kPathLdsExtra;
-            if (denoise) {
-                if (r->stats) hipLaunchKernelGGL((k_path<true, true>), dim3(pblocks), dim3(kTraceBlock), plds, s, sc, probe, nz, p, wf.q[0], packet ? wf.hits : (const float4 *)nullptr, wf.Lsum, wf.ctr, seed0, gb, r->path_refill);
-                else hipLaunchKernelGGL((k_path<true, false>), dim3(pblocks), dim3(kTraceBlock), plds, s, sc, probe, nz, p, wf.q[0], packet ? wf.hits : (const float4 *)nullptr, wf.Lsum, wf.ctr, seed0, gb, r->path_refill);
-            } else if (r->stats) hipLaunchKernelGGL((k_path<false, true>), dim3(pblocks), dim3(kTraceBlock), plds, s, sc, probe, nz, p, wf.q[0], packet ? wf.hits : (const float4 *)nullptr, wf.Lsum, wf.ctr, seed0, gb, r->path_refill);
-            else hipLaunchKernelGGL((k_path<false, false>), dim3(pblocks), dim3(kTraceBlock), plds, s, sc, probe, nz, p, wf.q[0], packet ? wf.hits : (const float4 *)nullptr, wf.Lsum, wf.ctr, seed0, gb, r->path_refill);
-            stage_end(r, s);
-        }
-        for (uint32_t b = 0; b < nb && !path; ++b) {
-            seed += 1u;
-            const Queue qin = wf.q[b & 1u], qout = wf.q[(b + 1u) & 1u];
-            stage_begin(r, ST_SHADE, s);
-            if (denoise && b == 0u)
-                hipLaunchKernelGGL(k_shade<true>, dim3(shade_blocks), dim3(kBlock), 0, s, sc, probe, nz, p, qin, wf.hits, qout, wf.sq, wf.Lsum, wf.ctr, (int)b, seed, gb, r->sort_queues);
-            else
-                hipLaunchKernelGGL(k_shade<false>, dim3(shade_blocks), dim3(kBlock), 0, s, sc, probe, nz, p, qin, wf.hits, qout, wf.sq, wf.Lsum, wf.ctr, (int)b, seed, gb, r->sort_queues);
-            stage_end(r, s);
-            trace(b + 1u < nb ? (int)(b + 1u) : -1, (int)b);
-        }
-        if (split) HIP_TRY(hipEventRecord(wf.done, s));
-        HIP_TRY(hipGetLastError());
     }
     tk.p = p; tk.lane = lane; tk.split = split; tk.denoise = denoise; tk.cur = gb.cur;
     return LPT_OK;
@@ -1725,12 +1748,41 @@
         hipStreamSynchronize(r->stream);
         return st;
     };
-    for (uint32_t k = 0; k < pieces; ++k) {
-        if (k >= ahead) { const int st = finish(k - ahead); if (st != LPT_OK) return bail(st); }
-        const uint32_t g0 = k * per_piece, g1 = std::min(granules, g0 + per_piece);
-        r->n_wavefronts++;
-        const int st = wavefront_trace(r, b.view, b.n, b.frame_count0, b.seed0, b.acc0, g0 * granule, (g1 - g0) * granule, tk[k % ahead], pieces == 1u);
-        if (st != LPT_OK) return bail(st);
+    const uint32_t phase = (ahead > 1u && pieces > 1u) ? r->lane_phase : 0u;
+    const uint32_t group = phase ? ahead : 1u;
+    for (uint32_t k0 = 0; k0 < pieces; k0 += group) {
+        const uint32_t k1 = std::min(pieces, k0 + group);
+        for (uint32_t k = k0; k < k1; ++k) {
+            if (k >= ahead) { const int st = finish(k - ahead); if (st != LPT_OK) return bail(st); }
+            const uint32_t g0 = k * per_piece, g1 = std::min(granules, g0 + per_piece);
+            r->n_wavefronts++;
+            const int st = wavefront_trace(r, b.view, b.n, b.frame_count0, b.seed0, b.acc0, g0 * granule, (g1 - g0) * granule, tk[k % ahead], pieces == 1u, phase != 0u);
+            if (st != LPT_OK) return bail(st);
+        }
+        if (!phase) continue;
+        const uint32_t stages = tk[k0 % ahead].stages;
+        for (uint32_t k = k0; k < k1; ++k) {
+            Wavefront &wf = r->wf[tk[k % ahead].lane];
+            while (wf.trav.size() < stages) {
+                hipEvent_t e = nullptr;
+                const hipError_t he = hipEventCreateWithFlags(&e, hipEventDisableTiming);
+                if (he != hipSuccess) return bail(fail(LPT_ERR_HIP, "hipEventCreate failed: %s", hipGetErrorString(he)));
+                wf.trav.push_back(e);
+            }
+        }
+        for (uint32_t t = 0; t < stages; ++t) {
+            for (uint32_t k = k0; k < k1; ++k) {
+                const Ticket &cur = tk[k % ahead];
+                const Wavefront &prev = r->wf[tk[(k > k0 ? k - 1u : k1 - 1u) % ahead].lane];
+                PhaseHooks ph;
+                ph.rec_trav = r->wf[cur.lane].trav[t];
+                if (phase == 1u && t == 0u && k > k0) ph.wait_start = prev.trav[0];
+                if (phase == 2u && k > k0) ph.wait_trav = prev.trav[t];
+                if (phase == 2u && k == k0 && t > 0u) ph.wait_trav = prev.trav[t - 1u];
+                const int st = cur.run ? cur.run(t, ph) : LPT_OK;
+                if (st != LPT_OK) return bail(st);
+            }
+        }
     }
     for (uint32_t k = pieces > ahead ? pieces - ahead : 0u; k < pieces; ++k) { const int st = finish(k); if (st != LPT_OK) return bail(st); }
     return LPT_OK;
```

After: 6331 (median of 6 runs). +16.7%, better.
